# Hansard-T/FHE-Linformer

Measured on AMD Instinct MI355X. Metric: encrypted Linformer-d128 forward ms/sample, lower is better.
Workload: dtype u64

## Files before the change

### fhe-linformer_amd/csrc/context.cpp

```cpp
#include "context.h"
#include <hip/hip_runtime.h>
#include <algorithm>
#include <cstdio>
#include <cstdlib>
#include <cstring>
#include <sys/random.h>
#include <time.h>
#include <cxxabi.h>
#include <dlfcn.h>
#include <execinfo.h>

namespace fhelin {

void hip_check(hipError_t e, const char* what) {
    if (e != hipSuccess) throw Error(FHELIN_ERR_HIP, std::string(what) + ": " + hipGetErrorString(e));
}

void* DevicePool::raw_malloc(size_t bytes) {
    if (backend_.malloc_fn) return backend_.malloc_fn(bytes);
    void* p = nullptr;
    if (hipMalloc(&p, bytes) != hipSuccess) {
        (void)hipGetLastError();
        return nullptr;
    }
    return p;
}
void DevicePool::raw_free(void* p) {
    if (backend_.free_fn) backend_.free_fn(p);
    else (void)hipFree(p);
}
DevicePool::~DevicePool() {
    for (auto& ln : lane_) {
        for (auto& pk : ln.parked)
            for (int k = 0; k < pk.n_ev; ++k) (void)hipEventDestroy(pk.ev[k]);
        for (auto& sl : ln.slabs)
            if (sl.base) raw_free(sl.base);
    }
    for (hipEvent_t e : spare_events_) (void)hipEventDestroy(e);
}
size_t DevicePool::slabs() const {
    size_t n = 0;
    for (const auto& ln : lane_)
        for (const auto& sl : ln.slabs) n += sl.base != nullptr;
    return n;
}
size_t DevicePool::free_ranges() const {
    size_t n = 0;
    for (const auto& ln : lane_) n += ln.by_size.size();
    return n;
}
void DevicePool::erase_size_entry(Lane& ln, int slab, size_t off, size_t len) {
    auto r = ln.by_size.equal_range(len);
    for (auto it = r.first; it != r.second; ++it)
        if (it->second.first == slab && it->second.second == off) {
            ln.by_size.erase(it);
            return;
        }
    throw Error(FHELIN_ERR_INTERNAL, "DevicePool: free list out of step");
}
void DevicePool::insert_free(Lane& ln, int slab, size_t off, size_t len) {
    Slab& sl = ln.slabs[slab];
    auto nxt = sl.free_at.lower_bound(off);
    if (nxt != sl.free_at.begin()) {
        auto prv = std::prev(nxt);
        if (prv->first + prv->second == off) {
            off = prv->first;
            len += prv->second;
            erase_size_entry(ln, slab, prv->first, prv->second);
            sl.free_at.erase(prv);
        }
    }
    if (nxt != sl.free_at.end() && off + len == nxt->first) {
        len += nxt->second;
        erase_size_entry(ln, slab, nxt->first, nxt->second);
        sl.free_at.erase(nxt);
    }
    sl.free_at[off] = len;
    ln.by_size.emplace(len, std::make_pair(slab, off));
}
bool DevicePool::grow(Lane& ln, size_t bytes) {
    size_t want = std::max(bytes, std::min(SLAB_MAX, std::max(SLAB_MIN, reserved_)));
    want = (want + (size_t(2) << 20) - 1) & ~((size_t(2) << 20) - 1);
    timespec t0, t1;
    clock_gettime(CLOCK_MONOTONIC, &t0);
    void* p = raw_malloc(want);
    if (!p && want > bytes) {
        want = (bytes + (size_t(2) << 20) - 1) & ~((size_t(2) << 20) - 1);
        p = raw_malloc(want);
    }
    clock_gettime(CLOCK_MONOTONIC, &t1);
    if (!p) return false;
    malloc_calls += 1;
    malloc_bytes += want;
    malloc_ns += (u64)((t1.tv_sec - t0.tv_sec) * 1000000000ll + (t1.tv_nsec - t0.tv_nsec));
    reserved_ += want;
    if (reserved_ > reserved_peak) reserved_peak = reserved_;
    int idx = -1;
    for (size_t i = 0; i < ln.slabs.size(); ++i)
        if (!ln.slabs[i].base) idx = (int)i;
    if (idx < 0) {
        ln.slabs.emplace_back();
        idx = (int)ln.slabs.size() - 1;
    }
    Slab& sl = ln.slabs[idx];
    sl.base = static_cast<char*>(p);
    sl.size = want;
    sl.used = 0;
    sl.free_at.clear();
    insert_free(ln, idx, 0, want);
    return true;
}
void* DevicePool::alloc(size_t bytes) {
    if (bytes == 0) bytes = 256;
    const size_t gran = bytes > (size_t(64) << 10) ? 4096 : 256;
    bytes = (bytes + gran - 1) & ~(gran - 1);
    Lane& ln = lane_[cur_lane];
    if (!ln.parked.empty()) {
        for (auto& pk : ln.parked) {
            for (int k = 0; k < pk.n_ev; ++k) {
                hip_check(hipStreamWaitEvent(lane_stream[cur_lane], pk.ev[k], 0), "hipStreamWaitEvent(pool reuse)");
                spare_events_.push_back(pk.ev[k]);
            }
            insert_free(ln, pk.slab, pk.off, pk.len);
        }
        ln.parked.clear();
    }
    auto it = ln.by_size.lower_bound(bytes);
    if (it == ln.by_size.end()) {
        if (!grow(ln, bytes)) {
            trim();
            if (!grow(ln, bytes)) throw Error(FHELIN_ERR_HIP, "hipMalloc: out of device memory (" + std::to_string(bytes >> 20) + " MiB asked, " +
                                                                  std::to_string(reserved_ >> 20) + " MiB held, " + std::to_string(live_bytes_ >> 20) + " MiB in use)");
        }
        it = ln.by_size.lower_bound(bytes);
    }
    const int slab = it->second.first;
    const size_t off = it->second.second, len = it->first;
    Slab& sl = ln.slabs[slab];
    ln.by_size.erase(it);
    sl.free_at.erase(off);
    if (len > bytes) {
        sl.free_at[off + bytes] = len - bytes;
        ln.by_size.emplace(len - bytes, std::make_pair(slab, off + bytes));
    }
    sl.used += bytes;
    void* p = sl.base + off;
    live_[p] = Live{bytes, cur_lane, slab, off};
    live_bytes_ += bytes;
    if (live_bytes_ > live_peak) live_peak = live_bytes_;
    return p;
}
void DevicePool::free(void* p, unsigned used_by_lanes) {
    if (!p) return;
    auto it = live_.find(p);
    if (it == live_.end()) throw Error(FHELIN_ERR_STATE, "DevicePool::free of unknown pointer");
    const Live lv = it->second;
    live_.erase(it);
    live_bytes_ -= lv.bytes;
    Lane& ln = lane_[lv.lane];
    ln.slabs[lv.slab].used -= lv.bytes;
    unsigned wait = used_by_lanes;
    if (have_streams && lv.lane != cur_lane) {
        wait |= 1u << cur_lane;
        if (conservative_foreign_free)
            for (int k = 0; k <= n_user_lanes; ++k) wait |= 1u << k;
    }
    wait &= ~(1u << lv.lane);
    if (!have_streams || !wait) {
        insert_free(ln, lv.slab, lv.off, lv.bytes);
        return;
    }
    Parked pk{lv.slab, lv.off, lv.bytes, {}, 0};
    for (int k = 0; k < MAX_LANES; ++k) {
        if (!(wait & (1u << k)) || !lane_stream[k]) continue;
        hipEvent_t ev = nullptr;
        if (!spare_events_.empty()) {
            ev = spare_events_.back();
            spare_events_.pop_back();
        } else {
            hip_check(hipEventCreateWithFlags(&ev, hipEventDisableTiming), "hipEventCreate(pool)");
        }
        hip_check(hipEventRecord(ev, lane_stream[k]), "hipEventRecord(pool free)");
        pk.ev[pk.n_ev++] = ev;
    }
    foreign_frees += 1;
    ln.parked.push_back(pk);
}
void DevicePool::trim() {
    trims += 1;
    if (!backend_.malloc_fn) (void)hipDeviceSynchronize();
    for (auto& ln : lane_) {
        for (auto& pk : ln.parked) {
            for (int k = 0; k < pk.n_ev; ++k) spare_events_.push_back(pk.ev[k]);
            insert_free(ln, pk.slab, pk.off, pk.len);
        }
        ln.parked.clear();
        for (size_t i = 0; i < ln.slabs.size(); ++i) {
            Slab& sl = ln.slabs[i];
            if (!sl.base || sl.used != 0) continue;
            erase_size_entry(ln, (int)i, 0, sl.size);
            raw_free(sl.base);
            reserved_ -= sl.size;
            sl = Slab();
        }
    }
}

template <class T>
const T* Context::upload_table(const std::vector<T>& v) {
    void* p = nullptr;
    size_t bytes = std::max<size_t>(v.size() * sizeof(T), 16);
    hip_check(hipMalloc(&p, bytes), "hipMalloc(table)");
    if (!v.empty()) hip_check(hipMemcpy(p, v.data(), v.size() * sizeof(T), hipMemcpyHostToDevice), "hipMemcpy(table)");
    table_allocs.push_back(p);
    return static_cast<const T*>(p);
}
template const u64* Context::upload_table<u64>(const std::vector<u64>&);
template const int* Context::upload_table<int>(const std::vector<int>&);
template const u32* Context::upload_table<u32>(const std::vector<u32>&);
template const double* Context::upload_table<double>(const std::vector<double>&);

static u64 mont_r(u64 m) { return (u64)((((u128)1) << 64) % m); }

static u64 prod_mod(const std::vector<u64>& ms, int skip, u64 t) {
    u64 r = 1 % t;
    for (int i = 0; i < (int)ms.size(); ++i)
        if (i != skip) r = h_mulmod(r, ms[i] % t, t);
    return r;
}

static void resolve_seed(Params& p) {
    if (p.have_seed_bytes) return;
    if (p.seed != 0) {
        std::memset(p.seed_bytes, 0, sizeof p.seed_bytes);
        for (int i = 0; i < 8; ++i) p.seed_bytes[i] = (uint8_t)(p.seed >> (8 * i));
    } else {
        size_t got = 0;
        while (got < sizeof p.seed_bytes) {
            const ssize_t n = getrandom(p.seed_bytes + got, sizeof p.seed_bytes - got, 0);
            if (n <= 0) throw Error(FHELIN_ERR_INTERNAL, "getrandom failed: no entropy for key generation");
            got += (size_t)n;
        }
    }
    p.have_seed_bytes = true;
}

static Params resolve_params(Params p) {
    resolve_seed(p);
    if (p.n_p < 0 && p.n_q >= 1 && p.dnum >= 1 && p.special_bits >= 1) {
        const int a = (p.n_q + p.dnum - 1) / p.dnum;
        const int first = p.first_bits + (std::min(a, p.n_q) - 1) * p.scale_bits;
        const int other = p.n_q > a ? std::min(a, p.n_q - a) * p.scale_bits : 0;
        p.n_p = (std::max(first, other) + p.special_bits - 1) / p.special_bits;
    }
    return p;
}

Context::Context(const Params& p_in) : prm(resolve_params(p_in)) {
    const Params& p = prm;
    if (p.log_n < 12 || p.log_n > 17) throw Error(FHELIN_ERR_ARG, "log_n must be in [12,17]");
    if (p.n_q < 1 || p.n_q > 64 || p.n_p < 0 || p.n_p > 16) throw Error(FHELIN_ERR_ARG, "bad limb counts");
    if (p.dnum < 1) throw Error(FHELIN_ERR_ARG, "dnum must be >= 1");
    if (p.first_bits > 60 || p.scale_bits > 60 || p.special_bits > 60) throw Error(FHELIN_ERR_ARG, "primes must be <= 60 bits");
    if (p.first_bits < 20 || p.scale_bits < 20 || (p.n_p > 0 && p.special_bits < 20)) throw Error(FHELIN_ERR_ARG, "primes must be >= 20 bits");
    if (p.log_slots < 1 || p.log_slots > p.log_n - 1) throw Error(FHELIN_ERR_ARG, "log_slots out of range");
    N = 1 << p.log_n;
    L = p.n_q - 1;
    K = p.n_p;
    alpha = (p.n_q + p.dnum - 1) / p.dnum;
    if (alpha > 16) throw Error(FHELIN_ERR_ARG, "digit size > 16 limbs not supported");
    if ((p.n_q + alpha - 1) / alpha > 16) throw Error(FHELIN_ERR_ARG, "more than 16 key-switching digits not supported");
    try {
        chain = make_prime_chain(p.log_n, p.n_q, p.first_bits, p.scale_bits, p.n_p, p.special_bits);
    } catch (const std::exception& e) {
        throw Error(FHELIN_ERR_ARG, std::string("prime chain: ") + e.what());
    }
    moduli = chain.q;
    moduli.insert(moduli.end(), chain.p.begin(), chain.p.end());
    for (u64 q : moduli)
        if (q >> 60) throw Error(FHELIN_ERR_ARG, "prime chain: a modulus is >= 2^60 (lower scale_bits or first_bits)");
    for (u64 q : moduli) {
        barrett.push_back(h_barrett(q));
        tw.push_back(make_twiddles(q, p.log_n));
    }
    sf_real.assign(p.n_q + 1, 0.0L);
    sf_real[0] = (long double)chain.q[L];
    for (int k = 0; k < L; ++k) sf_real[k + 1] = sf_real[k] * sf_real[k] / (long double)chain.q[L - k];

    if (p.device < 0) return;

    int ndev = 0;
    if (hipGetDeviceCount(&ndev) != hipSuccess || ndev <= 0)
        throw Error(FHELIN_ERR_NO_DEVICE, "no HIP device visible: the fhe-linformer_amd engine has no CPU fallback");
    if (p.device >= ndev) throw Error(FHELIN_ERR_ARG, "device index out of range");
    hip_check(hipSetDevice(p.device), "hipSetDevice");
    hip_check(hipStreamCreateWithFlags(&stream, hipStreamNonBlocking), "hipStreamCreate");
    main_stream = stream;
    own_stream = true;
    {
        int want = 2;
        if (const char* e = std::getenv("FHELIN_LANES")) want = std::atoi(e);
        n_lanes = std::max(0, std::min(want, DevicePool::MAX_LANES - 1));
        for (int k = 1; k <= n_lanes; ++k) {
            hip_check(hipStreamCreateWithFlags(&lane_stream[k], hipStreamNonBlocking), "hipStreamCreate(lane)");
            hip_check(hipEventCreateWithFlags(&lane_event[k], hipEventDisableTiming), "hipEventCreate(lane)");
        }
        hip_check(hipEventCreateWithFlags(&fork_event, hipEventDisableTiming), "hipEventCreate(fork)");
        pool.lane_stream[0] = main_stream;
        for (int k = 1; k <= n_lanes; ++k) pool.lane_stream[k] = lane_stream[k];
        pool.have_streams = true;
        if (const char* e = std::getenv("FHELIN_ASYNC")) async_lanes = std::atoi(e) != 0;
        if (const char* e = std::getenv("FHELIN_FUSE_MODDOWN")) fuse_moddown = std::atoi(e) != 0;
        if (const char* e = std::getenv("FHELIN_FUSE_FINISH")) fuse_finish = std::atoi(e) != 0;
        if (const char* e = std::getenv("FHELIN_HOST_ENCODE")) host_encode = std::atoi(e) != 0;
        if (const char* e = std::getenv("FHELIN_FUSE_GATHER")) fuse_gather = std::atoi(e) != 0;
        if (const char* e = std::getenv("FHELIN_FUSE_LIFT")) fuse_lift = std::atoi(e) != 0;
        if (const char* e = std::getenv("FHELIN_LDS_DIGITS")) lds_digits = std::atoi(e) != 0;
        if (const char* e = std::getenv("FHELIN_NTT_TRACE")) trace_small_ntt = std::atoi(e);
        if (const char* e = std::getenv("FHELIN_HOST_WAITS")) trace_waits = std::atoi(e) != 0;
    }
    hip_check(hipEventCreate(&ev_start), "hipEventCreate");
    stage_words = (size_t)2 << p.log_n;
    for (int i = 0; i < STAGE_SLOTS; ++i) {
        hip_check(hipHostMalloc(reinterpret_cast<void**>(&stage_buf[i]), stage_words * sizeof(u64), hipHostMallocDefault), "hipHostMalloc(stage)");
        hip_check(hipEventCreateWithFlags(&stage_ev[i], hipEventDisableTiming), "hipEventCreate(stage)");
    }
    hip_check(hipHostMalloc(reinterpret_cast<void**>(&small_buf), (size_t)SMALL_SLOTS * SMALL_WORDS * sizeof(u64), hipHostMallocDefault), "hipHostMalloc(stage, small)");
    for (int i = 0; i < SMALL_SLOTS; ++i) hip_check(hipEventCreateWithFlags(&small_ev[i], hipEventDisableTiming), "hipEventCreate(stage, small)");
    hip_check(hipEventCreate(&ev_stop), "hipEventCreate");
    has_device = true;

    const int nl = (int)moduli.size();
    {
        std::vector<u64> bar(2 * nl), ninv(8 * nl, 0);
        for (int i = 0; i < nl; ++i) {
            bar[2 * i] = barrett[i].r0;
            bar[2 * i + 1] = barrett[i].r1;
            ninv[8 * i] = tw[i].n_inv;
            ninv[8 * i + 1] = tw[i].n_inv_s;
            ninv[8 * i + 2] = tw[i].w1_n_inv;
            ninv[8 * i + 3] = tw[i].w1_n_inv_s;
            int bits = 0;
            while (bits < 64 && (moduli[i] >> bits)) ++bits;
            if (bits >= 12 && bits <= 60) {
                ninv[8 * i + 4] = (u64)(bits - 10);
                ninv[8 * i + 5] = (u64)((((u128)1) << (bits + 22)) / moduli[i]);
            }
        }
        dt.log_n = p.log_n;
        dt.n_limbs = nl;
        dt.moduli = upload_table(moduli);
        dt.barrett = upload_table(bar);
        {
            std::vector<u64> qi(nl);
            for (int i = 0; i < nl; ++i) {
                u64 x = moduli[i];
                for (int it = 0; it < 6; ++it) x *= 2 - moduli[i] * x;
                qi[i] = x;
            }
            dt.qinv = upload_table(qi);
            std::vector<u64> mr(2 * (size_t)nl);
            for (int i = 0; i < nl; ++i) {
                mr[2 * i] = mont_r(moduli[i]);
                mr[2 * i + 1] = h_shoup(mr[2 * i], moduli[i]);
            }
            dt.mont = upload_table(mr);
        }
        dt.ninv = upload_table(ninv);
        std::vector<u64> f((size_t)nl * 2 * N), g((size_t)nl * 2 * N);
        for (int i = 0; i < nl; ++i) {
            std::memcpy(&f[(size_t)i * 2 * N], tw[i].fwd.data(), sizeof(u64) * 2 * N);
            std::memcpy(&g[(size_t)i * 2 * N], tw[i].inv.data(), sizeof(u64) * 2 * N);
        }
        dt.tw_fwd = upload_table(f);
        dt.tw_inv = upload_table(g);
        const size_t tiles = N >> 12;
        const size_t per_limb = tiles * 15 * 256 * 2;
        for (int dir = 0; dir < 2; ++dir) {
            const std::vector<u64>& src = dir ? g : f;
            std::vector<u64> r((size_t)nl * per_limb);
            for (int i = 0; i < nl; ++i)
                for (size_t T = 0; T < tiles; ++T)
                    for (int kb = 0; kb < 4; ++kb)
                        for (int j = 0; j < (8 >> kb); ++j)
                            for (size_t tau = 0; tau < 256; ++tau) {
                                const size_t idx = (N >> (kb + 1)) + ((((T << 8) | tau)) << (3 - kb)) + j;
                                const size_t s_ = (size_t)(8 >> kb) - 1 + j;
                                const size_t o = (size_t)i * per_limb + ((T * 15 + s_) * 256 + tau) * 2;
                                r[o] = src[(size_t)i * 2 * N + 2 * idx];
                                r[o + 1] = src[(size_t)i * 2 * N + 2 * idx + 1];
                            }
            (dir ? dt.tw_rows_inv : dt.tw_rows_fwd) = upload_table(r);
        }
    }
    {
        std::vector<u64> phatinv(2 * std::max(K, 1)), phatmod((size_t)std::max(K, 1) * (L + 1)), pinv(2 * (L + 1));
        for (int j = 0; j < K; ++j) {
            u64 pj = chain.p[j];
            u64 hat = prod_mod(chain.p, j, pj);
            u64 inv = h_invmod(hat, pj);
            phatinv[2 * j] = inv;
            phatinv[2 * j + 1] = h_shoup(inv, pj);
            for (int t = 0; t <= L; ++t) phatmod[(size_t)j * (L + 1) + t] = pack30(h_mulmod(prod_mod(chain.p, j, chain.q[t]), mont_r(chain.q[t]), chain.q[t]));
        }
        for (int t = 0; t <= L; ++t) {
            u64 qt = chain.q[t];
            u64 pm = prod_mod(chain.p, -1, qt);
            u64 inv = K > 0 ? h_invmod(pm, qt) : 1;
            pinv[2 * t] = inv;
            pinv[2 * t + 1] = h_shoup(inv, qt);
        }
        d_phatinv = upload_table(phatinv);
        d_phatmod = upload_table(phatmod);
        d_pinv = upload_table(pinv);
        std::vector<u64> pmod(2 * (L + 1));
        for (int t = 0; t <= L; ++t) {
            pmod[2 * t] = prod_mod(chain.p, -1, chain.q[t]);
            pmod[2 * t + 1] = h_shoup(pmod[2 * t], chain.q[t]);
        }
        d_pmod = upload_table(pmod);
        std::vector<u64> qlinv((size_t)(L + 1) * (L + 1) * 2, 0), qlmod((size_t)(L + 1) * (L + 1), 0);
        for (int l = 0; l <= L; ++l)
            for (int t = 0; t < l; ++t) {
                u64 qt = chain.q[t];
                u64 r = chain.q[l] % qt;
                u64 inv = h_invmod(r, qt);
                qlmod[(size_t)l * (L + 1) + t] = r;
                qlinv[((size_t)l * (L + 1) + t) * 2] = inv;
                qlinv[((size_t)l * (L + 1) + t) * 2 + 1] = h_shoup(inv, qt);
            }
        d_qlinv = upload_table(qlinv);
        d_qlmod = upload_table(qlmod);
    }
    lvl.resize(L + 2);
    for (int ell = 1; ell <= L + 1; ++ell) {
        LevelTables& lt = lvl[ell];
        lt.ell = ell;
        lt.beta = digits_at(ell);
        const int nt = ell + K;
        std::vector<u64> hatinv(2 * ell), hatmod((size_t)ell * nt, 0), hatmod2((size_t)ell * nt, 0);
        std::vector<int> tab((size_t)lt.beta * nt, -1);
        for (int j = 0; j < lt.beta; ++j) {
            const int lo = j * alpha, hi = std::min((j + 1) * alpha, ell);
            std::vector<u64> dig(chain.q.begin() + lo, chain.q.begin() + hi);
            for (int i = lo; i < hi; ++i) {
                u64 qi = chain.q[i];
                u64 inv = h_invmod(prod_mod(dig, i - lo, qi), qi);
                hatinv[2 * i] = inv;
                hatinv[2 * i + 1] = h_shoup(inv, qi);
                for (int t = 0; t < nt; ++t) {
                    u64 mt = t < ell ? chain.q[t] : chain.p[t - ell];
                    const u64 hr = h_mulmod(prod_mod(dig, i - lo, mt), mont_r(mt), mt);
                    hatmod[(size_t)i * nt + t] = pack30(hr);
                    hatmod2[(size_t)i * nt + t] = pack30(h_mulmod(hr, mont_r(mt), mt));
                }
            }
            for (int t = 0; t < nt; ++t) {
                bool own = t >= lo && t < hi;
                tab[(size_t)j * nt + t] = own ? -1 : (t < ell ? limb_id_q(t) : limb_id_p(t - ell));
            }
        }
        lt.up_hatinv = upload_table(hatinv);
        lt.up_hatmod = upload_table(hatmod);
        lt.up_hatmod_r2 = upload_table(hatmod2);
        lt.ext_limb_tab = upload_table(tab);
        if (ell >= 2 && K >= 1) {
            const u64 ql = chain.q[ell - 1];
            const int e1 = ell - 1;
            std::vector<u64> mhi(2 * (K + 1)), mhm((size_t)(K + 1) * e1), minv(2 * e1), mmod(e1);
            for (int j = 0; j <= K; ++j) {
                const u64 b = j < K ? chain.p[j] : ql;
                const u64 hat_b = j < K ? h_mulmod(prod_mod(chain.p, j, b), ql % b, b) : prod_mod(chain.p, -1, b);
                const u64 inv = h_invmod(hat_b, b);
                mhi[2 * j] = inv;
                mhi[2 * j + 1] = h_shoup(inv, b);
                for (int t = 0; t < e1; ++t) {
                    const u64 qt = chain.q[t];
                    mhm[(size_t)j * e1 + t] = pack30(j < K ? h_mulmod(prod_mod(chain.p, j, qt), ql % qt, qt) : prod_mod(chain.p, -1, qt));
                }
            }
            for (int t = 0; t < e1; ++t) {
                const u64 qt = chain.q[t];
                mmod[t] = h_mulmod(prod_mod(chain.p, -1, qt), ql % qt, qt);
                const u64 inv = h_invmod(mmod[t], qt);
                minv[2 * t] = inv;
                minv[2 * t + 1] = h_shoup(inv, qt);
            }
            lt.md_hatinv = upload_table(mhi);
            lt.md_hatmod = upload_table(mhm);
            lt.md_minv = upload_table(minv);
            lt.md_mmod = upload_table(mmod);
        }
    }
}

void Context::upload_async(u64* dst, const u64* src, size_t words) {
    if (words <= SMALL_WORDS && small_buf) {
        const int i = small_next;
        small_next = (small_next + 1) % SMALL_SLOTS;
        if (small_used[i]) {
            timespec a, b;
            if (trace_waits) clock_gettime(CLOCK_MONOTONIC, &a);
            hip_check(hipEventSynchronize(small_ev[i]), "hipEventSynchronize(stage, small)");
            if (trace_waits) {
                clock_gettime(CLOCK_MONOTONIC, &b);
                note_wait("upload ring (small)", (u64)((b.tv_sec - a.tv_sec) * 1000000000ll + (b.tv_nsec - a.tv_nsec)));
            }
        }
        u64* slot = small_buf + (size_t)i * SMALL_WORDS;
        std::memcpy(slot, src, words * sizeof(u64));
        hip_check(hipMemcpyAsync(dst, slot, words * sizeof(u64), hipMemcpyHostToDevice, stream), "hipMemcpyAsync(stage, small)");
        hip_check(hipEventRecord(small_ev[i], stream), "hipEventRecord(stage, small)");
        small_used[i] = true;
        return;
    }
    if (words > stage_words) throw Error(FHELIN_ERR_INTERNAL, "upload_async: block larger than a staging slot");
    const int i = stage_next;
    stage_next = (stage_next + 1) % STAGE_SLOTS;
    if (stage_used[i]) {
        timespec a, b;
        if (trace_waits) clock_gettime(CLOCK_MONOTONIC, &a);
        hip_check(hipEventSynchronize(stage_ev[i]), "hipEventSynchronize(stage)");
        if (trace_waits) {
            clock_gettime(CLOCK_MONOTONIC, &b);
            note_wait("upload ring (large)", (u64)((b.tv_sec - a.tv_sec) * 1000000000ll + (b.tv_nsec - a.tv_nsec)));
        }
    }
    std::memcpy(stage_buf[i], src, words * sizeof(u64));
    hip_check(hipMemcpyAsync(dst, stage_buf[i], words * sizeof(u64), hipMemcpyHostToDevice, stream), "hipMemcpyAsync(stage)");
    hip_check(hipEventRecord(stage_ev[i], stream), "hipEventRecord(stage)");
    stage_used[i] = true;
}

Context::~Context() {
    if (trace_waits) {
        fprintf(stderr, "[fhelin] host time blocked inside the library, by site (waits, ms):\n");
        for (const auto& e : wait_sites) fprintf(stderr, "  %8llu %10.1f  %s\n", (unsigned long long)e.second.first, e.second.second / 1e6, e.first.c_str());
    }
    if (trace_small_ntt && !small_ntt_sites.empty()) {
        std::vector<std::pair<std::string, std::pair<u64, u64>>> v(small_ntt_sites.begin(), small_ntt_sites.end());
        std::sort(v.begin(), v.end(), [](const auto& a, const auto& b) { return a.second.first > b.second.first; });
        fprintf(stderr, "[fhelin] transforms of <= %d limb vectors by call stack (launch pairs, limb vectors):\n", trace_small_ntt);
        for (size_t i = 0; i < v.size() && i < 40; ++i)
            fprintf(stderr, "  %8llu %9llu  %s\n", (unsigned long long)v[i].second.first, (unsigned long long)v[i].second.second, v[i].first.c_str());
    }
    if (has_device) {
        (void)hipSetDevice(prm.device);
        (void)hipDeviceSynchronize();
        for (void* p : table_allocs) (void)hipFree(p);
        for (int k = 1; k <= n_lanes; ++k) {
            if (lane_event[k]) (void)hipEventDestroy(lane_event[k]);
            if (lane_stream[k]) (void)hipStreamDestroy(lane_stream[k]);
        }
        if (fork_event) (void)hipEventDestroy(fork_event);
        for (int i = 0; i < STAGE_SLOTS; ++i) {
            if (stage_ev[i]) (void)hipEventDestroy(stage_ev[i]);
            if (stage_buf[i]) (void)hipHostFree(stage_buf[i]);
        }
        for (int i = 0; i < SMALL_SLOTS; ++i)
            if (small_ev[i]) (void)hipEventDestroy(small_ev[i]);
        if (small_buf) (void)hipHostFree(small_buf);
        if (ev_start) (void)hipEventDestroy(ev_start);
        if (ev_stop) (void)hipEventDestroy(ev_stop);
        if (own_stream && main_stream) (void)hipStreamDestroy(main_stream);
    }
}

void Context::require_device() const {
    if (!has_device)
        throw Error(FHELIN_ERR_NO_DEVICE, "operation needs the HIP device path (host-only context): no CPU fallback exists");
}

void Context::sync() {
    require_device();
    hip_check(hipStreamSynchronize(stream), "hipStreamSynchronize");
    if (stream == main_stream) {
        for (int k = 1; k <= n_lanes; ++k) {
            hip_check(hipStreamSynchronize(lane_stream[k]), "hipStreamSynchronize(lane)");
            lane_hold[k].clear();
        }
    }
}

void Context::note_small_ntt(int nvec) {
    void* fr[12];
    const int n = backtrace(fr, 12);
    std::string key;
    for (int i = 2; i < n && i < 9; ++i) {
        Dl_info info;
        std::string name = "?";
        if (dladdr(fr[i], &info) && info.dli_sname) {
            int st = 0;
            char* d = abi::__cxa_demangle(info.dli_sname, nullptr, nullptr, &st);
            name = (st == 0 && d) ? d : info.dli_sname;
            if (d) std::free(d);
            const size_t par = name.find('(');
            if (par != std::string::npos) name.resize(par);
        }
        key += (i > 2 ? " < " : "") + name;
    }
    auto& e = small_ntt_sites[key];
    e.first += 1;
    e.second += (u64)nvec;
}

void Context::release_holds(int lane, u64 up_to_seq) {
    auto& h = lane_hold[lane];
    h.erase(std::remove_if(h.begin(), h.end(), [&](const std::pair<u64, std::shared_ptr<void>>& e) { return e.first <= up_to_seq; }),
            h.end());
}

void Context::fork_lanes() {
    hip_check(hipEventRecord(fork_event, main_stream), "hipEventRecord(fork)");
    for (int k = 1; k <= n_lanes; ++k) hip_check(hipStreamWaitEvent(lane_stream[k], fork_event, 0), "hipStreamWaitEvent(fork)");
}

void Context::join_lanes() {
    for (int k = 1; k <= n_lanes; ++k) {
        hip_check(hipEventRecord(lane_event[k], lane_stream[k]), "hipEventRecord(lane)");
        hip_check(hipStreamWaitEvent(main_stream, lane_event[k], 0), "hipStreamWaitEvent(join)");
    }
}

u64 Context::galois_element(int r) const {
    const u64 M = 2ull * N;
    const u64 order = N / 2;
    long rr = r % (long)order;
    if (rr < 0) rr += order;
    u64 g = 1, b = 5;
    u64 e = (u64)rr;
    while (e) {
        if (e & 1) g = (g * b) % M;
        b = (b * b) % M;
        e >>= 1;
    }
    return g;
}

static std::vector<u32> build_automorph_map(u64 g, size_t N, int ln) {
    const u64 M = 2ull * N;
    std::vector<u32> m(N);
    for (u32 j = 0; j < (u32)N; ++j) {
        u64 e = (2ull * bitrev32(j, ln) + 1) * g % M;
        m[j] = bitrev32((u32)((e - 1) >> 1), ln);
    }
    return m;
}

const u32* Context::automorph_map(u64 g) {
    require_device();
    auto it = automorph_maps.find(g);
    if (it != automorph_maps.end()) return it->second;
    const u64 M = 2ull * N;
    u64 gi = g;
    for (int i = 0; i < 6; ++i) gi = gi * (2 - g * gi % M + M) % M;
    const u32* d = upload_table(build_automorph_map(g, N, prm.log_n));
    automorph_maps[g] = d;
    const u32* di = d;
    if (gi != g) {
        auto iit = automorph_maps.find(gi);
        di = iit != automorph_maps.end() ? iit->second : upload_table(build_automorph_map(gi, N, prm.log_n));
        automorph_maps[gi] = di;
    }
    automorph_inverse[d] = di;
    automorph_inverse[di] = d;
    return d;
}

const u32* Context::automorph_inverse_of(const u32* map) {
    if (!map) return nullptr;
    auto it = automorph_inverse.find(map);
    if (it == automorph_inverse.end()) throw Error(FHELIN_ERR_INTERNAL, "automorphism map without a registered inverse");
    return it->second;
}

}
```

### fhe-linformer_amd/csrc/context.h

```cpp
#pragma once
#include <cstdint>
#include <map>
#include <memory>
#include <stdexcept>
#include <string>
#include <unordered_map>
#include <vector>
#include <hip/hip_runtime_api.h>
#include "../../include/fhelin.h"
#include "hostmath.h"
#include "kernels.h"

namespace fhelin {

struct Params {
    int log_n = 16;
    int n_q = 24;
    int first_bits = 55;
    int scale_bits = 52;
    int n_p = 6;
    int special_bits = 60;
    int dnum = 4;
    int log_slots = 14;
    int hamming = 192;
    uint64_t seed = 0;
    uint8_t seed_bytes[32] = {};
    bool have_seed_bytes = false;
    int device = 0;
};

struct Error : std::runtime_error {
    int code;
    Error(int c, const std::string& m) : std::runtime_error(m), code(c) {}
};

void hip_check(hipError_t e, const char* what);

class DevicePool {
public:
    static constexpr int MAX_LANES = 5;
    static constexpr size_t SLAB_MAX = size_t(8) << 30, SLAB_MIN = size_t(32) << 20;
    struct Backend {
        void* (*malloc_fn)(size_t) = nullptr;
        void (*free_fn)(void*) = nullptr;
    };
    DevicePool() = default;
    explicit DevicePool(const Backend& b) : backend_(b) {}
    ~DevicePool();
    void* alloc(size_t bytes);
    void free(void* p, unsigned used_by_lanes = 0);
    bool conservative_foreign_free = false;
    int n_user_lanes = 0;
    void trim();
    size_t bytes_reserved() const { return reserved_; }
    size_t bytes_live() const { return live_bytes_; }
    size_t slabs() const;
    size_t free_ranges() const;
    int cur_lane = 0;
    hipStream_t lane_stream[MAX_LANES] = {};
    bool have_streams = false;
    u64 malloc_calls = 0, malloc_bytes = 0, malloc_ns = 0;
    u64 foreign_frees = 0;
    u64 trims = 0;
    size_t live_peak = 0, reserved_peak = 0;
private:
    struct Slab {
        char* base = nullptr;
        size_t size = 0, used = 0;
        std::map<size_t, size_t> free_at;
    };
    struct Live { size_t bytes; int lane; int slab; size_t off; };
    struct Parked { int slab; size_t off, len; hipEvent_t ev[MAX_LANES]; int n_ev; };
    struct Lane {
        std::vector<Slab> slabs;
        std::multimap<size_t, std::pair<int, size_t>> by_size;
        std::vector<Parked> parked;
    };
    Backend backend_;
    Lane lane_[MAX_LANES];
    std::unordered_map<void*, Live> live_;
    std::vector<hipEvent_t> spare_events_;
    size_t reserved_ = 0, live_bytes_ = 0;
    void insert_free(Lane& ln, int slab, size_t off, size_t len);
    void erase_size_entry(Lane& ln, int slab, size_t off, size_t len);
    bool grow(Lane& ln, size_t bytes);
    void* raw_malloc(size_t bytes);
    void raw_free(void* p);
};

template <class T>
class Scratch {
public:
    Scratch() = default;
    Scratch(DevicePool& pool, size_t count) : pool_(&pool), p_(static_cast<T*>(pool.alloc(count * sizeof(T)))) {}
    Scratch(Scratch&& o) noexcept : pool_(o.pool_), p_(o.release()) {}
    Scratch& operator=(Scratch&& o) noexcept {
        if (this != &o) {
            drop();
            pool_ = o.pool_;
            p_ = o.release();
        }
        return *this;
    }
    Scratch(const Scratch&) = delete;
    Scratch& operator=(const Scratch&) = delete;
    ~Scratch() { drop(); }
    operator T*() const& { return p_; }
    operator T*() && = delete;
    T* get() const { return p_; }
    void reset() {
        if (T* p = release()) pool_->free(p);
    }
    T* release() noexcept {
        T* p = p_;
        p_ = nullptr;
        return p;
    }
private:
    void drop() noexcept {
        try { reset(); } catch (...) {}
    }
    DevicePool* pool_ = nullptr;
    T* p_ = nullptr;
};

struct LevelTables {
    int ell = 0;
    int beta = 0;
    const u64* up_hatinv = nullptr;
    const u64* up_hatmod = nullptr;
    const u64* up_hatmod_r2 = nullptr;
    const int* ext_limb_tab = nullptr;
    const u64* md_hatinv = nullptr;
    const u64* md_hatmod = nullptr;
    const u64* md_minv = nullptr;
    const u64* md_mmod = nullptr;
};

struct OpStats {
    u64 limb_ntt = 0;
    u64 keyswitch = 0;
    u64 keyswitch_limbs = 0;
    u64 rescale = 0;
    u64 ct_pt_mult = 0;
    u64 bootstrap = 0;
    u64 encode = 0;
    u64 rescale_limbs = 0;
    u64 ct_pt_limbs = 0;
};

struct Context {
    Params prm;
    OpStats stats;
    int N = 0;
    int L = 0;
    int K = 0;
    int alpha = 0;
    PrimeChain chain;
    std::vector<u64> moduli;
    std::vector<Barrett> barrett;
    std::vector<TwiddleTable> tw;
    std::vector<long double> sf_real;

    bool has_device = false;
    hipStream_t stream = nullptr;
    hipStream_t main_stream = nullptr;
    bool own_stream = false;
    int n_lanes = 0;
    hipStream_t lane_stream[DevicePool::MAX_LANES] = {};
    hipEvent_t lane_event[DevicePool::MAX_LANES] = {};
    hipEvent_t fork_event = nullptr;
    bool async_lanes = true;
    int async_rr = 0;
    u64 lane_seq[DevicePool::MAX_LANES] = {};
    std::vector<std::pair<u64, std::shared_ptr<void>>> lane_hold[DevicePool::MAX_LANES];
    void release_holds(int lane, u64 up_to_seq);
    void fork_lanes();
    void join_lanes();
    struct LaneScope {
        Context& c;
        LaneScope(Context& ctx, int k) : c(ctx) {
            c.stream = c.lane_stream[k];
            c.pool.cur_lane = k;
        }
        ~LaneScope() {
            c.stream = c.main_stream;
            c.pool.cur_lane = 0;
        }
    };
    DevicePool pool;
    DeviceTables dt{};
    std::vector<void*> table_allocs;
    hipEvent_t ev_start = nullptr, ev_stop = nullptr;

    static constexpr int STAGE_SLOTS = 64;
    u64* stage_buf[STAGE_SLOTS] = {};
    hipEvent_t stage_ev[STAGE_SLOTS] = {};
    bool stage_used[STAGE_SLOTS] = {};
    int stage_next = 0;
    size_t stage_words = 0;
    static constexpr int SMALL_SLOTS = 256;
    static constexpr size_t SMALL_WORDS = 8192;
    u64* small_buf = nullptr;
    hipEvent_t small_ev[SMALL_SLOTS] = {};
    bool small_used[SMALL_SLOTS] = {};
    int small_next = 0;
    void upload_async(u64* dst, const u64* src, size_t words);

    const u64* d_phatinv = nullptr;
    const u64* d_phatmod = nullptr;
    const u64* d_pinv = nullptr;
    const u64* d_pmod = nullptr;
    const u64* d_qlinv = nullptr;
    const u64* d_qlmod = nullptr;
    std::vector<LevelTables> lvl;
    std::map<u64, const u32*> automorph_maps;

    explicit Context(const Params& p);
    ~Context();
    Context(const Context&) = delete;
    Context& operator=(const Context&) = delete;

    void require_device() const;
    template <class T> T* dalloc(size_t count) { return static_cast<T*>(pool.alloc(count * sizeof(T))); }
    template <class T> Scratch<T> scratch(size_t count) { return Scratch<T>(pool, count); }
    template <class T> const T* upload_table(const std::vector<T>& v);
    int limb_id_q(int i) const { return i; }
    int limb_id_p(int j) const { return L + 1 + j; }
    int digits_at(int ell) const { return (ell + alpha - 1) / alpha; }
    u64 galois_element(int rot_index) const;
    const u32* automorph_map(u64 galois);
    const u32* automorph_inverse_of(const u32* map);
    std::map<const u32*, const u32*> automorph_inverse;
    bool fuse_finish = true;
    bool fuse_moddown = false;
    bool host_encode = false;
    bool fuse_gather = true;
    bool fuse_lift = true;
    bool lds_digits = true;
    struct FftDev {
        const u32* rot = nullptr;
        const double* ksi = nullptr;
    };
    std::map<int, FftDev> fft_dev;
    void sync();
    void ntt(const LimbBatch& b, bool inverse, int active = -1) {
        stats.limb_ntt += (u64)(active >= 0 ? active : b.nvec);
        if (trace_small_ntt && b.nvec <= trace_small_ntt) note_small_ntt(b.nvec);
        launch_ntt(dt, b, inverse, stream);
    }
    bool trace_waits = false;
    std::map<std::string, std::pair<u64, u64>> wait_sites;
    void note_wait(const char* site, u64 ns) {
        auto& e = wait_sites[site];
        e.first += 1;
        e.second += ns;
    }
    int trace_small_ntt = 0;
    std::map<std::string, std::pair<u64, u64>> small_ntt_sites;
    void note_small_ntt(int nvec);
    void ntt_epilogue(const LimbBatch& b, const NttEpilogue& ep) {
        stats.limb_ntt += (u64)b.nvec;
        if (trace_small_ntt && b.nvec <= trace_small_ntt) note_small_ntt(b.nvec);
        launch_ntt_epilogue(dt, b, ep, stream);
    }
};

}
```

### fhe-linformer_amd/csrc/evaluator.cpp

```cpp
#include "evaluator.h"
#include <map>
#include <hip/hip_runtime.h>
#include <cmath>
#include <cstring>

namespace fhelin {

DevBlock::~DevBlock() {
    if (d && ctx) {
        try { ctx->pool.free(d); } catch (...) {}
    }
}
Ciphertext::~Ciphertext() {
    if (async_ev) (void)hipEventDestroy(async_ev);
    if (d && ctx && !block) {
        try { ctx->pool.free(d); } catch (...) {}
    }
}
Encoding::~Encoding() {
    if (ready) (void)hipEventDestroy(ready);
    if (d && ctx) {
        try { ctx->pool.free(d, lanes_ordered); } catch (...) {}
    }
}
EvalKey::~EvalKey() {
    if (d && ctx) {
        try { ctx->pool.free(d); } catch (...) {}
    }
    if (d_perm && ctx) {
        try { ctx->pool.free(d_perm); } catch (...) {}
    }
}

static void launch_ok(const char* what) { hip_check(hipGetLastError(), what); }

CtPtr Evaluator::new_ct(int npoly, int ell, int deg, long double scale, int slots) {
    c_.require_device();
    if (ell < 1 || ell > c_.L + 1 || npoly < 1 || npoly > 3) throw Error(FHELIN_ERR_ARG, "new_ct: bad shape");
    auto ct = std::make_shared<Ciphertext>();
    ct->ctx = &c_;
    ct->npoly = npoly;
    ct->ell = ell;
    ct->deg = deg;
    ct->scale = scale;
    ct->slots = slots;
    ct->d = c_.dalloc<u64>(ct->words());
    return ct;
}

CtPtr Evaluator::clone(const CtPtr& a) {
    CtPtr o = new_ct(a->npoly, a->ell, a->deg, a->scale, a->slots);
    hip_check(hipMemcpyAsync(o->d, a->d, a->words() * 8, hipMemcpyDeviceToDevice, c_.stream), "clone");
    return o;
}

std::vector<CtPtr> Evaluator::new_ct_batch(int count, int npoly, int ell, int deg, long double scale, int slots) {
    c_.require_device();
    if (count < 1 || ell < 1 || ell > c_.L + 1 + (c_.K > 0 ? 1 : 0) || npoly < 1 || npoly > 3) throw Error(FHELIN_ERR_ARG, "new_ct_batch: bad shape");
    auto blk = std::make_shared<DevBlock>();
    blk->ctx = &c_;
    const size_t words = (size_t)npoly * ell * c_.N;
    blk->d = c_.dalloc<u64>(words * count);
    std::vector<CtPtr> v;
    for (int i = 0; i < count; ++i) {
        auto ct = std::make_shared<Ciphertext>();
        ct->ctx = &c_;
        ct->npoly = npoly;
        ct->ell = ell;
        ct->deg = deg;
        ct->scale = scale;
        ct->slots = slots;
        ct->block = blk;
        ct->d = blk->d + words * i;
        v.push_back(ct);
    }
    return v;
}

u64* Evaluator::contiguous_base(const std::vector<CtPtr>& v) {
    if (v.empty() || !v[0]->block) return nullptr;
    const size_t words = v[0]->words();
    for (size_t i = 0; i < v.size(); ++i)
        if (v[i]->block != v[0]->block || v[i]->d != v[0]->d + words * i || v[i]->words() != words) return nullptr;
    return v[0]->d;
}

std::vector<CtPtr> Evaluator::make_contiguous(const std::vector<CtPtr>& v, int site) {
    if (v.size() <= 1 || contiguous_base(v)) return v;
    if (site >= 0 && site < 8) gather_copies[site] += v.size();
    std::vector<CtPtr> o = new_ct_batch((int)v.size(), v[0]->npoly, v[0]->ell, v[0]->deg, v[0]->scale, v[0]->slots);
    for (size_t lo = 0; lo < v.size(); lo += EwItems::MAX_ITEMS) {
        EwItems it;
        it.n = (int)std::min<size_t>(EwItems::MAX_ITEMS, v.size() - lo);
        it.vecs = v[0]->npoly * v[0]->ell;
        it.b_vecs = 0;
        for (int i = 0; i < it.n; ++i) {
            if (v[lo + i]->words() != v[0]->words()) throw Error(FHELIN_ERR_INTERNAL, "make_contiguous: operands of different shapes");
            it.out[i] = o[lo + i]->d;
            it.a[i] = v[lo + i]->d;
            it.b[i] = nullptr;
        }
        launch_ew_items(c_.dt, it, 4, v[0]->ell, c_.stream);
    }
    hip_check(hipGetLastError(), "batch gather");
    return o;
}

KeyPtr Evaluator::new_key() {
    c_.require_device();
    auto k = std::make_shared<EvalKey>();
    k->ctx = &c_;
    k->digits = c_.digits_at(c_.L + 1);
    k->d = c_.dalloc<u64>(k->words());
    return k;
}

void Evaluator::keyswitch(const u64* c_ntt, int ell, const EvalKey& key, u64* out, const u64* add0, const u64* add1,
                          const u32* map, const u64* post) {
    keyswitch_batch(1, c_ntt, 0, ell, key, out, 0, add0, add1, 0, map, post, 0);
}

void Evaluator::keyswitch_batch(int B, const u64* c_ntt, size_t c_stride, int ell, const EvalKey& key, u64* out, size_t out_stride,
                                const u64* add0, const u64* add1, size_t add_stride, const u32* map, const u64* post,
                                size_t post_stride) {
    keyswitch_impl(B, nullptr, c_ntt, c_stride, ell, &key, out, out_stride, add0, add1, add_stride, map, post, post_stride);
}

void Evaluator::keyswitch_rows(const KsRows& rows, const u64* c_ntt, size_t c_stride, int ell, u64* out, size_t out_stride,
                               const u64* add0, size_t add_stride) {
    const int B = (int)rows.keys.size();
    if (B < 1) return;
    if (B > KsShape::MAX_ROWS || rows.maps.size() != rows.keys.size()) throw Error(FHELIN_ERR_ARG, "keyswitch_rows: bad row count");
    keyswitch_impl(B, &rows, c_ntt, c_stride, ell, nullptr, out, out_stride, add0, nullptr, add_stride, nullptr, nullptr, 0);
}

void Evaluator::keyswitch_impl(int B, const KsRows* rows, const u64* c_ntt, size_t c_stride, int ell, const EvalKey* key, u64* out,
                               size_t out_stride, const u64* add0, const u64* add1, size_t add_stride, const u32* map, const u64* post,
                               size_t post_stride) {
    c_.require_device();
    if (c_.K < 1) throw Error(FHELIN_ERR_STATE, "hybrid key switching needs at least one special prime");
    if (B < 1) return;
    const size_t N = c_.N;
    const int K = c_.K;
    KsShape sh{ell, K, c_.alpha, c_.lvl[ell].beta, c_.L + 1, B, c_stride, out_stride, add_stride, post_stride};
    const bool shared = rows && rows->shared_input;
    if (rows) {
        sh.per_row = 1;
        sh.shared_input = shared ? 1 : 0;
        for (int b = 0; b < B; ++b) {
            sh.evk_row[b] = rows->keys[b]->d;
            sh.map_row[b] = rows->maps[b];
        }
    }
    KsShape shu = sh;
    shu.batch = shared ? 1 : B;
    c_.stats.keyswitch += (u64)B;
    c_.stats.keyswitch_limbs += (u64)B * ell;
    Scratch<u64> ext = modup(shu, c_ntt, true);
    Scratch<u64> accQ = c_.scratch<u64>((size_t)B * 2 * ell * N);
    Scratch<u64> accP = c_.scratch<u64>((size_t)B * 2 * K * N);
    launch_ks_inner(c_.dt, sh, accQ, accP, ext, key ? key->d : nullptr, c_ntt, c_.stream);
    const bool identity = !map && !rows;
    moddown(sh, accQ, accP, out, add0, add1, map, post, c_.fuse_moddown || (c_.fuse_finish && identity));
    launch_ok("keyswitch");
}


Scratch<u64> Evaluator::modup(const KsShape& up, const u64* src, bool times_r2, int group2, size_t group2_stride) {
    const size_t N = c_.N;
    const int n = up.batch, ell = up.ell, nt = ell + c_.K;
    const LevelTables& lt = c_.lvl[ell];
    Scratch<u64> cc = c_.scratch<u64>((size_t)n * ell * N);
    {
        LimbBatch ib{cc, n * ell, nullptr, 0, ell, src};
        if (n > 1 && up.c_stride != (size_t)ell * N) {
            ib.src_group = ell;
            ib.src_group_stride = up.c_stride;
        }
        if (group2 > 0) {
            ib.src_group2 = group2;
            ib.src_group2_stride = group2_stride;
        }
        c_.ntt(ib, true);
    }
    Scratch<u64> ext = c_.scratch<u64>((size_t)n * lt.beta * nt * N);
    launch_modup_conv(c_.dt, up, ext, cc, src, lt.up_hatinv, times_r2 ? lt.up_hatmod_r2 : lt.up_hatmod, c_.stream);
    LimbBatch eb{ext, n * lt.beta * nt, lt.ext_limb_tab, 0, 1};
    eb.tab_len = lt.beta * nt;
    eb.lazy_out = true;
    c_.ntt(eb, false, n * (lt.beta * nt - ell));
    return ext;
}

void Evaluator::moddown(const KsShape& sh, const u64* accQ, u64* accP, u64* out, const u64* add0, const u64* add1, const u32* map,
                        const u64* post, bool row_pass, const std::function<void(const u64* conv)>& finish) {
    const size_t N = c_.N;
    const int B = sh.batch, ell = sh.ell, K = c_.K;
    c_.ntt(LimbBatch{accP, B * 2 * K, nullptr, c_.L + 1, K}, true);
    Scratch<u64> conv = c_.scratch<u64>((size_t)B * 2 * ell * N);
    launch_moddown_conv(c_.dt, sh, conv, accP, c_.d_phatinv, c_.d_phatmod, c_.stream);
    const LimbBatch cb{conv, B * 2 * ell, nullptr, 0, ell};
    if (row_pass) {
        NttEpilogue ep;
        ep.acc = accQ;
        ep.acc_poly_stride = (size_t)ell * N;
        ep.out = out;
        ep.out_stride = sh.out_stride;
        ep.w = c_.d_pinv;
        ep.ell = ell;
        ep.add0 = add0;
        ep.add1 = add1;
        ep.add_stride = sh.add_stride;
        ep.post = post;
        ep.post_stride = sh.post_stride;
        if (sh.per_row) {
            ep.per_row = 1;
            for (int b = 0; b < B; ++b) ep.invmap_row[b] = c_.automorph_inverse_of(sh.map_row[b]);
        } else if (map) {
            ep.invmap = c_.automorph_inverse_of(map);
        }
        c_.ntt_epilogue(cb, ep);
        return;
    }
    c_.ntt(cb, false);
    if (finish) finish(conv);
    else launch_moddown_finish(c_.dt, sh, out, accQ, conv, c_.d_pinv, add0, add1, map, post, c_.stream);
}

void Evaluator::moddown_rescale(const KsShape& sh, const u64* accQ, u64* accP, u64* out) {
    const size_t N = c_.N;
    const int B = sh.batch, ell = sh.ell, K = c_.K;
    const LevelTables& lt = c_.lvl[ell];
    c_.ntt(LimbBatch{accP, B * 2 * K, nullptr, c_.L + 1, K}, true);
    Scratch<u64> top = c_.scratch<u64>((size_t)B * 2 * N);
    {
        LimbBatch tb{top, B * 2, nullptr, ell - 1, 1, accQ + (size_t)(ell - 1) * N};
        tb.src_group = 1;
        tb.src_group_stride = (size_t)ell * N;
        c_.ntt(tb, true);
    }
    Scratch<u64> conv = c_.scratch<u64>((size_t)B * 2 * (ell - 1) * N);
    launch_moddown_rescale_conv(c_.dt, sh, conv, accP, top, lt.md_hatinv, lt.md_hatmod, lt.md_mmod, c_.stream);
    moddown_rescale_finish(sh, out, accQ, conv, lt.md_minv);
}

void Evaluator::moddown_rescale_finish(const KsShape& sh, u64* out, const u64* accQ, u64* conv, const u64* minv) {
    const int e1 = sh.ell - 1;
    const LimbBatch cb{conv, sh.batch * 2 * e1, nullptr, 0, e1};
    if (c_.fuse_finish) {
        NttEpilogue ep;
        ep.acc = accQ;
        ep.acc_poly_stride = (size_t)sh.ell * c_.N;
        ep.out = out;
        ep.out_stride = sh.out_stride;
        ep.w = minv;
        ep.ell = e1;
        c_.ntt_epilogue(cb, ep);
        return;
    }
    c_.ntt(cb, false);
    launch_moddown_rescale_finish(c_.dt, sh, out, accQ, conv, minv, c_.stream);
}

bool Evaluator::have_rotation_keys(const std::vector<int>& indices, int slots) const {
    const int ns = slots > 0 ? slots : (1 << c_.prm.log_slots);
    for (int r : indices) {
        if (r % ns == 0) return false;
        if (!rot_keys.count(c_.galois_element(r))) return false;
    }
    return !indices.empty();
}

const u64* Evaluator::permuted(const EvalKey& key, const u32* map) {
    if (key.d_perm) return key.d_perm;
    const int nvec = key.digits * 2 * (c_.L + 1 + c_.K);
    key.d_perm = c_.dalloc<u64>(key.words());
    launch_automorph_pack30(c_.dt, key.d_perm, key.d, map, nvec, c_.stream);
    launch_ok("key permutation");
    hip_check(hipStreamSynchronize(c_.stream), "key permutation sync");
    return key.d_perm;
}

std::vector<CtPtr> Evaluator::rotate_sum_batch(const std::vector<CtPtr>& vin, const std::vector<int>& indices) {
    if (vin.empty()) return {};
    const int R = (int)indices.size();
    if (R < 1 || R > KsShape::MAX_ROT) throw Error(FHELIN_ERR_ARG, "rotate_sum_batch: 1..7 rotations");
    if (!have_rotation_keys(indices, vin[0]->slots)) throw Error(FHELIN_ERR_KEY, "rotate_sum_batch: missing rotation key");
    if (c_.K < 1) throw Error(FHELIN_ERR_STATE, "hybrid key switching needs at least one special prime");
    std::vector<const EvalKey*> keys;
    std::vector<const u32*> maps;
    for (int r : indices) {
        const u64 g = c_.galois_element(r);
        keys.push_back(rot_keys.at(g).get());
        maps.push_back(c_.automorph_map(g));
    }
    const size_t N = c_.N;
    const int K = c_.K, L1 = c_.L + 1;
    hipStream_t s = c_.stream;
    std::vector<CtPtr> out(vin.size());
    std::vector<char> done(vin.size(), 0);
    for (size_t first = 0; first < vin.size(); ++first) {
        if (done[first]) continue;
        if (vin[first]->npoly != 2) throw Error(FHELIN_ERR_STATE, "rotate: ciphertext must have 2 components");
        std::vector<size_t> idx;
        for (size_t i = first; i < vin.size() && (int)idx.size() < batch_limit; ++i) {
            const CtPtr &a = vin[first], &b = vin[i];
            if (!done[i] && b->npoly == 2 && b->ell == a->ell && b->deg == a->deg && fabsl(b->scale / a->scale - 1.0L) < 1e-9L)
                idx.push_back(i);
        }
        std::vector<CtPtr> chunk;
        for (size_t i : idx) chunk.push_back(vin[i]);
        chunk = make_contiguous(chunk, 0);
        const int B = (int)chunk.size(), ell = chunk[0]->ell;
        const size_t pn = (size_t)ell * N, ctw = 2 * pn;
        const LevelTables& lt = c_.lvl[ell];
        std::vector<CtPtr> o = new_ct_batch(B, 2, ell, chunk[0]->deg, chunk[0]->scale, chunk[0]->slots);
        const u64* base = chunk[0]->d;
        KsShape sh{ell, K, c_.alpha, lt.beta, L1, B, ctw, ctw, pn, ctw};
        sh.n_rot = R;
        sh.lds_digits = c_.lds_digits ? 1 : 0;
        for (int r = 0; r < R; ++r) {
            sh.evk_rot[r] = permuted(*keys[r], maps[r]);
            sh.map_rot[r] = maps[r];
            if (c_.galois_element(indices[r]) % (u64)(c_.N / 256) != 1) sh.lds_digits = 0;
        }
        int steps = 0;
        while ((1 << steps) < R + 1) ++steps;
        c_.stats.keyswitch += (u64)B * steps;
        c_.stats.keyswitch_limbs += (u64)B * steps * ell;
        {
            Scratch<u64> ext = modup(sh, base + pn, false);
            Scratch<u64> accQ = c_.scratch<u64>((size_t)B * 2 * ell * N);
            Scratch<u64> accP = c_.scratch<u64>((size_t)B * 2 * K * N);
            launch_ks_inner_multi(c_.dt, sh, accQ, accP, ext, base + pn, s);
            Scratch<u64> c0sum;
            if (c_.fuse_gather) {
                sh.gsrc = base;
                sh.gsrc_stride = ctw;
            } else {
                c0sum = c_.scratch<u64>((size_t)B * ell * N);
                launch_gather_sum(c_.dt, sh, c0sum, base, ctw, s);
            }
            moddown(sh, accQ, accP, o[0]->d, c0sum, nullptr, nullptr, base);
            launch_ok("rotate_sum_batch");
        }
        for (int b = 0; b < B; ++b) {
            o[b]->scale = vin[idx[b]]->scale;
            out[idx[b]] = o[b];
            done[idx[b]] = 1;
        }
    }
    return out;
}

Evaluator::FoldedKey Evaluator::folded_key(const PtPtr& p, int index, long double scale) {
    const u64 g = c_.galois_element(index);
    auto kit = rot_keys.find(g);
    if (kit == rot_keys.end()) throw Error(FHELIN_ERR_KEY, "no rotation key for index " + std::to_string(index) + " (EvalRotateKeyGen list)");
    for (size_t i = 0; i < folded_keys.size(); ++i) {
        const FoldedKey& f = folded_keys[i];
        if (f.pt.get() == p.get() && f.key.get() == kit->second.get() && f.index == index && f.scale == scale) {
            FoldedKey hit = f;
            if (i + 1 != folded_keys.size()) {
                folded_keys.erase(folded_keys.begin() + i);
                folded_keys.push_back(hit);
            }
            return hit;
        }
    }
    FoldedKey f;
    f.pt = p;
    f.key = kit->second;
    f.index = index;
    f.scale = scale;
    const int nl = c_.L + 1 + c_.K;
    f.enc = p->at(nl, scale);
    f.d = std::make_shared<DevBlock>();
    f.d->ctx = &c_;
    f.d->d = c_.dalloc<u64>(f.key->words());
    launch_fold_key(c_.dt, f.d->d, f.key->d, c_.automorph_map(g), f.enc->d, f.key->digits * 2 * nl, c_.stream);
    launch_ok("fold_key");
    hip_check(hipStreamSynchronize(c_.stream), "fold_key sync");
    if (folded_keys.size() >= MAX_FOLDED) {
        hip_check(hipStreamSynchronize(c_.main_stream), "folded key eviction sync");
        for (int k = 1; k <= c_.n_lanes; ++k) hip_check(hipStreamSynchronize(c_.lane_stream[k]), "folded key eviction sync (lane)");
        folded_keys.erase(folded_keys.begin());
    }
    folded_keys.push_back(f);
    return f;
}

std::vector<CtPtr> Evaluator::hoisted_dot_rows(const std::vector<CtPtr>& xin, const std::vector<PtPtr>& pts, const std::vector<int>& indices,
                                              bool rescale_out) {
    if (xin.empty()) return {};
    const int R = (int)indices.size();
    if (R < 1 || R > KsShape::MAX_ROT || (int)pts.size() != R + 1)
        throw Error(FHELIN_ERR_ARG, "hoisted_dot_rows: 1..7 rotations, one plaintext per rotation + the unrotated term's");
    if (!have_rotation_keys(indices, xin[0]->slots)) throw Error(FHELIN_ERR_KEY, "hoisted_dot_rows: missing rotation key");
    if (c_.K < 1) throw Error(FHELIN_ERR_STATE, "hybrid key switching needs at least one special prime");
    const int ns = xin[0]->slots > 0 ? xin[0]->slots : (1 << c_.prm.log_slots);
    for (int r : indices)
        if (r % ns == 0) throw Error(FHELIN_ERR_ARG, "hoisted_dot_rows: a rotation by 0 is the unrotated term (pts[0])");
    if (rescale_out && c_.K + 1 > 16)
        return rescale_batch(hoisted_dot_rows(xin, pts, indices, false));
    std::vector<CtPtr> x = xin;
    {
        std::vector<CtPtr> need;
        std::vector<size_t> pos;
        for (size_t i = 0; i < x.size(); ++i)
            if (x[i]->deg >= 2) {
                need.push_back(x[i]);
                pos.push_back(i);
            }
        if (!need.empty()) {
            std::vector<CtPtr> r = rescale_batch(need);
            for (size_t k = 0; k < pos.size(); ++k) x[pos[k]] = r[k];
        }
    }
    std::vector<const u32*> maps;
    for (int r : indices) maps.push_back(c_.automorph_map(c_.galois_element(r)));
    const size_t N = c_.N;
    const int K = c_.K, L1 = c_.L + 1;
    hipStream_t s = c_.stream;
    std::vector<CtPtr> out(x.size());
    std::vector<char> done(x.size(), 0);
    for (size_t first = 0; first < x.size(); ++first) {
        if (done[first]) continue;
        if (x[first]->npoly != 2) throw Error(FHELIN_ERR_STATE, "hoisted_dot_rows: ciphertext must have 2 components");
        std::vector<size_t> idx;
        for (size_t i = first; i < x.size() && (int)idx.size() < batch_limit; ++i) {
            const CtPtr &a = x[first], &b = x[i];
            if (!done[i] && b->npoly == 2 && b->ell == a->ell && b->deg == a->deg && fabsl(b->scale / a->scale - 1.0L) < 1e-9L) idx.push_back(i);
        }
        std::vector<CtPtr> chunk;
        for (size_t i : idx) chunk.push_back(x[i]);
        chunk = make_contiguous(chunk, 0);
        const int B = (int)chunk.size(), ell = chunk[0]->ell;
        const size_t pn = (size_t)ell * N, ctw = 2 * pn;
        const LevelTables& lt = c_.lvl[ell];
        const long double sf = c_.sf_real[chunk[0]->level()];
        const bool merged = rescale_out && ell >= 2 && K + 1 <= 16;
        if (rescale_out && !merged) throw Error(FHELIN_ERR_STATE, "hoisted_dot_rows: no limb left to drop");
        const int oell = merged ? ell - 1 : ell;
        std::vector<CtPtr> o = new_ct_batch(B, 2, oell, merged ? chunk[0]->deg : chunk[0]->deg + 1, chunk[0]->scale * sf, chunk[0]->slots);
        const u64* base = chunk[0]->d;
        KsShape sh{ell, K, c_.alpha, lt.beta, L1, B, ctw, (size_t)2 * oell * N, pn, ctw};
        sh.n_rot = R;
        sh.lds_digits = c_.lds_digits ? 1 : 0;
        HoistAdd h;
        h.n_rot = R;
        std::vector<FoldedKey> hold;
        const std::shared_ptr<Encoding> e0 = pts[0]->at(ell, sf);
        h.v[0] = e0->d;
        for (int r = 0; r < R; ++r) {
            hold.push_back(folded_key(pts[r + 1], indices[r], sf));
            sh.evk_rot[r] = hold.back().d->d;
            sh.map_rot[r] = maps[r];
            h.v[r + 1] = hold.back().enc->d;
            h.map[r] = maps[r];
            if (c_.galois_element(indices[r]) % (u64)(c_.N / 256) != 1) sh.lds_digits = 0;
        }
        c_.stats.keyswitch += (u64)B * R;
        c_.stats.keyswitch_limbs += (u64)B * R * ell;
        c_.stats.ct_pt_mult += (u64)B * (R + 1);
        c_.stats.ct_pt_limbs += (u64)B * (R + 1) * ell;
        if (merged) {
            c_.stats.rescale += (u64)B;
            c_.stats.rescale_limbs += (u64)B * ell;
        }
        {
            Scratch<u64> ext = modup(sh, base + pn, false);
            Scratch<u64> accQ = c_.scratch<u64>((size_t)B * 2 * ell * N);
            Scratch<u64> accP = c_.scratch<u64>((size_t)B * 2 * K * N);
            launch_ks_inner_multi(c_.dt, sh, accQ, accP, ext, base + pn, s);
            if (!merged) {
                Scratch<u64> pre = c_.scratch<u64>((size_t)B * ctw);
                launch_hoist_addends(c_.dt, sh, h, pre, base, s);
                moddown(sh, accQ, accP, o[0]->d, nullptr, nullptr, nullptr, pre);
            } else {
                h.acc = accQ;
                h.pmod = c_.d_pmod;
                launch_hoist_addends(c_.dt, sh, h, nullptr, base, s);
                moddown_rescale(sh, accQ, accP, o[0]->d);
            }
            launch_ok("hoisted_dot_rows");
        }
        for (int b = 0; b < B; ++b) {
            o[b]->scale = x[idx[b]]->scale * sf;
            if (merged) o[b]->scale = o[b]->scale / (long double)c_.chain.q[ell - 1];
            out[idx[b]] = o[b];
            done[idx[b]] = 1;
        }
    }
    return out;
}

CtPtr Evaluator::rotate_each_sum(const std::vector<CtPtr>& vin, const std::vector<int>& indices) {
    if (vin.empty() || vin.size() != indices.size()) throw Error(FHELIN_ERR_ARG, "rotate_each_sum: one index per ciphertext");
    const int ns = vin[0]->slots > 0 ? vin[0]->slots : (1 << c_.prm.log_slots);
    std::vector<CtPtr> rot;
    std::vector<int> ridx;
    CtPtr acc;
    for (size_t i = 0; i < vin.size(); ++i) {
        if (indices[i] % ns == 0) acc = acc ? add(acc, vin[i]) : vin[i];
        else {
            rot.push_back(vin[i]);
            ridx.push_back(indices[i]);
        }
    }
    for (size_t first = 0; first < rot.size(); first += KsShape::MAX_ROT) {
        const int R = (int)std::min(rot.size() - first, (size_t)KsShape::MAX_ROT);
        std::vector<CtPtr> chunk(rot.begin() + first, rot.begin() + first + R);
        bool uniform = have_rotation_keys(std::vector<int>(ridx.begin() + first, ridx.begin() + first + R), ns) && c_.K >= 1;
        for (const CtPtr& c : chunk)
            uniform = uniform && c->npoly == 2 && c->ell == chunk[0]->ell && c->deg == chunk[0]->deg &&
                      fabsl(c->scale / chunk[0]->scale - 1.0L) < 1e-9L;
        if (!uniform || R < 2) {
            for (int r = 0; r < R; ++r) {
                CtPtr t = rotate(chunk[r], ridx[first + r]);
                acc = acc ? add(acc, t) : t;
            }
            continue;
        }
        chunk = make_contiguous(chunk, 1);
        const size_t N = c_.N;
        const int K = c_.K, L1 = c_.L + 1, ell = chunk[0]->ell;
        const size_t pn = (size_t)ell * N, ctw = 2 * pn;
        const LevelTables& lt = c_.lvl[ell];
        const int nt = ell + K;
        hipStream_t s = c_.stream;
        const u64* base = chunk[0]->d;
        CtPtr o = new_ct(2, ell, chunk[0]->deg, chunk[0]->scale, chunk[0]->slots);
        {
            Scratch<u64> ext = modup(KsShape{ell, K, c_.alpha, lt.beta, L1, R, ctw, 0, 0, 0}, base + pn, false);
            KsShape sh{ell, K, c_.alpha, lt.beta, L1, 1, 0, ctw, pn, 0};
            sh.n_rot = R;
            sh.rot_ext_stride = (size_t)lt.beta * nt * N;
            sh.rot_input_stride = ctw;
            for (int r = 0; r < R; ++r) {
                const u64 g = c_.galois_element(ridx[first + r]);
                sh.map_rot[r] = c_.automorph_map(g);
                sh.evk_rot[r] = permuted(*rot_keys.at(g), sh.map_rot[r]);
            }
            c_.stats.keyswitch += (u64)R;
            c_.stats.keyswitch_limbs += (u64)R * ell;
            Scratch<u64> accQ = c_.scratch<u64>((size_t)2 * ell * N);
            Scratch<u64> accP = c_.scratch<u64>((size_t)2 * K * N);
            launch_ks_inner_multi(c_.dt, sh, accQ, accP, ext, base + pn, s);
            Scratch<u64> c0sum;
            if (c_.fuse_gather) {
                sh.gsrc = base;
                sh.gsrc_stride = 0;
            } else {
                c0sum = c_.scratch<u64>((size_t)ell * N);
                launch_gather_sum(c_.dt, sh, c0sum, base, 0, s);
            }
            moddown(sh, accQ, accP, o->d, c0sum, nullptr, nullptr, nullptr);
            launch_ok("rotate_each_sum");
        }
        acc = acc ? add(acc, o) : o;
    }
    return acc;
}

std::vector<CtPtr> Evaluator::rotate_each_sum_rows(const std::vector<std::vector<CtPtr>>& rows, const std::vector<int>& indices) {
    if (rows.empty()) return {};
    const int ns = rows[0][0]->slots > 0 ? rows[0][0]->slots : (1 << c_.prm.log_slots);
    std::vector<int> rot_pos, plain_pos, ridx;
    for (size_t r = 0; r < indices.size(); ++r) {
        if (indices[r] % ns == 0) plain_pos.push_back((int)r);
        else {
            rot_pos.push_back((int)r);
            ridx.push_back(indices[r]);
        }
    }
    const int R = (int)rot_pos.size();
    bool uniform = R >= 2 && R <= KsShape::MAX_ROT && have_rotation_keys(ridx, ns) && c_.K >= 1;
    const CtPtr& f = rows[0][0];
    for (const auto& row : rows) {
        uniform = uniform && row.size() == indices.size();
        for (const CtPtr& c : row)
            uniform = uniform && c->npoly == 2 && c->ell == f->ell && c->deg == f->deg && fabsl(c->scale / f->scale - 1.0L) < 1e-9L;
    }
    std::vector<CtPtr> out(rows.size());
    if (!uniform) {
        for (size_t b = 0; b < rows.size(); ++b) out[b] = rotate_each_sum(rows[b], indices);
        return out;
    }
    const size_t N = c_.N;
    const int K = c_.K, L1 = c_.L + 1, ell = f->ell;
    const size_t pn = (size_t)ell * N, ctw = 2 * pn;
    const LevelTables& lt = c_.lvl[ell];
    const int nt = ell + K;
    hipStream_t s = c_.stream;
    const size_t chunk_rows = (size_t)std::max(1, batch_limit / 2);
    for (size_t lo = 0; lo < rows.size(); lo += chunk_rows) {
        const size_t hi = std::min(rows.size(), lo + chunk_rows);
        const int B = (int)(hi - lo);
        std::vector<CtPtr> flat;
        for (size_t b = lo; b < hi; ++b)
            for (int r : rot_pos) flat.push_back(rows[b][r]);
        size_t row_stride = (size_t)R * ctw;
        bool regular = B >= 1 && flat[0]->block != nullptr;
        for (int b = 0; b < B && regular; ++b) {
            for (int r = 0; r < R && regular; ++r) {
                const CtPtr& c = flat[(size_t)b * R + r];
                regular = c->block == flat[0]->block && c->words() == (size_t)ctw &&
                          c->d == flat[(size_t)b * R]->d + (size_t)r * ctw;
            }
            if (regular && b == 1) {
                regular = flat[R]->d > flat[0]->d;
                if (regular) row_stride = (size_t)(flat[R]->d - flat[0]->d);
            }
            if (regular && b >= 1) regular = flat[(size_t)b * R]->d == flat[0]->d + (size_t)b * row_stride;
        }
        if (!regular) {
            flat = make_contiguous(flat, 2);
            row_stride = (size_t)R * ctw;
        }
        const u64* base = flat[0]->d;
        std::vector<CtPtr> o = new_ct_batch(B, 2, ell, f->deg, f->scale, f->slots);
        {
            const bool spaced = row_stride != (size_t)R * ctw;
            Scratch<u64> ext = modup(KsShape{ell, K, c_.alpha, lt.beta, L1, B * R, ctw, 0, 0, 0}, base + pn, false, spaced ? R : 0,
                                     spaced ? row_stride : 0);
            KsShape sh{ell, K, c_.alpha, lt.beta, L1, B, row_stride, ctw, pn, 0};
            sh.n_rot = R;
            sh.rot_ext_stride = (size_t)lt.beta * nt * N;
            sh.rot_input_stride = ctw;
            sh.ext_batch_stride = (size_t)R * lt.beta * nt * N;
            for (int r = 0; r < R; ++r) {
                const u64 g = c_.galois_element(ridx[r]);
                sh.map_rot[r] = c_.automorph_map(g);
                sh.evk_rot[r] = permuted(*rot_keys.at(g), sh.map_rot[r]);
            }
            sh.gsrc = base;
            sh.gsrc_stride = row_stride;
            c_.stats.keyswitch += (u64)B * R;
            c_.stats.keyswitch_limbs += (u64)B * R * ell;
            Scratch<u64> accQ = c_.scratch<u64>((size_t)B * 2 * ell * N);
            Scratch<u64> accP = c_.scratch<u64>((size_t)B * 2 * K * N);
            launch_ks_inner_multi(c_.dt, sh, accQ, accP, ext, base + pn, s);
            moddown(sh, accQ, accP, o[0]->d, nullptr, nullptr, nullptr, nullptr);
            launch_ok("rotate_each_sum_rows");
        }
        for (int b = 0; b < B; ++b) out[lo + b] = o[b];
    }
    if (!plain_pos.empty()) {
        std::vector<CtPtr> acc(rows.size());
        for (size_t b = 0; b < rows.size(); ++b) acc[b] = rows[b][plain_pos[0]];
        for (size_t k = 1; k < plain_pos.size(); ++k) {
            std::vector<CtPtr> t(rows.size());
            for (size_t b = 0; b < rows.size(); ++b) t[b] = rows[b][plain_pos[k]];
            acc = add_batch(acc, t);
        }
        out = add_batch(acc, out);
    }
    return out;
}

std::vector<CtPtr> Evaluator::rotate_many(const CtPtr& a, const std::vector<int>& indices) {
    if (a->npoly != 2) throw Error(FHELIN_ERR_STATE, "rotate: ciphertext must have 2 components");
    const int ns = a->slots > 0 ? a->slots : (1 << c_.prm.log_slots);
    std::vector<CtPtr> out(indices.size());
    std::vector<size_t> todo;
    for (size_t i = 0; i < indices.size(); ++i) {
        if (indices[i] % ns == 0) out[i] = a;
        else todo.push_back(i);
    }
    const size_t pn = (size_t)a->ell * c_.N, ctw = 2 * pn;
    for (size_t first = 0; first < todo.size(); first += KsShape::MAX_ROWS) {
        const int B = (int)std::min(todo.size() - first, (size_t)KsShape::MAX_ROWS);
        if (B == 1) {
            out[todo[first]] = rotate(a, indices[todo[first]]);
            continue;
        }
        KsRows rows;
        rows.shared_input = true;
        for (int b = 0; b < B; ++b) {
            const int index = indices[todo[first + b]];
            const u64 g = c_.galois_element(index);
            auto it = rot_keys.find(g);
            if (it == rot_keys.end())
                throw Error(FHELIN_ERR_KEY, "no rotation key for index " + std::to_string(index) + " (EvalRotateKeyGen list)");
            rows.keys.push_back(it->second.get());
            rows.maps.push_back(c_.automorph_map(g));
        }
        std::vector<CtPtr> o = new_ct_batch(B, 2, a->ell, a->deg, a->scale, a->slots);
        keyswitch_rows(rows, a->d + pn, 0, a->ell, o[0]->d, ctw, a->d, 0);
        for (int b = 0; b < B; ++b) out[todo[first + b]] = o[b];
    }
    return out;
}

std::vector<CtPtr> Evaluator::rotate_each(const std::vector<CtPtr>& vin, const std::vector<int>& indices) {
    if (vin.size() != indices.size()) throw Error(FHELIN_ERR_ARG, "rotate_each: one index per ciphertext");
    std::vector<CtPtr> out(vin.size());
    std::vector<char> done(vin.size(), 0);
    for (size_t first = 0; first < vin.size(); ++first) {
        if (done[first]) continue;
        const CtPtr& a = vin[first];
        if (a->npoly != 2) throw Error(FHELIN_ERR_STATE, "rotate: ciphertext must have 2 components");
        const int ns = a->slots > 0 ? a->slots : (1 << c_.prm.log_slots);
        if (indices[first] % ns == 0) {
            out[first] = clone(a);
            done[first] = 1;
            continue;
        }
        std::vector<size_t> idx;
        for (size_t i = first; i < vin.size() && (int)idx.size() < std::min(batch_limit, (int)KsShape::MAX_ROWS); ++i) {
            const CtPtr& b = vin[i];
            if (!done[i] && indices[i] % ns != 0 && b->npoly == 2 && b->ell == a->ell && b->deg == a->deg &&
                fabsl(b->scale / a->scale - 1.0L) < 1e-9L)
                idx.push_back(i);
        }
        if (idx.size() < 2) {
            out[first] = rotate(a, indices[first]);
            done[first] = 1;
            continue;
        }
        std::vector<CtPtr> chunk;
        KsRows rows;
        for (size_t i : idx) {
            chunk.push_back(vin[i]);
            const u64 g = c_.galois_element(indices[i]);
            auto it = rot_keys.find(g);
            if (it == rot_keys.end())
                throw Error(FHELIN_ERR_KEY, "no rotation key for index " + std::to_string(indices[i]) + " (EvalRotateKeyGen list)");
            rows.keys.push_back(it->second.get());
            rows.maps.push_back(c_.automorph_map(g));
        }
        chunk = make_contiguous(chunk, 3);
        const int B = (int)chunk.size();
        const size_t pn = (size_t)a->ell * c_.N, ctw = 2 * pn;
        std::vector<CtPtr> o = new_ct_batch(B, 2, a->ell, a->deg, a->scale, a->slots);
        keyswitch_rows(rows, chunk[0]->d + pn, ctw, a->ell, o[0]->d, ctw, chunk[0]->d, ctw);
        for (int b = 0; b < B; ++b) {
            o[b]->scale = vin[idx[b]]->scale;
            out[idx[b]] = o[b];
            done[idx[b]] = 1;
        }
    }
    return out;
}

void Evaluator::lift_and_ntt(u64* lifted, const u64* last, int P, int ell, const NttEpilogue* ep, const u64* qlm_row) {
    auto ntt = [&](const LimbBatch& b) {
        if (ep)
            c_.ntt_epilogue(b, *ep);
        else
            c_.ntt(b, false);
    };
    const u64* qlm = qlm_row ? qlm_row : c_.d_qlmod + (size_t)(ell - 1) * (c_.L + 1);
    bool fuse = c_.fuse_lift;
    for (int j = 0; j + 1 < ell && fuse; ++j) fuse = c_.moduli[ell - 1] < 2 * c_.chain.q[j];
    if (fuse) {
        LimbBatch fb{lifted, P * (ell - 1), nullptr, 0, ell - 1, last};
        fb.lift_qlm = qlm;
        fb.lift_limb = ell - 1;
        ntt(fb);
        return;
    }
    launch_rescale_lift(c_.dt, lifted, last, P, ell, qlm, c_.stream);
    ntt(LimbBatch{lifted, P * (ell - 1), nullptr, 0, ell - 1});
}

void Evaluator::rescale_finish(u64* out, const u64* c, const u64* last, int P, int ell, const u64* qlinv_row, const u64* qlm_row) {
    const size_t N = c_.N;
    const u64* qlinv = qlinv_row ? qlinv_row : c_.d_qlinv + (size_t)(ell - 1) * (c_.L + 1) * 2;
    Scratch<u64> lifted = c_.scratch<u64>((size_t)P * (ell - 1) * N);
    if (c_.fuse_finish) {
        NttEpilogue ep;
        ep.acc = c;
        ep.acc_poly_stride = (size_t)ell * N;
        ep.out = out;
        ep.out_stride = (size_t)2 * (ell - 1) * N;
        ep.w = qlinv;
        ep.ell = ell - 1;
        lift_and_ntt(lifted, last, P, ell, &ep, qlm_row);
    } else {
        lift_and_ntt(lifted, last, P, ell, nullptr, qlm_row);
        launch_rescale_finish(c_.dt, out, c, lifted, P, ell, qlinv, c_.stream);
    }
}

CtPtr Evaluator::raw_rescale(const CtPtr& a) {
    const int ell = a->ell, P = a->npoly;
    if (ell < 2) throw Error(FHELIN_ERR_STATE, "rescale: no limb left to drop");
    const size_t N = c_.N;
    Scratch<u64> last = c_.scratch<u64>((size_t)P * N);
    c_.stats.rescale += 1;
    c_.stats.rescale_limbs += (u64)ell;
    {
        LimbBatch lb{last, P, nullptr, ell - 1, 1, a->d + (size_t)(ell - 1) * N};
        lb.src_group = 1;
        lb.src_group_stride = (size_t)ell * N;
        c_.ntt(lb, true);
    }
    CtPtr o = new_ct(P, ell - 1, a->deg, a->scale, a->slots);
    rescale_finish(o->d, a->d, last, P, ell);
    launch_ok("rescale");
    return o;
}

CtPtr Evaluator::raw_rotate(const CtPtr& a, u64 g, const EvalKey& key, bool accumulate) {
    if (a->npoly != 2) throw Error(FHELIN_ERR_STATE, "rotate: ciphertext must have 2 components");
    const size_t pn = (size_t)a->ell * c_.N;
    CtPtr o = new_ct(2, a->ell, a->deg, a->scale, a->slots);
    keyswitch(a->d + pn, a->ell, key, o->d, a->d, nullptr, c_.automorph_map(g), accumulate ? a->d : nullptr);
    return o;
}

std::vector<CtPtr> Evaluator::rotate_batch(const std::vector<CtPtr>& vin, int index) { return rotate_batch_impl(vin, index, false); }
std::vector<CtPtr> Evaluator::rotate_add_batch(const std::vector<CtPtr>& vin, int index) { return rotate_batch_impl(vin, index, true); }

std::vector<CtPtr> Evaluator::rotate_batch_impl(const std::vector<CtPtr>& vin, int index, bool accumulate) {
    if (vin.empty()) return {};
    const int ns = vin[0]->slots > 0 ? vin[0]->slots : (1 << c_.prm.log_slots);
    std::vector<CtPtr> out(vin.size());
    if (vin.size() == 1 || index % ns == 0) {
        for (size_t i = 0; i < vin.size(); ++i) out[i] = accumulate ? rotate_add(vin[i], index) : rotate(vin[i], index);
        return out;
    }
    const u64 g = c_.galois_element(index);
    auto it = rot_keys.find(g);
    if (it == rot_keys.end())
        throw Error(FHELIN_ERR_KEY, "no rotation key for index " + std::to_string(index) + " (EvalRotateKeyGen list)");
    return rotate_galois_batch(vin, g, *it->second, accumulate);
}

std::vector<CtPtr> Evaluator::conjugate_batch(const std::vector<CtPtr>& v) {
    if (!conj_key) throw Error(FHELIN_ERR_KEY, "no conjugation key");
    return rotate_galois_batch(v, 2ull * c_.N - 1, *conj_key, false);
}

std::vector<CtPtr> Evaluator::rotate_galois_batch(const std::vector<CtPtr>& vin, u64 g, const EvalKey& key, bool accumulate) {
    std::vector<CtPtr> out(vin.size());
    if (vin.size() == 1) {
        out[0] = raw_rotate(vin[0], g, key, accumulate);
        return out;
    }
    const u32* map = c_.automorph_map(g);
    std::vector<char> done(vin.size(), 0);
    for (size_t first = 0; first < vin.size(); ++first) {
        if (done[first]) continue;
        if (vin[first]->npoly != 2) throw Error(FHELIN_ERR_STATE, "rotate: ciphertext must have 2 components");
        std::vector<size_t> idx;
        for (size_t i = first; i < vin.size() && (int)idx.size() < batch_limit; ++i) {
            const CtPtr &a = vin[first], &b = vin[i];
            if (!done[i] && b->npoly == 2 && b->ell == a->ell && b->deg == a->deg && fabsl(b->scale / a->scale - 1.0L) < 1e-9L)
                idx.push_back(i);
        }
        std::vector<CtPtr> chunk;
        for (size_t i : idx) chunk.push_back(vin[i]);
        chunk = make_contiguous(chunk, 4);
        const int B = (int)chunk.size();
        const int ell = chunk[0]->ell;
        const size_t pn = (size_t)ell * c_.N, ctw = 2 * pn;
        std::vector<CtPtr> o = new_ct_batch(B, 2, ell, chunk[0]->deg, chunk[0]->scale, chunk[0]->slots);
        const u64* base = chunk[0]->d;
        keyswitch_batch(B, base + pn, ctw, ell, key, o[0]->d, ctw, base, nullptr, ctw, map, accumulate ? base : nullptr, ctw);
        for (int b = 0; b < B; ++b) {
            o[b]->scale = vin[idx[b]]->scale;
            out[idx[b]] = o[b];
            done[idx[b]] = 1;
        }
    }
    return out;
}

std::vector<std::vector<CtPtr>> Evaluator::rotate_many_batch(const std::vector<CtPtr>& xs, const std::vector<int>& indices) {
    std::vector<std::vector<CtPtr>> out(xs.size());
    if (xs.empty()) return out;
    bool uniform = xs.size() >= 2 && !c_.fuse_moddown && c_.K >= 1;
    for (const CtPtr& x : xs)
        uniform = uniform && x->npoly == 2 && x->ell == xs[0]->ell && x->deg == xs[0]->deg && x->slots == xs[0]->slots;
    if (!uniform) {
        for (size_t i = 0; i < xs.size(); ++i) out[i] = rotate_many(xs[i], indices);
        return out;
    }
    const int ns = xs[0]->slots > 0 ? xs[0]->slots : (1 << c_.prm.log_slots);
    std::vector<size_t> todo;
    for (size_t i = 0; i < xs.size(); ++i) out[i].resize(indices.size());
    for (size_t k = 0; k < indices.size(); ++k) {
        if (indices[k] % ns == 0)
            for (size_t i = 0; i < xs.size(); ++i) out[i][k] = xs[i];
        else
            todo.push_back(k);
    }
    const int R = (int)todo.size();
    if (R == 0) return out;
    std::vector<const EvalKey*> keys;
    std::vector<const u32*> maps;
    for (size_t k : todo) {
        const u64 g = c_.galois_element(indices[k]);
        auto it = rot_keys.find(g);
        if (it == rot_keys.end())
            throw Error(FHELIN_ERR_KEY, "no rotation key for index " + std::to_string(indices[k]) + " (EvalRotateKeyGen list)");
        keys.push_back(it->second.get());
        maps.push_back(c_.automorph_map(g));
    }
    const size_t N = c_.N;
    const int K = c_.K, L1 = c_.L + 1, ell = xs[0]->ell;
    const size_t pn = (size_t)ell * N, ctw = 2 * pn;
    const LevelTables& lt = c_.lvl[ell];
    const int nt = ell + K;
    hipStream_t s = c_.stream;
    const size_t per_pass = (size_t)std::max(1, 160 / R);
    for (size_t lo = 0; lo < xs.size(); lo += per_pass) {
        const size_t hi = std::min(xs.size(), lo + per_pass);
        const int B = (int)(hi - lo);
        std::vector<CtPtr> in = make_contiguous(std::vector<CtPtr>(xs.begin() + lo, xs.begin() + hi), 6);
        const u64* base = in[0]->d;
        const int rows = B * R;
        c_.stats.keyswitch += (u64)rows;
        c_.stats.keyswitch_limbs += (u64)rows * ell;
        std::vector<CtPtr> o = new_ct_batch(rows, 2, ell, xs[lo]->deg, xs[lo]->scale, xs[lo]->slots);
        {
            Scratch<u64> ext = modup(KsShape{ell, K, c_.alpha, lt.beta, L1, B, ctw, 0, 0, 0}, base + pn, true);
            Scratch<u64> accQ = c_.scratch<u64>((size_t)rows * 2 * ell * N);
            Scratch<u64> accP = c_.scratch<u64>((size_t)rows * 2 * K * N);
            auto row_shape = [&](int first, int cnt) {
                KsShape sh{ell, K, c_.alpha, lt.beta, L1, B * cnt, ctw, ctw, ctw, 0};
                sh.per_row = 1;
                sh.shared_input = 1;
                sh.row_mod = cnt;
                sh.ext_batch_stride = (size_t)lt.beta * nt * N;
                for (int b = 0; b < cnt; ++b) {
                    sh.evk_row[b] = keys[first + b]->d;
                    sh.map_row[b] = maps[first + b];
                }
                return sh;
            };
            auto for_row_chunks = [&](auto&& launch) {
                for (int i = 0; i < B; ++i)
                    for (int first = 0; first < R; first += KsShape::MAX_ROWS) {
                        const int cnt = std::min(R - first, (int)KsShape::MAX_ROWS);
                        KsShape sh1{ell, K, c_.alpha, lt.beta, L1, cnt, 0, ctw, 0, 0};
                        sh1.per_row = 1;
                        sh1.shared_input = 1;
                        for (int b = 0; b < cnt; ++b) {
                            sh1.evk_row[b] = keys[first + b]->d;
                            sh1.map_row[b] = maps[first + b];
                        }
                        launch(sh1, (size_t)i * R + first, i);
                    }
            };
            const bool one_chunk = R <= (int)KsShape::MAX_ROWS;
            if (one_chunk) launch_ks_inner(c_.dt, row_shape(0, R), accQ, accP, ext, nullptr, base + pn, s);
            else
                for_row_chunks([&](const KsShape& sh1, size_t row0, int i) {
                    launch_ks_inner(c_.dt, sh1, accQ + row0 * 2 * ell * N, accP + row0 * 2 * K * N, ext + (size_t)i * lt.beta * nt * N, nullptr,
                                    base + pn + (size_t)i * ctw, s);
                });
            moddown(KsShape{ell, K, c_.alpha, lt.beta, L1, rows, 0, ctw, 0, 0}, accQ, accP, nullptr, nullptr, nullptr, nullptr, nullptr, false,
                    [&](const u64* conv) {
                        if (one_chunk) launch_moddown_finish(c_.dt, row_shape(0, R), o[0]->d, accQ, conv, c_.d_pinv, base, nullptr, nullptr, nullptr, s);
                        else
                            for_row_chunks([&](const KsShape& sh1, size_t row0, int i) {
                                launch_moddown_finish(c_.dt, sh1, o[row0]->d, accQ + row0 * 2 * ell * N, conv + row0 * 2 * ell * N, c_.d_pinv,
                                                      base + (size_t)i * ctw, nullptr, nullptr, nullptr, s);
                            });
                    });
            launch_ok("rotate_many_batch");
        }
        for (int i = 0; i < B; ++i)
            for (int r = 0; r < R; ++r) {
                o[(size_t)i * R + r]->scale = xs[lo + i]->scale;
                out[lo + i][todo[r]] = o[(size_t)i * R + r];
            }
    }
    return out;
}

std::vector<CtPtr> Evaluator::rescale_batch(const std::vector<CtPtr>& vin) {
    std::vector<CtPtr> out(vin.size());
    std::vector<char> done(vin.size(), 0);
    for (size_t first = 0; first < vin.size(); ++first) {
        if (done[first]) continue;
        std::vector<size_t> idx;
        for (size_t i = first; i < vin.size() && (int)idx.size() < batch_limit; ++i)
            if (!done[i] && vin[i]->npoly == 2 && vin[first]->npoly == 2 && vin[i]->ell == vin[first]->ell) idx.push_back(i);
        if (idx.size() < 2) {
            out[first] = rescale(vin[first]);
            done[first] = 1;
            continue;
        }
        std::vector<CtPtr> chunk;
        for (size_t i : idx) chunk.push_back(vin[i]);
        chunk = make_contiguous(chunk, 5);
        const int B = (int)chunk.size(), ell = chunk[0]->ell, P = 2 * B;
        if (ell < 2) throw Error(FHELIN_ERR_STATE, "rescale: no limb left to drop");
        const size_t N = c_.N;
        const u64* base = chunk[0]->d;
        Scratch<u64> last = c_.scratch<u64>((size_t)P * N);
        c_.stats.rescale += (u64)B;
        c_.stats.rescale_limbs += (u64)B * ell;
        LimbBatch lb{last, P, nullptr, ell - 1, 1, base + (size_t)(ell - 1) * N};
        lb.src_group = 1;
        lb.src_group_stride = (size_t)ell * N;
        c_.ntt(lb, true);
        std::vector<CtPtr> o = new_ct_batch(B, 2, ell - 1, 1, 0, chunk[0]->slots);
        rescale_finish(o[0]->d, base, last, P, ell);
        launch_ok("rescale_batch");
        last.reset();
        for (int b = 0; b < B; ++b) {
            const CtPtr& a = vin[idx[b]];
            o[b]->scale = a->scale / (long double)c_.chain.q[ell - 1];
            o[b]->deg = a->deg > 1 ? a->deg - 1 : 1;
            out[idx[b]] = o[b];
            done[idx[b]] = 1;
        }
    }
    return out;
}

std::vector<CtPtr> Evaluator::mult_plain_batch(const std::vector<CtPtr>& vin, const PtPtr& p) {
    return mult_plain_each(vin, std::vector<PtPtr>(vin.size(), p));
}

namespace {
template <class SameShape, class Emit>
void for_runs(size_t n, SameShape same, Emit emit) {
    size_t lo = 0;
    while (lo < n) {
        size_t hi = lo + 1;
        while (hi < n && hi - lo < (size_t)EwItems::MAX_ITEMS && same(lo, hi)) ++hi;
        emit(lo, hi);
        lo = hi;
    }
}
}

std::vector<CtPtr> Evaluator::mult_plain_each(const std::vector<CtPtr>& vin, const std::vector<PtPtr>& p) {
    if (vin.size() != p.size()) throw Error(FHELIN_ERR_ARG, "mult_plain_each: one plaintext per ciphertext");
    if (vin.empty()) return {};
    std::vector<CtPtr> x = vin;
    {
        std::vector<CtPtr> need;
        std::map<const Ciphertext*, size_t> slot;
        for (size_t i = 0; i < vin.size(); ++i)
            if (vin[i]->deg >= 2 && !slot.count(vin[i].get())) {
                slot[vin[i].get()] = need.size();
                need.push_back(vin[i]);
            }
        if (!need.empty()) {
            std::vector<CtPtr> r = rescale_batch(need);
            for (size_t i = 0; i < vin.size(); ++i)
                if (vin[i]->deg >= 2) x[i] = r[slot[vin[i].get()]];
        }
    }
    std::vector<CtPtr> out(x.size());
    bool one_shape = x.size() > 1;
    for (const CtPtr& c : x) one_shape = one_shape && c->npoly == x[0]->npoly && c->ell == x[0]->ell && c->deg == x[0]->deg;
    std::vector<CtPtr> all;
    if (one_shape) all = new_ct_batch((int)x.size(), x[0]->npoly, x[0]->ell, x[0]->deg + 1, x[0]->scale, x[0]->slots);
    for_runs(x.size(), [&](size_t a, size_t b) { return x[a]->npoly == x[b]->npoly && x[a]->ell == x[b]->ell && x[a]->deg == x[b]->deg; },
             [&](size_t lo, size_t hi) {
                 const CtPtr& f = x[lo];
                 std::vector<CtPtr> o = one_shape ? std::vector<CtPtr>(all.begin() + lo, all.begin() + hi)
                                                  : new_ct_batch((int)(hi - lo), f->npoly, f->ell, f->deg + 1, f->scale, f->slots);
                 EwItems it;
                 it.n = (int)(hi - lo);
                 it.vecs = f->npoly * f->ell;
                 it.b_vecs = f->ell;
                 for (size_t i = lo; i < hi; ++i) {
                     auto enc = p[i]->at(x[i]->ell, c_.sf_real[x[i]->level()]);
                     o[i - lo]->scale = x[i]->scale * enc->scale;
                     it.out[i - lo] = o[i - lo]->d;
                     it.a[i - lo] = x[i]->d;
                     it.b[i - lo] = enc->d;
                     out[i] = o[i - lo];
                 }
                 launch_ew_items(c_.dt, it, 0, f->ell, c_.stream);
                 c_.stats.ct_pt_mult += (u64)(hi - lo);
                 c_.stats.ct_pt_limbs += (u64)(hi - lo) * f->ell;
             });
    launch_ok("mult_plain_each");
    return out;
}

CtPtr Evaluator::dot_plain(const std::vector<CtPtr>& vin, const std::vector<PtPtr>& p, long double pt_scale, const CtPtr& dest) {
    if (vin.size() != p.size() || vin.empty()) throw Error(FHELIN_ERR_ARG, "dot_plain: one plaintext per ciphertext, at least one term");
    std::vector<CtPtr> x = vin;
    {
        std::vector<CtPtr> need;
        std::map<const Ciphertext*, size_t> slot;
        for (size_t i = 0; i < vin.size(); ++i)
            if (vin[i]->deg >= 2 && !slot.count(vin[i].get())) {
                slot[vin[i].get()] = need.size();
                need.push_back(vin[i]);
            }
        if (!need.empty()) {
            std::vector<CtPtr> r = rescale_batch(need);
            for (size_t i = 0; i < vin.size(); ++i)
                if (vin[i]->deg >= 2) x[i] = r[slot[vin[i].get()]];
        }
    }
    bool uniform = x.size() >= 2;
    for (const CtPtr& c : x)
        uniform = uniform && c->npoly == x[0]->npoly && c->ell == x[0]->ell && c->deg == x[0]->deg && fabsl(c->scale / x[0]->scale - 1.0L) < 1e-9L;
    if (!uniform) {
        if (pt_scale > 0) throw Error(FHELIN_ERR_ARG, "dot_plain: an explicit plaintext scale needs uniform operands");
        std::vector<CtPtr> prod = mult_plain_each(x, p);
        CtPtr acc = prod[0];
        for (size_t i = 1; i < prod.size(); ++i) acc = add(acc, prod[i]);
        return acc;
    }
    const CtPtr& f = x[0];
    const long double sf = pt_scale > 0 ? pt_scale : c_.sf_real[f->level()];
    CtPtr acc;
    for (size_t lo = 0; lo < x.size(); lo += EwItems::MAX_ITEMS) {
        const size_t hi = std::min(x.size(), lo + (size_t)EwItems::MAX_ITEMS);
        EwItems it;
        it.n = (int)(hi - lo);
        it.vecs = f->npoly * f->ell;
        it.b_vecs = f->ell;
        for (size_t i = lo; i < hi; ++i) {
            it.a[i - lo] = x[i]->d;
            it.b[i - lo] = p[i]->at(f->ell, sf)->d;
        }
        const bool into_dest = dest && x.size() <= (size_t)EwItems::MAX_ITEMS && dest->npoly == f->npoly && dest->ell == f->ell;
        CtPtr o = into_dest ? dest : new_ct(f->npoly, f->ell, f->deg + 1, f->scale * sf, f->slots);
        if (into_dest) {
            o->deg = f->deg + 1;
            o->scale = f->scale * sf;
            o->slots = f->slots;
        }
        launch_ew_dot(c_.dt, o->d, it, f->ell, c_.stream);
        c_.stats.ct_pt_mult += (u64)(hi - lo);
        c_.stats.ct_pt_limbs += (u64)(hi - lo) * f->ell;
        acc = acc ? add(acc, o) : o;
    }
    launch_ok("dot_plain");
    return acc;
}

bool Evaluator::dot_plain_groups(const std::vector<CtPtr>& cts, const std::vector<std::vector<PtPtr>>& pts, long double pt_scale,
                                 const std::vector<CtPtr>& dest) {
    if (!dot_groups || cts.empty() || cts.size() > (size_t)EwDotGroups::MAX_A || pts.empty() || pts.size() > (size_t)EwDotGroups::MAX_G ||
        dest.size() != pts.size())
        return false;
    const CtPtr& f = cts[0];
    for (const CtPtr& c : cts)
        if (c->npoly != 2 || c->deg != 1 || c->ell != f->ell || fabsl(c->scale / f->scale - 1.0L) > 1e-9L) return false;
    for (const CtPtr& o : dest)
        if (!o || o->npoly != 2 || o->ell != f->ell) return false;
    const long double sf = pt_scale > 0 ? pt_scale : c_.sf_real[f->level()];
    EwDotGroups d;
    d.na = (int)cts.size();
    d.ng = (int)pts.size();
    d.ell = f->ell;
    for (int b = 0; b < d.na; ++b) d.a[b] = cts[b]->d;
    u64 terms = 0;
    for (int g = 0; g < d.ng; ++g) {
        if (pts[g].size() != cts.size()) return false;
        for (int b = 0; b < d.na; ++b) {
            d.p[g][b] = pts[g][b] ? pts[g][b]->at(f->ell, sf)->d : nullptr;
            terms += pts[g][b] ? 1 : 0;
        }
        d.out[g] = dest[g]->d;
        dest[g]->deg = f->deg + 1;
        dest[g]->scale = f->scale * sf;
        dest[g]->slots = f->slots;
    }
    launch_ew_dot_groups(c_.dt, d, c_.stream);
    launch_ok("dot_plain_groups");
    c_.stats.ct_pt_mult += terms;
    c_.stats.ct_pt_limbs += terms * (u64)f->ell;
    return true;
}

bool Evaluator::dot_plain_groups_batch(const std::vector<std::vector<CtPtr>>& cts, const std::vector<std::vector<PtPtr>>& pts, long double pt_scale,
                                       const std::vector<std::vector<CtPtr>>& dest) {
    const size_t nb = cts.size();
    if (!dot_groups || nb < 2 || dest.size() != nb || cts[0].empty() || cts[0].size() > (size_t)EwDotGroups::MAX_A || pts.empty() ||
        pts.size() > (size_t)EwDotGroups::MAX_G)
        return false;
    const size_t na = cts[0].size(), ng = pts.size();
    const CtPtr& f = cts[0][0];
    for (size_t x = 0; x < nb; ++x) {
        if (cts[x].size() != na || dest[x].size() != ng) return false;
        for (const CtPtr& c : cts[x])
            if (c->npoly != 2 || c->deg != 1 || c->ell != f->ell || fabsl(c->scale / f->scale - 1.0L) > 1e-9L) return false;
        for (const CtPtr& o : dest[x])
            if (!o || o->npoly != 2 || o->ell != f->ell) return false;
    }
    EwDotGroups d;
    d.na = (int)na;
    d.ng = (int)ng;
    d.ell = f->ell;
    d.nbatch = (int)nb;
    for (size_t b = 0; b < na; ++b) {
        if (cts[1][b]->d <= cts[0][b]->d) return false;
        const size_t st = (size_t)(cts[1][b]->d - cts[0][b]->d);
        for (size_t x = 0; x < nb; ++x)
            if (cts[x][b]->d != cts[0][b]->d + x * st) return false;
        d.a[b] = cts[0][b]->d;
        d.a_stride[b] = st;
    }
    for (size_t g = 0; g < ng; ++g) {
        if (dest[1][g]->d <= dest[0][g]->d) return false;
        const size_t st = (size_t)(dest[1][g]->d - dest[0][g]->d);
        for (size_t x = 0; x < nb; ++x)
            if (dest[x][g]->d != dest[0][g]->d + x * st) return false;
        d.out[g] = dest[0][g]->d;
        d.out_stride[g] = st;
    }
    const long double sf = pt_scale > 0 ? pt_scale : c_.sf_real[f->level()];
    u64 terms = 0;
    std::vector<std::shared_ptr<Encoding>> hold;
    for (size_t g = 0; g < ng; ++g) {
        if (pts[g].size() != na) return false;
        for (size_t b = 0; b < na; ++b) {
            if (pts[g][b]) {
                hold.push_back(pts[g][b]->at(f->ell, sf));
                d.p[g][b] = hold.back()->d;
                ++terms;
            } else {
                d.p[g][b] = nullptr;
            }
        }
        for (size_t x = 0; x < nb; ++x) {
            dest[x][g]->deg = f->deg + 1;
            dest[x][g]->scale = cts[x][0]->scale * sf;
            dest[x][g]->slots = f->slots;
        }
    }
    launch_ew_dot_groups(c_.dt, d, c_.stream);
    launch_ok("dot_plain_groups_batch");
    c_.stats.ct_pt_mult += terms * nb;
    c_.stats.ct_pt_limbs += terms * nb * (u64)f->ell;
    return true;
}

bool Evaluator::dot_plain_cyclic(const std::vector<CtPtr>& cts, const std::vector<PtPtr>& pts, const std::vector<CtPtr>& dest) {
    constexpr int P = EwCyclic::PERIOD;
    if (cts.empty() || (int)cts.size() > P || (int)pts.size() != P || (int)dest.size() != P) return false;
    const CtPtr& f = cts[0];
    for (const CtPtr& c : cts)
        if (c->npoly != 2 || c->deg != 1 || c->ell != f->ell || fabsl(c->scale / f->scale - 1.0L) > 1e-9L) return false;
    for (const CtPtr& o : dest)
        if (!o || o->npoly != 2 || o->ell != f->ell) return false;
    const long double sf = c_.sf_real[f->level()];
    EwCyclic d;
    d.n = (int)cts.size();
    d.ell = f->ell;
    std::vector<std::shared_ptr<Encoding>> hold;
    for (int j = 0; j < P; ++j) {
        hold.push_back(pts[j]->at(f->ell, sf));
        d.m[j] = hold.back()->d;
        d.a[j] = j < d.n ? cts[j]->d : nullptr;
        d.out[j] = dest[j]->d;
        dest[j]->deg = f->deg + 1;
        dest[j]->scale = f->scale * sf;
        dest[j]->slots = f->slots;
    }
    launch_ew_cyclic_dot(c_.dt, d, c_.stream);
    launch_ok("dot_plain_cyclic");
    c_.stats.ct_pt_mult += (u64)P * d.n;
    c_.stats.ct_pt_limbs += (u64)P * d.n * (u64)f->ell;
    return true;
}

bool Evaluator::dot_plain_window(const std::vector<CtPtr>& cur, const std::vector<CtPtr>& prev, const std::vector<PtPtr>& pts,
                                 const std::vector<CtPtr>& dest, bool accumulate) {
// ... 610 lines not shown
```

### fhe-linformer_amd/csrc/evaluator.h

```cpp
#pragma once
#include <functional>
#include <map>
#include <memory>
#include <vector>
#include "context.h"
#include "kernels_elem.h"

namespace fhelin {

struct DevBlock {
    Context* ctx = nullptr;
    u64* d = nullptr;
    ~DevBlock();
};

struct Ciphertext {
    Context* ctx = nullptr;
    u64* d = nullptr;
    std::shared_ptr<DevBlock> block;
    int npoly = 2;
    int ell = 0;
    int deg = 1;
    long double scale = 0;
    int slots = 0;
    bool async_pending = false;
    int async_lane = 0;
    u64 async_seq = 0;
    hipEvent_t async_ev = nullptr;
    bool seeded = false;
    u64 nonce = 0;
    uint8_t seed[32] = {};
    std::vector<int> wrap_pos;
    int wrap_total = 0;
    bool wrapped() const { return !wrap_pos.empty(); }
    ~Ciphertext();
    int level() const { return ctx->L + 1 - ell; }
    size_t words() const { return (size_t)npoly * ell * ctx->N; }
};
typedef std::shared_ptr<Ciphertext> CtPtr;

struct Encoding {
    Context* ctx = nullptr;
    u64* d = nullptr;
    int ell = 0;
    long double scale = 0;
    hipEvent_t ready = nullptr;
    int made_lane = 0;
    unsigned lanes_ordered = 0;
    ~Encoding();
};

struct Plaintext {
    Context* ctx = nullptr;
    std::vector<double> values;
    std::vector<double> imag;
    int slots = 0;
    int level = 0;
    static constexpr size_t MAX_ENCODINGS = 16;
    std::vector<std::shared_ptr<Encoding>> cache;
    std::shared_ptr<Encoding> at(int ell, long double scale);
};
typedef std::shared_ptr<Plaintext> PtPtr;

struct EvalKey {
    Context* ctx = nullptr;
    u64* d = nullptr;
    mutable u64* d_perm = nullptr;
    int digits = 0;
    bool seeded = false;
    ~EvalKey();
    size_t words() const { return (size_t)digits * 2 * (ctx->L + 1 + ctx->K) * ctx->N; }
};
typedef std::shared_ptr<EvalKey> KeyPtr;

void real_to_scalars(const Context& c, long double v, int ell, ScalarSet& sc);

class Evaluator {
public:
    explicit Evaluator(Context& c) : c_(c) {}
    Context& ctx() { return c_; }

    CtPtr new_ct(int npoly, int ell, int deg, long double scale, int slots);
    std::vector<CtPtr> new_ct_batch(int count, int npoly, int ell, int deg, long double scale, int slots);
    static u64* contiguous_base(const std::vector<CtPtr>& v);
    std::vector<CtPtr> make_contiguous(const std::vector<CtPtr>& v, int site = -1);
    u64 gather_copies[8] = {};
    bool dot_groups = true;
    bool cheb_leaf_at_product = true;
    bool cheb_leaf_classes = true;
    bool cheb_rounds = true;
    int batch_limit = 32;
    CtPtr clone(const CtPtr& a);
    KeyPtr new_key();

    std::map<u64, KeyPtr> rot_keys;
    KeyPtr relin_key;
    KeyPtr conj_key;

    void keyswitch(const u64* c_ntt, int ell, const EvalKey& key, u64* out, const u64* add0, const u64* add1, const u32* map,
                   const u64* post = nullptr);
    void keyswitch_batch(int batch, const u64* c_ntt, size_t c_stride, int ell, const EvalKey& key, u64* out, size_t out_stride,
                         const u64* add0, const u64* add1, size_t add_stride, const u32* map, const u64* post, size_t post_stride);
    struct KsRows {
        std::vector<const EvalKey*> keys;
        std::vector<const u32*> maps;
        bool shared_input = false;
    };
    void keyswitch_rows(const KsRows& rows, const u64* c_ntt, size_t c_stride, int ell, u64* out, size_t out_stride, const u64* add0,
                        size_t add_stride);
    std::vector<CtPtr> rotate_sum_batch(const std::vector<CtPtr>& v, const std::vector<int>& indices);
    bool have_rotation_keys(const std::vector<int>& indices, int slots) const;
    const u64* permuted(const EvalKey& key, const u32* map);
    CtPtr rotate_each_sum(const std::vector<CtPtr>& v, const std::vector<int>& indices);
    std::vector<CtPtr> rotate_each_sum_rows(const std::vector<std::vector<CtPtr>>& rows, const std::vector<int>& indices);
    std::vector<CtPtr> hoisted_dot_rows(const std::vector<CtPtr>& xs, const std::vector<PtPtr>& pts, const std::vector<int>& indices,
                                        bool rescale_out = false);
    bool merged_products = false;
    bool merged_rescale = true;
    bool double_hoist = true;
    struct FoldedKey {
        PtPtr pt;
        KeyPtr key;
        int index = 0;
        long double scale = 0;
        std::shared_ptr<Encoding> enc;
        std::shared_ptr<DevBlock> d;
    };
    std::vector<FoldedKey> folded_keys;
    static constexpr size_t MAX_FOLDED = 12;
    FoldedKey folded_key(const PtPtr& p, int index, long double scale);
    std::vector<CtPtr> rotate_many(const CtPtr& a, const std::vector<int>& indices);
    std::vector<std::vector<CtPtr>> rotate_many_batch(const std::vector<CtPtr>& xs, const std::vector<int>& indices);
    std::vector<CtPtr> rotate_galois_batch(const std::vector<CtPtr>& v, u64 galois, const EvalKey& key, bool accumulate);
    std::vector<CtPtr> conjugate_batch(const std::vector<CtPtr>& v);
    std::vector<CtPtr> raw_modraise_batch(const std::vector<CtPtr>& v, int new_ell);
    std::vector<CtPtr> rotate_each(const std::vector<CtPtr>& v, const std::vector<int>& indices);
    std::vector<CtPtr> rotate_add_batch(const std::vector<CtPtr>& v, int index);
    std::vector<CtPtr> rotate_batch(const std::vector<CtPtr>& v, int index);
    std::vector<CtPtr> rotate_batch_impl(const std::vector<CtPtr>& v, int index, bool accumulate);
    std::vector<CtPtr> mult_plain_batch(const std::vector<CtPtr>& v, const PtPtr& p);
    std::vector<CtPtr> mult_plain_each(const std::vector<CtPtr>& v, const std::vector<PtPtr>& p);
    bool dot_plain_groups(const std::vector<CtPtr>& cts, const std::vector<std::vector<PtPtr>>& pts, long double pt_scale,
                          const std::vector<CtPtr>& dest);
    bool dot_plain_cyclic(const std::vector<CtPtr>& cts, const std::vector<PtPtr>& pts, const std::vector<CtPtr>& dest);
    bool dot_plain_window(const std::vector<CtPtr>& cur, const std::vector<CtPtr>& prev, const std::vector<PtPtr>& pts,
                          const std::vector<CtPtr>& dest, bool accumulate);
    bool dot_plain_groups_batch(const std::vector<std::vector<CtPtr>>& cts, const std::vector<std::vector<PtPtr>>& pts, long double pt_scale,
                                const std::vector<std::vector<CtPtr>>& dest);
    CtPtr dot_plain(const std::vector<CtPtr>& v, const std::vector<PtPtr>& p, long double pt_scale = 0,
                    const CtPtr& dest = CtPtr());
    std::vector<CtPtr> add_batch(const std::vector<CtPtr>& a, const std::vector<CtPtr>& b);
    std::vector<CtPtr> add_plain_batch(const std::vector<CtPtr>& v, const PtPtr& p);
    std::vector<CtPtr> sub_batch(const std::vector<CtPtr>& a, const std::vector<CtPtr>& b);
    std::vector<CtPtr> mult_batch(const std::vector<CtPtr>& a, const std::vector<CtPtr>& b);
    std::vector<CtPtr> mult_affine_rescale_batch(const std::vector<CtPtr>& a, const std::vector<CtPtr>& b, int f, double cadd,
                                                 const std::vector<CtPtr>& sub);
    std::vector<CtPtr> eval_chebyshev_many(const std::vector<CtPtr>& xs, const std::vector<double>& coeffs, double a, double b);
    std::vector<CtPtr> rescale_batch(const std::vector<CtPtr>& v);

    CtPtr add(const CtPtr& a, const CtPtr& b);
    CtPtr sub(const CtPtr& a, const CtPtr& b);
    CtPtr negate(const CtPtr& a);
    CtPtr add_plain(const CtPtr& a, const PtPtr& p);
    CtPtr mult_plain(const CtPtr& a, const PtPtr& p);
    CtPtr mult(const CtPtr& a, const CtPtr& b);
    CtPtr mult_no_relin(const CtPtr& a, const CtPtr& b);
    CtPtr relinearize(const CtPtr& a);
    CtPtr mult_int(const CtPtr& a, u64 k, bool raise_deg, long double new_scale, int keep_ell = 0);
    std::vector<CtPtr> adjust_deg1_batch(const std::vector<CtPtr>& v, int ell, long double scale);
    std::vector<CtPtr> adjust_deg1_batch(const std::vector<CtPtr>& v, int ell, const std::vector<long double>& scales);
    std::vector<CtPtr> scaled_diff_batch(const std::vector<CtPtr>& u, const std::vector<CtPtr>& w, const std::vector<u128>& a,
                                         const std::vector<u128>& c, bool raise_deg, const std::vector<long double>& scales);
    CtPtr mult_real(const CtPtr& a, double c);
    CtPtr add_real(const CtPtr& a, double c);
    CtPtr lincomb(const std::vector<CtPtr>& terms, const std::vector<double>& coef, double c0);
    CtPtr lincomb_at(const std::vector<CtPtr>& terms, const std::vector<double>& coef, double c0, long double want_scale, int keep_ell);
    CtPtr rotate(const CtPtr& a, int index);
    CtPtr conjugate(const CtPtr& a);
    CtPtr eval_poly(const CtPtr& x, const std::vector<double>& coeffs);
    CtPtr eval_chebyshev(const CtPtr& x, const std::vector<double>& coeffs, double a, double b);
    CtPtr mult_many(const std::vector<CtPtr>& v);
    std::vector<CtPtr> eval_poly_many(const std::vector<CtPtr>& xs, const std::vector<double>& coeffs);
    std::vector<CtPtr> mult_many_rows(const std::vector<std::vector<CtPtr>>& vs);
    CtPtr rescale(const CtPtr& a);
    CtPtr level_reduce(const CtPtr& a, int new_ell);
    CtPtr adjust(const CtPtr& a, int ell, int deg, long double scale);

    CtPtr raw_rescale(const CtPtr& a);
    void lift_and_ntt(u64* lifted, const u64* last, int P, int ell, const NttEpilogue* ep = nullptr, const u64* qlm_row = nullptr);
    void rescale_finish(u64* out, const u64* c, const u64* last, int P, int ell, const u64* qlinv_row = nullptr, const u64* qlm_row = nullptr);
    CtPtr raw_rotate(const CtPtr& a, u64 galois, const EvalKey& key, bool accumulate = false);
    CtPtr rotate_add(const CtPtr& a, int index);
    CtPtr raw_mult_relin(const CtPtr& a, const CtPtr& b, const EvalKey& key);
    CtPtr raw_modraise(const CtPtr& a, int new_ell);

private:
    Context& c_;
    void keyswitch_impl(int batch, const KsRows* rows, const u64* c_ntt, size_t c_stride, int ell, const EvalKey* key, u64* out,
                        size_t out_stride, const u64* add0, const u64* add1, size_t add_stride, const u32* map, const u64* post,
                        size_t post_stride);
    Scratch<u64> modup(const KsShape& up, const u64* src, bool times_r2, int group2 = 0, size_t group2_stride = 0);
    void moddown(const KsShape& sh, const u64* accQ, u64* accP, u64* out, const u64* add0, const u64* add1, const u32* map, const u64* post,
                 bool row_pass = false, const std::function<void(const u64* conv)>& finish = nullptr);
    void moddown_rescale(const KsShape& sh, const u64* accQ, u64* accP, u64* out);
    void moddown_rescale_finish(const KsShape& sh, u64* out, const u64* accQ, u64* conv, const u64* minv);
    typedef std::vector<CtPtr> CtRow;
    CtRow cheb_recurse(const std::vector<double>& c, const std::vector<CtRow>& T, const std::map<int, CtRow>& G, int baby);
    std::vector<CtPtr> add_sub_batch(const std::vector<CtPtr>& a, const std::vector<CtPtr>& b, int op);
    void match(const CtPtr& a, const CtPtr& b, CtPtr& ao, CtPtr& bo);
    void match_batch(const std::vector<CtPtr>& a, const std::vector<CtPtr>& b, std::vector<CtPtr>& x, std::vector<CtPtr>& y);
};

}
```

### fhe-linformer_amd/csrc/kernels_elem.h

```cpp
#pragma once
#include "kernels.h"

namespace fhelin {

struct ScalarSet {
    u64 v[128];
};

void launch_ew_mul(const DeviceTables& t, u64* out, const u64* a, const u64* b, int nvec, int b_mod, int limb_first, int limb_count, hipStream_t s);
void launch_ew_add(const DeviceTables& t, u64* out, const u64* a, const u64* b, int nvec, int b_mod, int limb_first, int limb_count, hipStream_t s);
void launch_ew_sub(const DeviceTables& t, u64* out, const u64* a, const u64* b, int nvec, int b_mod, int limb_first, int limb_count, hipStream_t s);
void launch_ew_muladd(const DeviceTables& t, u64* out, const u64* acc, const u64* a, const u64* b, int nvec, int b_mod, int limb_first,
                      int limb_count, hipStream_t s);
void launch_ew_neg(const DeviceTables& t, u64* out, const u64* a, int nvec, int limb_first, int limb_count, hipStream_t s);
void launch_ew_scalar(const DeviceTables& t, u64* out, const u64* a, const ScalarSet& sc, int nvec, int limb_first, int limb_count, hipStream_t s,
                      int in_limbs = 0);
void launch_ew_addscalar(const DeviceTables& t, u64* out, const u64* a, const ScalarSet& sc, int nvec, int limb_first, int limb_count, hipStream_t s,
                         int add_vecs = -1);
struct LinComb {
    static constexpr int MAX_TERMS = 32;
    int n = 0;
    int vecs = 0;
    const u64* a[MAX_TERMS];
};
void launch_ew_lincomb(const DeviceTables& t, u64* out, const LinComb& lc, const u64* scal, int ell, hipStream_t s, int in_limbs = 0);
void launch_tensor(const DeviceTables& t, u64* d, const u64* a, const u64* b, int ell, hipStream_t s);
struct EwItems;
void launch_tensor_items(const DeviceTables& t, const EwItems& it, int ell, hipStream_t s);
void launch_automorph(const DeviceTables& t, u64* out, const u64* in, const u32* map, int nvec, hipStream_t s);
void launch_automorph_pack30(const DeviceTables& t, u64* out, const u64* in, const u32* map, int nvec, hipStream_t s);
struct WrapMaskRow {
    const u64* src;
    u64* dst;
    const u64* mask;
    const u32* map;
    int32_t ell;
    int32_t src_ell;
};
static_assert(sizeof(WrapMaskRow) == 40, "WrapMaskRow is 40 bytes");
void launch_wrap_mask(const DeviceTables& t, const WrapMaskRow* rows, int n_rows, int max_ell, hipStream_t s);
void launch_rescale_lift(const DeviceTables& t, u64* lifted, const u64* last, int npoly, int ell, const u64* qlmod_row, hipStream_t s);
void launch_rescale_finish(const DeviceTables& t, u64* out, const u64* c, const u64* lifted, int npoly, int ell, const u64* qlinv_row,
                           hipStream_t s);
void launch_modraise(const DeviceTables& t, u64* out, const u64* src, int npoly, int src_limb, int nl, hipStream_t s);
void launch_reduce_i128(const DeviceTables& t, u64* out, const u64* coeffs, int limb_first, int nlimbs, hipStream_t s);

struct EwItems {
    static constexpr int MAX_ITEMS = 32;
    int n = 0;
    int vecs = 0;
    int b_vecs = 0;
    u64* out[MAX_ITEMS];
    const u64* a[MAX_ITEMS];
    const u64* b[MAX_ITEMS];
};
void launch_ew_items(const DeviceTables& t, const EwItems& it, int op, int limb_count, hipStream_t s);
struct EwScaledDiff {
    static constexpr int MAX_ITEMS = 32;
    int n = 0;
    int vecs = 0;
    int ell = 0;
    u64* out[MAX_ITEMS];
    const u64* u[MAX_ITEMS];
    const u64* w[MAX_ITEMS];
};
void launch_ew_scaled_diff(const DeviceTables& t, const EwScaledDiff& d, const u64* consts, hipStream_t s);
void launch_ew_dot(const DeviceTables& t, u64* out, const EwItems& it, int limb_count, hipStream_t s);
struct EwDotGroups {
    static constexpr int MAX_A = 16, MAX_G = 8;
    int na = 0, ng = 0, ell = 0;
    const u64* a[MAX_A];
    const u64* p[MAX_G][MAX_A];
    u64* out[MAX_G];
    int nbatch = 1;
    size_t a_stride[MAX_A] = {};
    size_t out_stride[MAX_G] = {};
    u32 pmask[MAX_G] = {};
};
void launch_ew_dot_groups(const DeviceTables& t, const EwDotGroups& d, hipStream_t s);
struct EwCyclic {
    static constexpr int PERIOD = 32;
    int n = 0, ell = 0;
    const u64* a[PERIOD];
    const u64* m[PERIOD];
    u64* out[PERIOD];
};
void launch_ew_cyclic_dot(const DeviceTables& t, const EwCyclic& d, hipStream_t s);
struct EwWindow {
    static constexpr int W = 32;
    int ell = 0, accumulate = 0;
    u32 cur_mask = 0, prev_mask = 0;
    const u64* cur[W];
    const u64* prev[W];
    const u64* m[W];
    u64* out[W];
};
void launch_ew_window_dot(const DeviceTables& t, const EwWindow& d, hipStream_t s);

struct KsShape {
    int ell;
    int k;
    int alpha;
    int beta;
    int L1;
    int batch = 1;
    size_t c_stride = 0;
    size_t out_stride = 0;
    size_t add_stride = 0;
    size_t post_stride = 0;
    static constexpr int MAX_ROWS = 16;
    int per_row = 0;
    int shared_input = 0;
    int row_mod = 0;
    const u64* evk_row[MAX_ROWS] = {};
    const u32* map_row[MAX_ROWS] = {};
    static constexpr int MAX_ROT = 7;
    int n_rot = 0;
    const u64* evk_rot[MAX_ROT] = {};
    const u32* map_rot[MAX_ROT] = {};
    size_t rot_ext_stride = 0;
    size_t rot_input_stride = 0;
    int lds_digits = 0;
    size_t ext_batch_stride = 0;
    const u64* gsrc = nullptr;
    size_t gsrc_stride = 0;
    int tch = 16;
};
void launch_modup_conv(const DeviceTables& t, const KsShape& sh, u64* ext, const u64* cc, const u64* c_ntt, const u64* hatinv,
                       const u64* hatmod, hipStream_t s);
void launch_ks_inner(const DeviceTables& t, const KsShape& sh, u64* accQ, u64* accP, const u64* ext, const u64* evk, const u64* c_ntt,
                     hipStream_t s);
void launch_ks_inner_multi(const DeviceTables& t, const KsShape& sh, u64* accQ, u64* accP, const u64* ext, const u64* c_ntt,
                           hipStream_t s);
void launch_fold_key(const DeviceTables& t, u64* out, const u64* key, const u32* map, const u64* V, int nvec, hipStream_t s);
struct HoistAdd {
    int n_rot = 0;
    const u64* v[KsShape::MAX_ROT + 1] = {};
    const u32* map[KsShape::MAX_ROT] = {};
    u64* acc = nullptr;
    const u64* pmod = nullptr;
};
void launch_hoist_addends(const DeviceTables& t, const KsShape& sh, const HoistAdd& h, u64* pre, const u64* ct, hipStream_t s);
void launch_gather_sum(const DeviceTables& t, const KsShape& sh, u64* out, const u64* in, size_t in_stride, hipStream_t s);
void launch_moddown_conv(const DeviceTables& t, const KsShape& sh, u64* conv, const u64* accP, const u64* phatinv, const u64* phatmod,
                         hipStream_t s);
void launch_affine_acc(const DeviceTables& t, const KsShape& sh, u64* accQ, const u64* d, const u64* sub, const ScalarSet& cst, int has_cst, int f,
                       const u64* pmod, hipStream_t s);
void launch_moddown_rescale_conv(const DeviceTables& t, const KsShape& sh, u64* conv, const u64* accP, const u64* top, const u64* hatinv,
                                 const u64* hatmod, const u64* mmod, hipStream_t s);
void launch_moddown_rescale_finish(const DeviceTables& t, const KsShape& sh, u64* out, const u64* accQ, const u64* conv, const u64* minv,
                                   hipStream_t s);
void launch_moddown_finish(const DeviceTables& t, const KsShape& sh, u64* out, const u64* accQ, const u64* conv, const u64* pinv,
                           const u64* add0, const u64* add1, const u32* map, const u64* post, hipStream_t s);

}
```

### fhe-linformer_amd/csrc/kernels_ks.hip

```cpp
#include <hip/hip_runtime.h>
#include <cstdlib>
#include "kernels.h"
#include "kernels_elem.h"

namespace fhelin {
namespace {

typedef u64 u64x2 __attribute__((ext_vector_type(2)));

__device__ __forceinline__ Barrett load_barrett(const DeviceTables& t, int limb) {
    Barrett b;
    b.q = t.moduli[limb];
    b.r0 = t.barrett[2 * limb];
    b.r1 = t.barrett[2 * limb + 1];
    return b;
}

constexpr int TCH = 16;

template <int MAXA, bool FULL>
__device__ __forceinline__ void modup_body(const DeviceTables& t, const KsShape& sh, u64* __restrict__ ext, const u64* __restrict__ cc,
                                           const u64* __restrict__ hatinv, const u64* __restrict__ hatmod, int j, int lo, int cnt, size_t n) {
    const size_t N = (size_t)1 << t.log_n;
    const int nt = sh.ell + sh.k;
    u32 y0[MAXA], y1[MAXA];
#pragma unroll
    for (int i = 0; i < MAXA; ++i) {
        if (FULL || i < cnt) {
            const int li = lo + i;
            split30(mul_shoup(cc[(size_t)li * N + n], hatinv[2 * li], hatinv[2 * li + 1], t.moduli[li]), y0[i], y1[i]);
        } else {
            y0[i] = y1[i] = 0;
        }
    }
    u64* dst = ext + (size_t)j * nt * N + n;
    const int t0 = blockIdx.z * sh.tch, t1 = min(nt, t0 + sh.tch);
    for (int tt = t0; tt < t1; ++tt) {
        if (tt >= lo && tt < lo + cnt) continue;
        const int limb = tt < sh.ell ? tt : sh.L1 + (tt - sh.ell);
        const u64 qt = t.moduli[limb], qti = t.qinv[limb];
        u64 slo = 0, shi = 0;
#pragma unroll
        for (int i0 = 0; i0 < MAXA; i0 += 8) {
            Acc30 acc = {0, 0, 0};
#pragma unroll
            for (int i = i0; i < i0 + 8 && i < MAXA; ++i)
                if (FULL || i < cnt) {
                    const u64 h = hatmod[(size_t)(lo + i) * nt + tt];
                    mac30(acc, y0[i], y1[i], (u32)h, (u32)(h >> 32));
                }
            acc30_flush(acc, slo, shi);
        }
        dst[(size_t)tt * N] = redc128(slo, shi, qt, qti);
    }
}

template <int MAXA>
__global__ __launch_bounds__(256) void modup_conv_kernel(DeviceTables t, KsShape sh, u64* __restrict__ ext, const u64* __restrict__ cc, const u64* __restrict__ c_ntt,
                                                         const u64* __restrict__ hatinv, const u64* __restrict__ hatmod) {
    const int bi = blockIdx.y / sh.beta, j = blockIdx.y % sh.beta;
    const size_t N = (size_t)1 << t.log_n;
    const size_t n = (size_t)blockIdx.x * 256 + threadIdx.x;
    const int lo = j * sh.alpha;
    const int cnt = min(sh.alpha, sh.ell - lo);
    const int nt = sh.ell + sh.k;
    cc += (size_t)bi * sh.ell * N;
    ext += (size_t)bi * sh.beta * nt * N;
    (void)c_ntt;
    if (cnt == MAXA)
        modup_body<MAXA, true>(t, sh, ext, cc, hatinv, hatmod, j, lo, cnt, n);
    else
        modup_body<MAXA, false>(t, sh, ext, cc, hatinv, hatmod, j, lo, cnt, n);
}

struct KsBlock {
    int bx, bi, tt;
};
__device__ __forceinline__ KsBlock ks_block(const KsShape& sh, int rows = 0) {
    const unsigned nx = gridDim.x, nblk = gridDim.x * gridDim.y;
    const unsigned nb = rows ? (unsigned)rows : (unsigned)sh.batch;
    unsigned b = blockIdx.y * nx + blockIdx.x;
    if ((nblk & 7) == 0) b = (b & 7) * (nblk >> 3) + (b >> 3);
    KsBlock k;
    k.bi = (int)(b % nb);
    k.bx = (int)((b / nb) % nx);
    k.tt = (int)(b / (nb * nx));
    return k;
}

__global__ __launch_bounds__(256) void ks_inner_kernel(DeviceTables t, KsShape sh, u64* __restrict__ accQ, u64* __restrict__ accP, const u64* __restrict__ ext,
                                                       const u64* __restrict__ evk, const u64* __restrict__ c_ntt) {
    const int nt = sh.ell + sh.k;
    const KsBlock kb_ = ks_block(sh);
    const int bi = kb_.bi, tt = kb_.tt;
    const int limb = tt < sh.ell ? tt : sh.L1 + (tt - sh.ell);
    if (sh.row_mod) {
        const int in = bi / sh.row_mod;
        ext += (size_t)in * sh.ext_batch_stride;
        c_ntt += (size_t)in * sh.c_stride;
        evk = sh.evk_row[bi % sh.row_mod];
    } else {
        if (!sh.shared_input) {
            ext += (size_t)bi * sh.beta * nt * ((size_t)1 << t.log_n);
            c_ntt += (size_t)bi * sh.c_stride;
        }
        if (sh.per_row) evk = sh.evk_row[bi];
    }
    const int own = tt < sh.ell ? tt / sh.alpha : -1;
    accQ += (size_t)bi * 2 * sh.ell * ((size_t)1 << t.log_n);
    accP += (size_t)bi * 2 * sh.k * ((size_t)1 << t.log_n);
    const Barrett br = load_barrett(t, limb);
    const size_t row = ((size_t)1 << t.log_n) >> 1;
    const size_t n2 = (size_t)kb_.bx * 256 + threadIdx.x;
    const size_t kstride = (size_t)(sh.L1 + sh.k) * row;
    const u64x2* E = reinterpret_cast<const u64x2*>(ext);
    const u64x2* K = reinterpret_cast<const u64x2*>(evk);
    u64 lo[4] = {0, 0, 0, 0}, hi[4] = {0, 0, 0, 0};
    const u64 monR = t.mont[2 * limb], monRs = t.mont[2 * limb + 1];
    for (int j0 = 0; j0 < sh.beta; j0 += 8) {
        Acc30 b0 = {0, 0, 0}, b1 = {0, 0, 0}, a0 = {0, 0, 0}, a1 = {0, 0, 0};
        const int j1 = min(sh.beta, j0 + 8);
        for (int j = j0; j < j1; ++j) {
            u64x2 d = j == own ? reinterpret_cast<const u64x2*>(c_ntt)[(size_t)tt * row + n2] : E[((size_t)j * nt + tt) * row + n2];
            if (j == own) {
                d.x = mul_shoup(d.x, monR, monRs, br.q);
                d.y = mul_shoup(d.y, monR, monRs, br.q);
            }
            const u64x2 kb = K[(size_t)(2 * j) * kstride + (size_t)limb * row + n2];
            const u64x2 ka = K[(size_t)(2 * j + 1) * kstride + (size_t)limb * row + n2];
            u32 dx0, dx1, dy0, dy1, k0, k1;
            split30(d.x, dx0, dx1);
            split30(d.y, dy0, dy1);
            split30(kb.x, k0, k1);
            mac30(b0, dx0, dx1, k0, k1);
            split30(kb.y, k0, k1);
            mac30(b1, dy0, dy1, k0, k1);
            split30(ka.x, k0, k1);
            mac30(a0, dx0, dx1, k0, k1);
            split30(ka.y, k0, k1);
            mac30(a1, dy0, dy1, k0, k1);
        }
        acc30_flush(b0, lo[0], hi[0]);
        acc30_flush(b1, lo[1], hi[1]);
        acc30_flush(a0, lo[2], hi[2]);
        acc30_flush(a1, lo[3], hi[3]);
    }
    u64x2 rb, ra;
    const u64 qi = t.qinv[limb];
    rb.x = redc128(lo[0], hi[0], br.q, qi);
    rb.y = redc128(lo[1], hi[1], br.q, qi);
    ra.x = redc128(lo[2], hi[2], br.q, qi);
    ra.y = redc128(lo[3], hi[3], br.q, qi);
    if (tt < sh.ell) {
        u64x2* O = reinterpret_cast<u64x2*>(accQ);
        O[(size_t)tt * row + n2] = rb;
        O[(size_t)(sh.ell + tt) * row + n2] = ra;
    } else {
        u64x2* O = reinterpret_cast<u64x2*>(accP);
        const int pj = tt - sh.ell;
        O[(size_t)pj * row + n2] = rb;
        O[(size_t)(sh.k + pj) * row + n2] = ra;
    }
}

__device__ __forceinline__ u32 sel_mask(u32 a, u32 b, unsigned long long mask) {
    u32 r;
    asm("v_cndmask_b32_e64 %0, %1, %2, %3" : "=v"(r) : "v"(a), "v"(b), "s"(mask));
    return r;
}

template <bool STAGE, int ROWS>
__global__ __launch_bounds__(256) void ks_inner_multi_kernel(DeviceTables t, KsShape sh, u64* __restrict__ accQ, u64* __restrict__ accP,
                                                             const u64* __restrict__ ext, const u64* __restrict__ c_ntt) {
    __shared__ u64x2 dl[STAGE ? ROWS : 1][STAGE ? 4 : 1][256];
    const int nt = sh.ell + sh.k;
    const KsBlock kb_ = ks_block(sh, (sh.batch + ROWS - 1) / ROWS);
    const int bi = kb_.bi * ROWS, tt = kb_.tt;
    const int limb = tt < sh.ell ? tt : sh.L1 + (tt - sh.ell);
    const size_t N = (size_t)1 << t.log_n, row = N >> 1;
    const size_t ext_stride = sh.ext_batch_stride ? sh.ext_batch_stride : (size_t)sh.beta * nt * N;
    const int own = tt < sh.ell ? tt / sh.alpha : -1;
    const Barrett br = load_barrett(t, limb);
    const size_t n2 = (size_t)kb_.bx * 256 + threadIdx.x;
    const size_t kstride = (size_t)(sh.L1 + sh.k) * row;
    bool live[ROWS];
    const u64* extr[ROWS];
    const u64* cr_[ROWS];
#pragma unroll
    for (int q = 0; q < ROWS; ++q) {
        live[q] = bi + q < sh.batch;
        const int b = live[q] ? bi + q : bi;
        extr[q] = ext + (size_t)b * ext_stride;
        cr_[q] = c_ntt + (size_t)b * sh.c_stride;
    }
    u64 lo[ROWS][4], hi[ROWS][4];
    Acc30 acc[ROWS][4];
#pragma unroll
    for (int q = 0; q < ROWS; ++q)
#pragma unroll
        for (int i = 0; i < 4; ++i) {
            lo[q][i] = hi[q][i] = 0;
            acc[q][i] = Acc30{0, 0, 0};
        }
    int pending = 0, folded = 0;
    if constexpr (STAGE) {
#pragma unroll
        for (int q = 0; q < ROWS; ++q) {
            const u64x2* __restrict__ e0 = reinterpret_cast<const u64x2*>(extr[q]);
            const u64x2* __restrict__ c0 = reinterpret_cast<const u64x2*>(cr_[q]);
            for (int j = 0; j < sh.beta; ++j) dl[q][j][threadIdx.x] = j == own ? c0[(size_t)tt * row + n2] : e0[((size_t)j * nt + tt) * row + n2];
        }
        __syncthreads();
    }
    struct Operands {
        u64x2 d[ROWS], kb, ka;
    };
    auto map_of = [&](int r) -> u32 { return sh.map_rot[r] ? sh.map_rot[r][2 * n2] : (u32)(2 * n2); };
    auto issue = [&](int r, int j, u32 m0) {
        const size_t mp = m0 >> 1;
        const u64x2* __restrict__ K = reinterpret_cast<const u64x2*>(sh.evk_rot[r]) + (size_t)limb * row + n2;
        Operands o;
#pragma unroll
        for (int q = 0; q < ROWS; ++q) {
            if constexpr (STAGE) {
                o.d[q] = dl[q][j][mp & 255];
            } else {
                const u64x2* __restrict__ er = reinterpret_cast<const u64x2*>(extr[q] + (size_t)r * sh.rot_ext_stride);
                const u64x2* __restrict__ cr = reinterpret_cast<const u64x2*>(cr_[q] + (size_t)r * sh.rot_input_stride);
                o.d[q] = j == own ? cr[(size_t)tt * row + mp] : er[((size_t)j * nt + tt) * row + mp];
            }
        }
        o.kb = K[(size_t)(2 * j) * kstride];
        o.ka = K[(size_t)(2 * j + 1) * kstride];
        return o;
    };
    const int total = sh.n_rot * sh.beta;
    int r = 0, j = 0;
    u32 m_cur = map_of(0), m_nxt = sh.n_rot > 1 ? map_of(1) : 0;
    Operands cur = issue(0, 0, m_cur);
    for (int it = 0; it < total; ++it) {
        int rn = r, jn = j + 1;
        u32 mn = m_cur;
        if (jn == sh.beta) {
            jn = 0;
            rn = r + 1;
            mn = m_nxt;
        }
        Operands nxt = cur;
        if (it + 1 < total) {
            nxt = issue(rn, jn, mn);
            if (jn == 0 && rn + 1 < sh.n_rot) m_nxt = map_of(rn + 1);
        }
        {
            const unsigned long long swp = __ballot((m_cur & 1) != 0);
            const u64x2 kb = cur.kb, ka = cur.ka;
            const u32 kbx0 = (u32)kb.x, kbx1 = (u32)(kb.x >> 32), kby0 = (u32)kb.y, kby1 = (u32)(kb.y >> 32);
            const u32 kax0 = (u32)ka.x, kax1 = (u32)(ka.x >> 32), kay0 = (u32)ka.y, kay1 = (u32)(ka.y >> 32);
#pragma unroll
            for (int q = 0; q < ROWS; ++q) {
                const u64x2 d = cur.d[q];
                u32 p0, p1, q0, q1;
                split30(d.x, p0, p1);
                split30(d.y, q0, q1);
                const u32 dx0 = sel_mask(p0, q0, swp), dx1 = sel_mask(p1, q1, swp), dy0 = sel_mask(q0, p0, swp), dy1 = sel_mask(q1, p1, swp);
                mac30(acc[q][0], dx0, dx1, kbx0, kbx1);
                mac30(acc[q][1], dy0, dy1, kby0, kby1);
                mac30(acc[q][2], dx0, dx1, kax0, kax1);
                mac30(acc[q][3], dy0, dy1, kay0, kay1);
            }
            if (++pending == 8) {
                pending = 0;
                const bool fold = ++folded == 2;
                if (fold) folded = 0;
#pragma unroll
                for (int q = 0; q < ROWS; ++q)
#pragma unroll
                    for (int i = 0; i < 4; ++i) {
                        acc30_flush(acc[q][i], lo[q][i], hi[q][i]);
                        acc[q][i] = Acc30{0, 0, 0};
                        if (fold) {
                            lo[q][i] = barrett_reduce128(lo[q][i], hi[q][i], br);
                            hi[q][i] = 0;
                        }
                    }
            }
        }
        cur = nxt;
        r = rn;
        j = jn;
        m_cur = mn;
    }
#pragma unroll
    for (int q = 0; q < ROWS; ++q) {
        if (!live[q]) continue;
        u64x2 rb, ra;
#pragma unroll
        for (int i = 0; i < 4; ++i) acc30_flush(acc[q][i], lo[q][i], hi[q][i]);
        const u64 qi = t.qinv[limb];
        rb.x = redc128(lo[q][0], hi[q][0], br.q, qi);
        rb.y = redc128(lo[q][1], hi[q][1], br.q, qi);
        ra.x = redc128(lo[q][2], hi[q][2], br.q, qi);
        ra.y = redc128(lo[q][3], hi[q][3], br.q, qi);
        if (tt < sh.ell) {
            u64x2* O = reinterpret_cast<u64x2*>(accQ + (size_t)(bi + q) * 2 * sh.ell * N);
            O[(size_t)tt * row + n2] = rb;
            O[(size_t)(sh.ell + tt) * row + n2] = ra;
        } else {
            u64x2* O = reinterpret_cast<u64x2*>(accP + (size_t)(bi + q) * 2 * sh.k * N);
            const int pj = tt - sh.ell;
            O[(size_t)pj * row + n2] = rb;
            O[(size_t)(sh.k + pj) * row + n2] = ra;
        }
    }
}

__global__ __launch_bounds__(256) void gather_sum_kernel(DeviceTables t, KsShape sh, u64* __restrict__ out, const u64* __restrict__ in,
                                                         size_t in_stride) {
    const int bi = blockIdx.y / sh.ell, tt = blockIdx.y % sh.ell;
    const size_t N = (size_t)1 << t.log_n;
    const size_t n = (size_t)blockIdx.x * 256 + threadIdx.x;
    const u64 q = t.moduli[tt];
    const u64* src = in + (size_t)bi * in_stride + (size_t)tt * N;
    u64 acc = 0;
    for (int r = 0; r < sh.n_rot; ++r) {
        const u64* sr = src + (size_t)r * sh.rot_input_stride;
        acc = add_mod(acc, sr[sh.map_rot[r] ? (size_t)sh.map_rot[r][n] : n], q);
    }
    out[((size_t)bi * sh.ell + tt) * N + n] = acc;
}

template <int MAXK, bool FULL>
__device__ __forceinline__ void moddown_body(const DeviceTables& t, const KsShape& sh, u64* __restrict__ conv, const u64* __restrict__ accP,
                                             const u64* __restrict__ phatinv, const u64* __restrict__ phatmod, int c, size_t n) {
    const size_t N = (size_t)1 << t.log_n;
    u32 z0[MAXK], z1[MAXK];
#pragma unroll
    for (int p = 0; p < MAXK; ++p) {
        if (FULL || p < sh.k) {
            split30(mul_shoup(accP[((size_t)c * sh.k + p) * N + n], phatinv[2 * p], phatinv[2 * p + 1], t.moduli[sh.L1 + p]), z0[p], z1[p]);
        } else {
            z0[p] = z1[p] = 0;
        }
    }
    u64* dst = conv + (size_t)c * sh.ell * N + n;
    const int t0 = blockIdx.z * sh.tch, t1 = min(sh.ell, t0 + sh.tch);
    for (int tt = t0; tt < t1; ++tt) {
        const u64 qt = t.moduli[tt], qti = t.qinv[tt];
        u64 slo = 0, shi = 0;
#pragma unroll
        for (int p0 = 0; p0 < MAXK; p0 += 8) {
            Acc30 acc = {0, 0, 0};
#pragma unroll
            for (int p = p0; p < p0 + 8 && p < MAXK; ++p)
                if (FULL || p < sh.k) {
                    const u64 h = phatmod[(size_t)p * sh.L1 + tt];
                    mac30(acc, z0[p], z1[p], (u32)h, (u32)(h >> 32));
                }
            acc30_flush(acc, slo, shi);
        }
        dst[(size_t)tt * N] = redc128(slo, shi, qt, qti);
    }
}

template <int MAXK>
__global__ __launch_bounds__(256) void moddown_conv_kernel(DeviceTables t, KsShape sh, u64* __restrict__ conv, const u64* __restrict__ accP, const u64* __restrict__ phatinv,
                                                           const u64* __restrict__ phatmod) {
    const int bi = blockIdx.y >> 1, c = blockIdx.y & 1;
    const size_t N = (size_t)1 << t.log_n;
    const size_t n = (size_t)blockIdx.x * 256 + threadIdx.x;
    accP += (size_t)bi * 2 * sh.k * N;
    conv += (size_t)bi * 2 * sh.ell * N;
    if (sh.k == MAXK)
        moddown_body<MAXK, true>(t, sh, conv, accP, phatinv, phatmod, c, n);
    else
        moddown_body<MAXK, false>(t, sh, conv, accP, phatinv, phatmod, c, n);
}

__global__ __launch_bounds__(256) void moddown_finish_kernel(DeviceTables t, KsShape sh, u64* __restrict__ out, const u64* __restrict__ accQ, const u64* __restrict__ conv,
                                                             const u64* __restrict__ pinv, const u64* __restrict__ add0, const u64* __restrict__ add1, const u32* __restrict__ map,
                                                             const u64* __restrict__ post) {
    const int bi = blockIdx.y / (2 * sh.ell), v = blockIdx.y % (2 * sh.ell);
    const int c = v / sh.ell, tt = v % sh.ell;
    const u64 q = t.moduli[tt];
    const u64 w = pinv[2 * tt], ws = pinv[2 * tt + 1];
    const size_t N = (size_t)1 << t.log_n;
    const size_t j = ((size_t)blockIdx.x * 256 + threadIdx.x) * 2;
    accQ += (size_t)bi * 2 * sh.ell * N;
    conv += (size_t)bi * 2 * sh.ell * N;
    out += (size_t)bi * sh.out_stride;
    const u64* add = c == 0 ? add0 : add1;
    if (add) add += (size_t)(sh.row_mod ? bi / sh.row_mod : bi) * sh.add_stride;
    if (post) post += (size_t)bi * sh.post_stride;
    if (sh.per_row) map = sh.map_row[sh.row_mod ? bi % sh.row_mod : bi];
    u64x2 r;
    if (map) {
        const u32 m0 = map[j], m1 = map[j + 1];
        r.x = mul_shoup(sub_mod(accQ[(size_t)v * N + m0], conv[(size_t)v * N + m0], q), w, ws, q);
        r.y = mul_shoup(sub_mod(accQ[(size_t)v * N + m1], conv[(size_t)v * N + m1], q), w, ws, q);
        if (add) {
            r.x = add_mod(r.x, add[(size_t)tt * N + m0], q);
            r.y = add_mod(r.y, add[(size_t)tt * N + m1], q);
        }
    } else {
        const u64x2 a = reinterpret_cast<const u64x2*>(accQ)[((size_t)v * N + j) >> 1];
        const u64x2 b = reinterpret_cast<const u64x2*>(conv)[((size_t)v * N + j) >> 1];
        r.x = mul_shoup(sub_mod(a.x, b.x, q), w, ws, q);
        r.y = mul_shoup(sub_mod(a.y, b.y, q), w, ws, q);
        if (add) {
            const u64x2 d = reinterpret_cast<const u64x2*>(add)[((size_t)tt * N + j) >> 1];
            r.x = add_mod(r.x, d.x, q);
            r.y = add_mod(r.y, d.y, q);
        }
    }
    if (post) {
        const u64x2 p = reinterpret_cast<const u64x2*>(post)[((size_t)v * N + j) >> 1];
        r.x = add_mod(r.x, p.x, q);
        r.y = add_mod(r.y, p.y, q);
    }
    if (sh.gsrc && c == 0) {
        const u64* __restrict__ g = sh.gsrc + (size_t)bi * sh.gsrc_stride + (size_t)tt * N;
        for (int rr = 0; rr < sh.n_rot; ++rr) {
            const u64* __restrict__ gr = g + (size_t)rr * sh.rot_input_stride;
            const u32* __restrict__ mr = sh.map_rot[rr];
            const u32 m0 = mr ? mr[j] : (u32)j;
            const u64x2 gp = reinterpret_cast<const u64x2*>(gr)[m0 >> 1];
            r.x = add_mod(r.x, (m0 & 1) ? gp.y : gp.x, q);
            r.y = add_mod(r.y, (m0 & 1) ? gp.x : gp.y, q);
        }
    }
    reinterpret_cast<u64x2*>(out)[((size_t)v * N + j) >> 1] = r;
}

__global__ __launch_bounds__(256) void fold_key_kernel(DeviceTables t, u64* __restrict__ out, const u64* __restrict__ key, const u32* __restrict__ map,
                                                       const u64* __restrict__ V) {
    const size_t v = blockIdx.y;
    const int limb = (int)(v % (size_t)t.n_limbs);
    const Barrett br = load_barrett(t, limb);
    const size_t N = (size_t)1 << t.log_n;
    const size_t j = ((size_t)blockIdx.x * 256 + threadIdx.x) * 2;
    const u32 m0 = map[j], m1 = map[j + 1];
    const u64x2 pv = reinterpret_cast<const u64x2*>(V)[((size_t)limb * N + j) >> 1];
    u64x2 r;
    const u64 R = t.mont[2 * limb], Rs = t.mont[2 * limb + 1];
    r.x = pack30(mul_shoup(mul_mod(pv.x, key[v * N + m0], br), R, Rs, br.q));
    r.y = pack30(mul_shoup(mul_mod(pv.y, key[v * N + m1], br), R, Rs, br.q));
    reinterpret_cast<u64x2*>(out)[(v * N + j) >> 1] = r;
}

__global__ __launch_bounds__(256) void hoist_addends_kernel(DeviceTables t, KsShape sh, HoistAdd h, u64* __restrict__ pre, const u64* __restrict__ ct) {
    const int bi = blockIdx.y / (2 * sh.ell), v = blockIdx.y % (2 * sh.ell);
    const int c = v / sh.ell, tt = v % sh.ell;
    const Barrett br = load_barrett(t, tt);
    const size_t N = (size_t)1 << t.log_n, row = N >> 1;
    const size_t n2 = (size_t)blockIdx.x * 256 + threadIdx.x;
    const u64x2* __restrict__ src = reinterpret_cast<const u64x2*>(ct + (size_t)bi * sh.c_stride + (size_t)v * N);
    const u64x2 x = src[n2];
    const u64x2 p0 = reinterpret_cast<const u64x2*>(h.v[0])[(size_t)tt * row + n2];
    Acc128 a0 = {0, 0}, a1 = {0, 0};
    acc_mac(a0, x.x, p0.x);
    acc_mac(a1, x.y, p0.y);
    if (c == 0)
        for (int r = 0; r < h.n_rot; ++r) {
            const u32 m0 = h.map[r][2 * n2];
            const u64x2 g = src[m0 >> 1];
            const u64x2 pr = reinterpret_cast<const u64x2*>(h.v[r + 1])[(size_t)tt * row + n2];
            acc_mac(a0, (m0 & 1) ? g.y : g.x, pr.x);
            acc_mac(a1, (m0 & 1) ? g.x : g.y, pr.y);
        }
    u64x2 o;
    o.x = barrett_reduce128(a0.lo, a0.hi, br);
    o.y = barrett_reduce128(a1.lo, a1.hi, br);
    if (h.acc) {
        u64x2* A = reinterpret_cast<u64x2*>(h.acc + (size_t)bi * 2 * sh.ell * N) + (size_t)v * row + n2;
        const u64 w = h.pmod[2 * tt], ws = h.pmod[2 * tt + 1];
        u64x2 a = *A;
        a.x = add_mod(a.x, mul_shoup(o.x, w, ws, br.q), br.q);
        a.y = add_mod(a.y, mul_shoup(o.y, w, ws, br.q), br.q);
        *A = a;
        return;
    }
    reinterpret_cast<u64x2*>(pre + (size_t)bi * 2 * sh.ell * N)[(size_t)v * row + n2] = o;
}

__global__ __launch_bounds__(256) void affine_acc_kernel(DeviceTables t, KsShape sh, u64* __restrict__ accQ, const u64* __restrict__ d,
                                                         const u64* __restrict__ sub, ScalarSet cst, int has_cst, int f, const u64* __restrict__ pmod) {
    const int bi = blockIdx.y / (2 * sh.ell), v = blockIdx.y % (2 * sh.ell);
    const int c = v / sh.ell, tt = v % sh.ell;
    const u64 q = t.moduli[tt];
    const size_t row = ((size_t)1 << t.log_n) >> 1;
    const size_t n2 = (size_t)blockIdx.x * 256 + threadIdx.x;
    u64x2 x = reinterpret_cast<const u64x2*>(d)[((size_t)bi * 3 * sh.ell + v) * row + n2];
    if (f == 2) {
        x.x = add_mod(x.x, x.x, q);
        x.y = add_mod(x.y, x.y, q);
    }
    if (has_cst && c == 0) {
        x.x = add_mod(x.x, cst.v[2 * tt], q);
        x.y = add_mod(x.y, cst.v[2 * tt], q);
    }
    if (sub) {
        const u64x2 sv = reinterpret_cast<const u64x2*>(sub)[((size_t)bi * 2 * sh.ell + v) * row + n2];
        x.x = sub_mod(x.x, sv.x, q);
        x.y = sub_mod(x.y, sv.y, q);
    }
    u64x2* A = reinterpret_cast<u64x2*>(accQ) + ((size_t)bi * 2 * sh.ell + v) * row + n2;
    u64x2 a = *A;
    if (f == 2) {
        a.x = add_mod(a.x, a.x, q);
        a.y = add_mod(a.y, a.y, q);
    }
    const u64 w = pmod[2 * tt], ws = pmod[2 * tt + 1];
    a.x = add_mod(a.x, mul_shoup(x.x, w, ws, q), q);
    a.y = add_mod(a.y, mul_shoup(x.y, w, ws, q), q);
    *A = a;
}

__global__ __launch_bounds__(256) void moddown_rescale_conv_kernel(DeviceTables t, KsShape sh, u64* __restrict__ conv, const u64* __restrict__ accP,
                                                                   const u64* __restrict__ top, const u64* __restrict__ hatinv,
                                                                   const u64* __restrict__ hatmod, const u64* __restrict__ mmod) {
    constexpr int MAXS = 16;
    const int bi = blockIdx.y >> 1, c = blockIdx.y & 1;
    const size_t N = (size_t)1 << t.log_n;
    const size_t n = (size_t)blockIdx.x * 256 + threadIdx.x;
    const int e1 = sh.ell - 1, ns = sh.k + 1;
    u32 z0[MAXS], z1[MAXS];
    u32 neg = 0;
#pragma unroll
    for (int p = 0; p < MAXS; ++p) {
        if (p < ns) {
            const u64 x = p < sh.k ? accP[(((size_t)bi * 2 + c) * sh.k + p) * N + n] : top[((size_t)bi * 2 + c) * N + n];
            const u64 m = t.moduli[p < sh.k ? sh.L1 + p : sh.ell - 1];
            const u64 y = mul_shoup(x, hatinv[2 * p], hatinv[2 * p + 1], m);
            neg += y > (m >> 1);
            split30(y, z0[p], z1[p]);
        } else {
            z0[p] = z1[p] = 0;
        }
    }
    u64* dst = conv + ((size_t)bi * 2 + c) * e1 * N + n;
    const int t0 = blockIdx.z * sh.tch, t1 = min(e1, t0 + sh.tch);
    for (int tt = t0; tt < t1; ++tt) {
        const Barrett br = load_barrett(t, tt);
        u64 slo = 0, shi = 0;
#pragma unroll
        for (int p0 = 0; p0 < MAXS; p0 += 8) {
            Acc30 acc = {0, 0, 0};
#pragma unroll
            for (int p = p0; p < p0 + 8; ++p)
                if (p < ns) {
                    const u64 hm = hatmod[(size_t)p * e1 + tt];
                    mac30(acc, z0[p], z1[p], (u32)hm, (u32)(hm >> 32));
                }
            acc30_flush(acc, slo, shi);
        }
        dst[(size_t)tt * N] = sub_mod(barrett_reduce128(slo, shi, br), barrett_reduce128((u64)neg * mmod[tt], 0, br), br.q);
    }
}

__global__ __launch_bounds__(256) void moddown_rescale_finish_kernel(DeviceTables t, KsShape sh, u64* __restrict__ out, const u64* __restrict__ accQ,
                                                                     const u64* __restrict__ conv, const u64* __restrict__ minv) {
    const int e1 = sh.ell - 1;
    const int bi = blockIdx.y / (2 * e1), v = blockIdx.y % (2 * e1);
    const int c = v / e1, tt = v % e1;
    const u64 q = t.moduli[tt];
    const u64 w = minv[2 * tt], ws = minv[2 * tt + 1];
    const size_t row = ((size_t)1 << t.log_n) >> 1;
    const size_t n2 = (size_t)blockIdx.x * 256 + threadIdx.x;
    const u64x2 a = reinterpret_cast<const u64x2*>(accQ)[(((size_t)bi * 2 + c) * sh.ell + tt) * row + n2];
    const u64x2 b = reinterpret_cast<const u64x2*>(conv)[(((size_t)bi * 2 + c) * e1 + tt) * row + n2];
    u64x2 r;
    r.x = mul_shoup(sub_mod(a.x, b.x, q), w, ws, q);
    r.y = mul_shoup(sub_mod(a.y, b.y, q), w, ws, q);
    reinterpret_cast<u64x2*>(out + (size_t)bi * sh.out_stride)[(size_t)v * row + n2] = r;
}

}

void launch_fold_key(const DeviceTables& t, u64* out, const u64* key, const u32* map, const u64* V, int nvec, hipStream_t s) {
    hipLaunchKernelGGL(fold_key_kernel, dim3((1u << t.log_n) / 512, (unsigned)nvec), dim3(256), 0, s, t, out, key, map, V);
}
void launch_hoist_addends(const DeviceTables& t, const KsShape& sh, const HoistAdd& h, u64* pre, const u64* ct, hipStream_t s) {
    hipLaunchKernelGGL(hoist_addends_kernel, dim3((1u << t.log_n) / 512, (unsigned)(sh.batch * 2 * sh.ell)), dim3(256), 0, s, t, sh, h, pre, ct);
}

void launch_affine_acc(const DeviceTables& t, const KsShape& sh, u64* accQ, const u64* d, const u64* sub, const ScalarSet& cst, int has_cst, int f,
                       const u64* pmod, hipStream_t s) {
    hipLaunchKernelGGL(affine_acc_kernel, dim3((1u << t.log_n) / 512, (unsigned)(sh.batch * 2 * sh.ell)), dim3(256), 0, s, t, sh, accQ, d, sub, cst,
                       has_cst, f, pmod);
}
static int conv_tch(unsigned planes, int targets) {
    static const int force = [] {
        const char* e = std::getenv("FHELIN_CONV_CHUNKS");
        return e ? std::atoi(e) : 0;
    }();
    if (force || planes < 2048u) return TCH;
    return targets > TCH ? targets : TCH;
}
void launch_moddown_rescale_conv(const DeviceTables& t, const KsShape& sh_in, u64* conv, const u64* accP, const u64* top, const u64* hatinv,
                                 const u64* hatmod, const u64* mmod, hipStream_t s) {
    KsShape sh = sh_in;
    const unsigned nx = (1u << t.log_n) / 256;
    sh.tch = conv_tch(nx * (unsigned)(sh.batch * 2), sh.ell - 1);
    dim3 g(nx, (unsigned)(sh.batch * 2), (unsigned)((sh.ell - 1 + sh.tch - 1) / sh.tch));
    hipLaunchKernelGGL(moddown_rescale_conv_kernel, g, dim3(256), 0, s, t, sh, conv, accP, top, hatinv, hatmod, mmod);
}
void launch_moddown_rescale_finish(const DeviceTables& t, const KsShape& sh, u64* out, const u64* accQ, const u64* conv, const u64* minv,
                                   hipStream_t s) {
    dim3 g((1u << t.log_n) / 512, (unsigned)(sh.batch * 2 * (sh.ell - 1)));
    hipLaunchKernelGGL(moddown_rescale_finish_kernel, g, dim3(256), 0, s, t, sh, out, accQ, conv, minv);
}

void launch_modup_conv(const DeviceTables& t, const KsShape& sh_in, u64* ext, const u64* cc, const u64* c_ntt, const u64* hatinv,
                       const u64* hatmod, hipStream_t s) {
    KsShape sh = sh_in;
    const unsigned nx = (1u << t.log_n) / 256;
    sh.tch = conv_tch(nx * (unsigned)(sh.batch * sh.beta), sh.ell + sh.k);
    dim3 g(nx, (unsigned)(sh.batch * sh.beta), (unsigned)((sh.ell + sh.k + sh.tch - 1) / sh.tch));
#define FHELIN_MODUP_CASE(A) case A: hipLaunchKernelGGL((modup_conv_kernel<A>), g, dim3(256), 0, s, t, sh, ext, cc, c_ntt, hatinv, hatmod); break;
    switch (sh.alpha) {
        FHELIN_MODUP_CASE(1) FHELIN_MODUP_CASE(2) FHELIN_MODUP_CASE(3) FHELIN_MODUP_CASE(4)
        FHELIN_MODUP_CASE(5) FHELIN_MODUP_CASE(6) FHELIN_MODUP_CASE(7) FHELIN_MODUP_CASE(8)
        default: hipLaunchKernelGGL((modup_conv_kernel<16>), g, dim3(256), 0, s, t, sh, ext, cc, c_ntt, hatinv, hatmod); break;
    }
#undef FHELIN_MODUP_CASE
}
void launch_ks_inner(const DeviceTables& t, const KsShape& sh, u64* accQ, u64* accP, const u64* ext, const u64* evk, const u64* c_ntt,
                     hipStream_t s) {
    dim3 g((1u << t.log_n) / 512, (unsigned)(sh.batch * (sh.ell + sh.k)));
    hipLaunchKernelGGL(ks_inner_kernel, g, dim3(256), 0, s, t, sh, accQ, accP, ext, evk, c_ntt);
}
void launch_ks_inner_multi(const DeviceTables& t, const KsShape& sh, u64* accQ, u64* accP, const u64* ext, const u64* c_ntt,
                           hipStream_t s) {
    static const int pair_rows = [] { const char* e = std::getenv("FHELIN_KS_ROW_PAIRS"); return e ? std::atoi(e) : 1; }();
    const bool stage = sh.lds_digits && sh.rot_ext_stride == 0 && sh.beta <= 4;
    if (pair_rows && sh.batch >= 2) {
        dim3 g((1u << t.log_n) / 512, (unsigned)(((sh.batch + 1) / 2) * (sh.ell + sh.k)));
        if (stage)
            hipLaunchKernelGGL((ks_inner_multi_kernel<true, 2>), g, dim3(256), 0, s, t, sh, accQ, accP, ext, c_ntt);
        else
            hipLaunchKernelGGL((ks_inner_multi_kernel<false, 2>), g, dim3(256), 0, s, t, sh, accQ, accP, ext, c_ntt);
        return;
    }
    dim3 g((1u << t.log_n) / 512, (unsigned)(sh.batch * (sh.ell + sh.k)));
    if (stage)
        hipLaunchKernelGGL((ks_inner_multi_kernel<true, 1>), g, dim3(256), 0, s, t, sh, accQ, accP, ext, c_ntt);
    else
        hipLaunchKernelGGL((ks_inner_multi_kernel<false, 1>), g, dim3(256), 0, s, t, sh, accQ, accP, ext, c_ntt);
}
void launch_gather_sum(const DeviceTables& t, const KsShape& sh, u64* out, const u64* in, size_t in_stride, hipStream_t s) {
    dim3 g((1u << t.log_n) / 256, (unsigned)(sh.batch * sh.ell));
    hipLaunchKernelGGL(gather_sum_kernel, g, dim3(256), 0, s, t, sh, out, in, in_stride);
}
void launch_moddown_conv(const DeviceTables& t, const KsShape& sh_in, u64* conv, const u64* accP, const u64* phatinv, const u64* phatmod,
                         hipStream_t s) {
    KsShape sh = sh_in;
    const unsigned nx = (1u << t.log_n) / 256;
    sh.tch = conv_tch(nx * (unsigned)(2 * sh.batch), sh.ell);
    dim3 g(nx, (unsigned)(2 * sh.batch), (unsigned)((sh.ell + sh.tch - 1) / sh.tch));
#define FHELIN_MODDOWN_CASE(K) case K: hipLaunchKernelGGL((moddown_conv_kernel<K>), g, dim3(256), 0, s, t, sh, conv, accP, phatinv, phatmod); break;
    switch (sh.k) {
        FHELIN_MODDOWN_CASE(1) FHELIN_MODDOWN_CASE(2) FHELIN_MODDOWN_CASE(3) FHELIN_MODDOWN_CASE(4)
        FHELIN_MODDOWN_CASE(5) FHELIN_MODDOWN_CASE(6) FHELIN_MODDOWN_CASE(7) FHELIN_MODDOWN_CASE(8)
        default: hipLaunchKernelGGL((moddown_conv_kernel<16>), g, dim3(256), 0, s, t, sh, conv, accP, phatinv, phatmod); break;
    }
#undef FHELIN_MODDOWN_CASE
}
void launch_moddown_finish(const DeviceTables& t, const KsShape& sh, u64* out, const u64* accQ, const u64* conv, const u64* pinv,
                           const u64* add0, const u64* add1, const u32* map, const u64* post, hipStream_t s) {
    dim3 g((1u << t.log_n) / 512, (unsigned)(sh.batch * 2 * sh.ell));
    hipLaunchKernelGGL(moddown_finish_kernel, g, dim3(256), 0, s, t, sh, out, accQ, conv, pinv, add0, add1, map, post);
}

}
```

Before: 240.1.

## Fold rotation automorphism into key-switch inner product and sum addend into row pass

Adds a rot_gather mode, on by default, in which single and batched rotations apply the automorphism inside the key-switch inner kernel. The kernel reads permuted NTT indices with a parity swap and uses pre-permuted evaluation keys, and ModDown conversion applies a sign correction from the inverse Galois element. This removes the separate un-permuted modup and permuting finish pass. The rotate-sum paths also move the c0 gather-sum, scaled by P mod q, into the inner kernel so the row-pass ModDown can finish directly. It adds template variants, per-map Galois bookkeeping and correctness risk in the sign and index handling.

```diff
diff --git a/fhe-linformer_amd/csrc/context.cpp b/fhe-linformer_amd/csrc/context.cpp
--- a/fhe-linformer_amd/csrc/context.cpp
+++ b/fhe-linformer_amd/csrc/context.cpp
@@ -314,6 +314,7 @@
         if (const char* e = std::getenv("FHELIN_FUSE_FINISH")) fuse_finish = std::atoi(e) != 0;
         if (const char* e = std::getenv("FHELIN_HOST_ENCODE")) host_encode = std::atoi(e) != 0;
         if (const char* e = std::getenv("FHELIN_FUSE_GATHER")) fuse_gather = std::atoi(e) != 0;
+        if (const char* e = std::getenv("FHELIN_ROT_GATHER")) rot_gather = std::atoi(e) != 0;
         if (const char* e = std::getenv("FHELIN_FUSE_LIFT")) fuse_lift = std::atoi(e) != 0;
         if (const char* e = std::getenv("FHELIN_LDS_DIGITS")) lds_digits = std::atoi(e) != 0;
         if (const char* e = std::getenv("FHELIN_NTT_TRACE")) trace_small_ntt = std::atoi(e);
@@ -664,7 +665,15 @@
     }
     automorph_inverse[d] = di;
     automorph_inverse[di] = d;
+    automorph_ginv[d] = (u32)gi;
+    automorph_ginv[di] = (u32)g;
     return d;
+}
+
+u32 Context::automorph_ginv_of(const u32* map) const {
+    auto it = automorph_ginv.find(map);
+    if (it == automorph_ginv.end()) throw Error(FHELIN_ERR_INTERNAL, "automorphism map without a registered Galois element");
+    return it->second;
 }
 
 const u32* Context::automorph_inverse_of(const u32* map) {
diff --git a/fhe-linformer_amd/csrc/context.h b/fhe-linformer_amd/csrc/context.h
--- a/fhe-linformer_amd/csrc/context.h
+++ b/fhe-linformer_amd/csrc/context.h
@@ -232,10 +232,13 @@
     const u32* automorph_map(u64 galois);
     const u32* automorph_inverse_of(const u32* map);
     std::map<const u32*, const u32*> automorph_inverse;
+    u32 automorph_ginv_of(const u32* map) const;
+    std::map<const u32*, u32> automorph_ginv;
     bool fuse_finish = true;
     bool fuse_moddown = false;
     bool host_encode = false;
     bool fuse_gather = true;
+    bool rot_gather = true;
     bool fuse_lift = true;
     bool lds_digits = true;
     struct FftDev {
diff --git a/fhe-linformer_amd/csrc/evaluator.cpp b/fhe-linformer_amd/csrc/evaluator.cpp
--- a/fhe-linformer_amd/csrc/evaluator.cpp
+++ b/fhe-linformer_amd/csrc/evaluator.cpp
@@ -156,12 +156,33 @@
     shu.batch = shared ? 1 : B;
     c_.stats.keyswitch += (u64)B;
     c_.stats.keyswitch_limbs += (u64)B * ell;
-    Scratch<u64> ext = modup(shu, c_ntt, true);
+    const bool identity = !map && !rows;
+    const bool gather = !identity && !add1 && rot_in_gather();
+    const u64* evk = key ? key->d : nullptr;
+    if (gather) {
+        sh.gather = 1;
+        if (rows) {
+            for (int b = 0; b < B; ++b) {
+                sh.evk_row[b] = permuted(*rows->keys[b], rows->maps[b]);
+                sh.ginv_row[b] = c_.automorph_ginv_of(rows->maps[b]);
+            }
+        } else {
+            evk = permuted(*key, map);
+            sh.map_row[0] = map;
+            sh.ginv = c_.automorph_ginv_of(map);
+        }
+        if (add0) {
+            sh.gsrc = add0;
+            sh.gsrc_stride = add_stride;
+            sh.gsrc_pmod = c_.d_pmod;
+        }
+    }
+    Scratch<u64> ext = modup(shu, c_ntt, !gather);
     Scratch<u64> accQ = c_.scratch<u64>((size_t)B * 2 * ell * N);
     Scratch<u64> accP = c_.scratch<u64>((size_t)B * 2 * K * N);
-    launch_ks_inner(c_.dt, sh, accQ, accP, ext, key ? key->d : nullptr, c_ntt, c_.stream);
-    const bool identity = !map && !rows;
-    moddown(sh, accQ, accP, out, add0, add1, map, post, c_.fuse_moddown || (c_.fuse_finish && identity));
+    launch_ks_inner(c_.dt, sh, accQ, accP, ext, evk, c_ntt, c_.stream);
+    if (gather) moddown(sh, accQ, accP, out, nullptr, nullptr, nullptr, post, true);
+    else moddown(sh, accQ, accP, out, add0, add1, map, post, c_.fuse_moddown || (c_.fuse_finish && identity));
     launch_ok("keyswitch");
 }
 
@@ -196,6 +217,7 @@
                         const u64* post, bool row_pass, const std::function<void(const u64* conv)>& finish) {
     const size_t N = c_.N;
     const int B = sh.batch, ell = sh.ell, K = c_.K;
+    if (row_pass && sh.gsrc && !sh.gsrc_pmod) throw Error(FHELIN_ERR_INTERNAL, "moddown: the row pass cannot gather");
     c_.ntt(LimbBatch{accP, B * 2 * K, nullptr, c_.L + 1, K}, true);
     Scratch<u64> conv = c_.scratch<u64>((size_t)B * 2 * ell * N);
     launch_moddown_conv(c_.dt, sh, conv, accP, c_.d_phatinv, c_.d_phatmod, c_.stream);
@@ -213,7 +235,8 @@
         ep.add_stride = sh.add_stride;
         ep.post = post;
         ep.post_stride = sh.post_stride;
-        if (sh.per_row) {
+        if (sh.gather) {
+        } else if (sh.per_row) {
             ep.per_row = 1;
             for (int b = 0; b < B; ++b) ep.invmap_row[b] = c_.automorph_inverse_of(sh.map_row[b]);
         } else if (map) {
@@ -332,16 +355,19 @@
             Scratch<u64> ext = modup(sh, base + pn, false);
             Scratch<u64> accQ = c_.scratch<u64>((size_t)B * 2 * ell * N);
             Scratch<u64> accP = c_.scratch<u64>((size_t)B * 2 * K * N);
-            launch_ks_inner_multi(c_.dt, sh, accQ, accP, ext, base + pn, s);
-            Scratch<u64> c0sum;
+            const bool rp = sum_in_row_pass();
             if (c_.fuse_gather) {
                 sh.gsrc = base;
                 sh.gsrc_stride = ctw;
-            } else {
+                if (rp) sh.gsrc_pmod = c_.d_pmod;
+            }
+            launch_ks_inner_multi(c_.dt, sh, accQ, accP, ext, base + pn, s);
+            Scratch<u64> c0sum;
+            if (!c_.fuse_gather) {
                 c0sum = c_.scratch<u64>((size_t)B * ell * N);
                 launch_gather_sum(c_.dt, sh, c0sum, base, ctw, s);
             }
-            moddown(sh, accQ, accP, o[0]->d, c0sum, nullptr, nullptr, base);
+            moddown(sh, accQ, accP, o[0]->d, c0sum, nullptr, nullptr, base, rp);
             launch_ok("rotate_sum_batch");
         }
         for (int b = 0; b < B; ++b) {
@@ -476,7 +502,7 @@
             if (!merged) {
                 Scratch<u64> pre = c_.scratch<u64>((size_t)B * ctw);
                 launch_hoist_addends(c_.dt, sh, h, pre, base, s);
-                moddown(sh, accQ, accP, o[0]->d, nullptr, nullptr, nullptr, pre);
+                moddown(sh, accQ, accP, o[0]->d, nullptr, nullptr, nullptr, pre, sum_in_row_pass());
             } else {
                 h.acc = accQ;
                 h.pmod = c_.d_pmod;
@@ -546,16 +572,19 @@
             c_.stats.keyswitch_limbs += (u64)R * ell;
             Scratch<u64> accQ = c_.scratch<u64>((size_t)2 * ell * N);
             Scratch<u64> accP = c_.scratch<u64>((size_t)2 * K * N);
-            launch_ks_inner_multi(c_.dt, sh, accQ, accP, ext, base + pn, s);
-            Scratch<u64> c0sum;
+            const bool rp = sum_in_row_pass();
             if (c_.fuse_gather) {
                 sh.gsrc = base;
                 sh.gsrc_stride = 0;
-            } else {
+                if (rp) sh.gsrc_pmod = c_.d_pmod;
+            }
+            launch_ks_inner_multi(c_.dt, sh, accQ, accP, ext, base + pn, s);
+            Scratch<u64> c0sum;
+            if (!c_.fuse_gather) {
                 c0sum = c_.scratch<u64>((size_t)ell * N);
                 launch_gather_sum(c_.dt, sh, c0sum, base, 0, s);
             }
-            moddown(sh, accQ, accP, o->d, c0sum, nullptr, nullptr, nullptr);
+            moddown(sh, accQ, accP, o->d, c0sum, nullptr, nullptr, nullptr, rp);
             launch_ok("rotate_each_sum");
         }
         acc = acc ? add(acc, o) : o;
@@ -634,14 +663,16 @@
                 sh.map_rot[r] = c_.automorph_map(g);
                 sh.evk_rot[r] = permuted(*rot_keys.at(g), sh.map_rot[r]);
             }
+            const bool rp = sum_in_row_pass();
             sh.gsrc = base;
             sh.gsrc_stride = row_stride;
+            if (rp) sh.gsrc_pmod = c_.d_pmod;
             c_.stats.keyswitch += (u64)B * R;
             c_.stats.keyswitch_limbs += (u64)B * R * ell;
             Scratch<u64> accQ = c_.scratch<u64>((size_t)B * 2 * ell * N);
             Scratch<u64> accP = c_.scratch<u64>((size_t)B * 2 * K * N);
             launch_ks_inner_multi(c_.dt, sh, accQ, accP, ext, base + pn, s);
-            moddown(sh, accQ, accP, o[0]->d, nullptr, nullptr, nullptr, nullptr);
+            moddown(sh, accQ, accP, o[0]->d, nullptr, nullptr, nullptr, nullptr, rp);
             launch_ok("rotate_each_sum_rows");
         }
         for (int b = 0; b < B; ++b) out[lo + b] = o[b];
@@ -890,6 +921,7 @@
     }
     const int R = (int)todo.size();
     if (R == 0) return out;
+    const bool gather = rot_in_gather() && R <= (int)KsShape::MAX_ROWS;
     std::vector<const EvalKey*> keys;
     std::vector<const u32*> maps;
     for (size_t k : todo) {
@@ -917,7 +949,7 @@
         c_.stats.keyswitch_limbs += (u64)rows * ell;
         std::vector<CtPtr> o = new_ct_batch(rows, 2, ell, xs[lo]->deg, xs[lo]->scale, xs[lo]->slots);
         {
-            Scratch<u64> ext = modup(KsShape{ell, K, c_.alpha, lt.beta, L1, B, ctw, 0, 0, 0}, base + pn, true);
+            Scratch<u64> ext = modup(KsShape{ell, K, c_.alpha, lt.beta, L1, B, ctw, 0, 0, 0}, base + pn, !gather);
             Scratch<u64> accQ = c_.scratch<u64>((size_t)rows * 2 * ell * N);
             Scratch<u64> accP = c_.scratch<u64>((size_t)rows * 2 * K * N);
             auto row_shape = [&](int first, int cnt) {
@@ -947,21 +979,36 @@
                     }
             };
             const bool one_chunk = R <= (int)KsShape::MAX_ROWS;
-            if (one_chunk) launch_ks_inner(c_.dt, row_shape(0, R), accQ, accP, ext, nullptr, base + pn, s);
-            else
-                for_row_chunks([&](const KsShape& sh1, size_t row0, int i) {
-                    launch_ks_inner(c_.dt, sh1, accQ + row0 * 2 * ell * N, accP + row0 * 2 * K * N, ext + (size_t)i * lt.beta * nt * N, nullptr,
-                                    base + pn + (size_t)i * ctw, s);
-                });
-            moddown(KsShape{ell, K, c_.alpha, lt.beta, L1, rows, 0, ctw, 0, 0}, accQ, accP, nullptr, nullptr, nullptr, nullptr, nullptr, false,
-                    [&](const u64* conv) {
-                        if (one_chunk) launch_moddown_finish(c_.dt, row_shape(0, R), o[0]->d, accQ, conv, c_.d_pinv, base, nullptr, nullptr, nullptr, s);
-                        else
-                            for_row_chunks([&](const KsShape& sh1, size_t row0, int i) {
-                                launch_moddown_finish(c_.dt, sh1, o[row0]->d, accQ + row0 * 2 * ell * N, conv + row0 * 2 * ell * N, c_.d_pinv,
-                                                      base + (size_t)i * ctw, nullptr, nullptr, nullptr, s);
-                            });
+            if (gather) {
+                KsShape sh = row_shape(0, R);
+                sh.gather = 1;
+                for (int b = 0; b < R; ++b) {
+                    sh.evk_row[b] = permuted(*keys[b], maps[b]);
+                    sh.ginv_row[b] = c_.automorph_ginv_of(maps[b]);
+                }
+                sh.gsrc = base;
+                sh.gsrc_stride = ctw;
+                sh.gsrc_pmod = c_.d_pmod;
+                launch_ks_inner(c_.dt, sh, accQ, accP, ext, nullptr, base + pn, s);
+                moddown(sh, accQ, accP, o[0]->d, nullptr, nullptr, nullptr, nullptr, true);
+            } else {
+                if (one_chunk) launch_ks_inner(c_.dt, row_shape(0, R), accQ, accP, ext, nullptr, base + pn, s);
+                else
+                    for_row_chunks([&](const KsShape& sh1, size_t row0, int i) {
+                        launch_ks_inner(c_.dt, sh1, accQ + row0 * 2 * ell * N, accP + row0 * 2 * K * N, ext + (size_t)i * lt.beta * nt * N, nullptr,
+                                        base + pn + (size_t)i * ctw, s);
                     });
+                moddown(KsShape{ell, K, c_.alpha, lt.beta, L1, rows, 0, ctw, 0, 0}, accQ, accP, nullptr, nullptr, nullptr, nullptr, nullptr, false,
+                        [&](const u64* conv) {
+                            if (one_chunk)
+                                launch_moddown_finish(c_.dt, row_shape(0, R), o[0]->d, accQ, conv, c_.d_pinv, base, nullptr, nullptr, nullptr, s);
+                            else
+                                for_row_chunks([&](const KsShape& sh1, size_t row0, int i) {
+                                    launch_moddown_finish(c_.dt, sh1, o[row0]->d, accQ + row0 * 2 * ell * N, conv + row0 * 2 * ell * N,
+                                                          c_.d_pinv, base + (size_t)i * ctw, nullptr, nullptr, nullptr, s);
+                                });
+                        });
+            }
             launch_ok("rotate_many_batch");
         }
         for (int i = 0; i < B; ++i)
diff --git a/fhe-linformer_amd/csrc/evaluator.h b/fhe-linformer_amd/csrc/evaluator.h
--- a/fhe-linformer_amd/csrc/evaluator.h
+++ b/fhe-linformer_amd/csrc/evaluator.h
@@ -203,6 +203,8 @@
     void moddown(const KsShape& sh, const u64* accQ, u64* accP, u64* out, const u64* add0, const u64* add1, const u32* map, const u64* post,
                  bool row_pass = false, const std::function<void(const u64* conv)>& finish = nullptr);
     void moddown_rescale(const KsShape& sh, const u64* accQ, u64* accP, u64* out);
+    bool sum_in_row_pass() const { return c_.fuse_finish && c_.rot_gather; }
+    bool rot_in_gather() const { return c_.fuse_finish && c_.rot_gather && !c_.fuse_moddown; }
     void moddown_rescale_finish(const KsShape& sh, u64* out, const u64* accQ, u64* conv, const u64* minv);
     typedef std::vector<CtPtr> CtRow;
     CtRow cheb_recurse(const std::vector<double>& c, const std::vector<CtRow>& T, const std::map<int, CtRow>& G, int baby);
diff --git a/fhe-linformer_amd/csrc/kernels_elem.h b/fhe-linformer_amd/csrc/kernels_elem.h
--- a/fhe-linformer_amd/csrc/kernels_elem.h
+++ b/fhe-linformer_amd/csrc/kernels_elem.h
@@ -124,6 +124,10 @@
     size_t ext_batch_stride = 0;
     const u64* gsrc = nullptr;
     size_t gsrc_stride = 0;
+    const u64* gsrc_pmod = nullptr;
+    int gather = 0;
+    u32 ginv = 0;
+    u32 ginv_row[MAX_ROWS] = {};
     int tch = 16;
 };
 void launch_modup_conv(const DeviceTables& t, const KsShape& sh, u64* ext, const u64* cc, const u64* c_ntt, const u64* hatinv,
diff --git a/fhe-linformer_amd/csrc/kernels_ks.hip b/fhe-linformer_amd/csrc/kernels_ks.hip
--- a/fhe-linformer_amd/csrc/kernels_ks.hip
+++ b/fhe-linformer_amd/csrc/kernels_ks.hip
@@ -88,14 +88,22 @@
     return k;
 }
 
+__device__ __forceinline__ u32 sel_mask(u32 a, u32 b, unsigned long long mask) {
+    u32 r;
+    asm("v_cndmask_b32_e64 %0, %1, %2, %3" : "=v"(r) : "v"(a), "v"(b), "s"(mask));
+    return r;
+}
+
+template <bool GATHER>
 __global__ __launch_bounds__(256) void ks_inner_kernel(DeviceTables t, KsShape sh, u64* __restrict__ accQ, u64* __restrict__ accP, const u64* __restrict__ ext,
                                                        const u64* __restrict__ evk, const u64* __restrict__ c_ntt) {
     const int nt = sh.ell + sh.k;
     const KsBlock kb_ = ks_block(sh);
     const int bi = kb_.bi, tt = kb_.tt;
     const int limb = tt < sh.ell ? tt : sh.L1 + (tt - sh.ell);
+    const int in = sh.row_mod ? bi / sh.row_mod : bi;
+    const int ri = sh.per_row ? (sh.row_mod ? bi % sh.row_mod : bi) : 0;
     if (sh.row_mod) {
-        const int in = bi / sh.row_mod;
         ext += (size_t)in * sh.ext_batch_stride;
         c_ntt += (size_t)in * sh.c_stride;
         evk = sh.evk_row[bi % sh.row_mod];
@@ -117,28 +125,47 @@
     const u64x2* K = reinterpret_cast<const u64x2*>(evk);
     u64 lo[4] = {0, 0, 0, 0}, hi[4] = {0, 0, 0, 0};
     const u64 monR = t.mont[2 * limb], monRs = t.mont[2 * limb + 1];
+    size_t nd = n2;
+    [[maybe_unused]] u32 m0 = 0;
+    [[maybe_unused]] unsigned long long swp = 0;
+    if constexpr (GATHER) {
+        m0 = sh.map_row[ri][2 * n2];
+        nd = m0 >> 1;
+        swp = __ballot((m0 & 1) != 0);
+    }
     for (int j0 = 0; j0 < sh.beta; j0 += 8) {
         Acc30 b0 = {0, 0, 0}, b1 = {0, 0, 0}, a0 = {0, 0, 0}, a1 = {0, 0, 0};
         const int j1 = min(sh.beta, j0 + 8);
         for (int j = j0; j < j1; ++j) {
-            u64x2 d = j == own ? reinterpret_cast<const u64x2*>(c_ntt)[(size_t)tt * row + n2] : E[((size_t)j * nt + tt) * row + n2];
-            if (j == own) {
-                d.x = mul_shoup(d.x, monR, monRs, br.q);
-                d.y = mul_shoup(d.y, monR, monRs, br.q);
-            }
+            u64x2 d = j == own ? reinterpret_cast<const u64x2*>(c_ntt)[(size_t)tt * row + nd] : E[((size_t)j * nt + tt) * row + nd];
             const u64x2 kb = K[(size_t)(2 * j) * kstride + (size_t)limb * row + n2];
             const u64x2 ka = K[(size_t)(2 * j + 1) * kstride + (size_t)limb * row + n2];
-            u32 dx0, dx1, dy0, dy1, k0, k1;
-            split30(d.x, dx0, dx1);
-            split30(d.y, dy0, dy1);
-            split30(kb.x, k0, k1);
-            mac30(b0, dx0, dx1, k0, k1);
-            split30(kb.y, k0, k1);
-            mac30(b1, dy0, dy1, k0, k1);
-            split30(ka.x, k0, k1);
-            mac30(a0, dx0, dx1, k0, k1);
-            split30(ka.y, k0, k1);
-            mac30(a1, dy0, dy1, k0, k1);
+            if constexpr (GATHER) {
+                u32 p0, p1, q0, q1;
+                split30(d.x, p0, p1);
+                split30(d.y, q0, q1);
+                const u32 dx0 = sel_mask(p0, q0, swp), dx1 = sel_mask(p1, q1, swp), dy0 = sel_mask(q0, p0, swp), dy1 = sel_mask(q1, p1, swp);
+                mac30(b0, dx0, dx1, (u32)kb.x, (u32)(kb.x >> 32));
+                mac30(b1, dy0, dy1, (u32)kb.y, (u32)(kb.y >> 32));
+                mac30(a0, dx0, dx1, (u32)ka.x, (u32)(ka.x >> 32));
+                mac30(a1, dy0, dy1, (u32)ka.y, (u32)(ka.y >> 32));
+            } else {
+                if (j == own) {
+                    d.x = mul_shoup(d.x, monR, monRs, br.q);
+                    d.y = mul_shoup(d.y, monR, monRs, br.q);
+                }
+                u32 dx0, dx1, dy0, dy1, k0, k1;
+                split30(d.x, dx0, dx1);
+                split30(d.y, dy0, dy1);
+                split30(kb.x, k0, k1);
+                mac30(b0, dx0, dx1, k0, k1);
+                split30(kb.y, k0, k1);
+                mac30(b1, dy0, dy1, k0, k1);
+                split30(ka.x, k0, k1);
+                mac30(a0, dx0, dx1, k0, k1);
+                split30(ka.y, k0, k1);
+                mac30(a1, dy0, dy1, k0, k1);
+            }
         }
         acc30_flush(b0, lo[0], hi[0]);
         acc30_flush(b1, lo[1], hi[1]);
@@ -152,6 +179,14 @@
     ra.x = redc128(lo[2], hi[2], br.q, qi);
     ra.y = redc128(lo[3], hi[3], br.q, qi);
     if (tt < sh.ell) {
+        if constexpr (GATHER) {
+            if (sh.gsrc_pmod) {
+                const u64x2 gp = reinterpret_cast<const u64x2*>(sh.gsrc + (size_t)in * sh.gsrc_stride)[(size_t)tt * row + nd];
+                const u64 w = sh.gsrc_pmod[2 * tt], ws = sh.gsrc_pmod[2 * tt + 1];
+                rb.x = add_mod(rb.x, mul_shoup((m0 & 1) ? gp.y : gp.x, w, ws, br.q), br.q);
+                rb.y = add_mod(rb.y, mul_shoup((m0 & 1) ? gp.x : gp.y, w, ws, br.q), br.q);
+            }
+        }
         u64x2* O = reinterpret_cast<u64x2*>(accQ);
         O[(size_t)tt * row + n2] = rb;
         O[(size_t)(sh.ell + tt) * row + n2] = ra;
@@ -161,12 +196,6 @@
         O[(size_t)pj * row + n2] = rb;
         O[(size_t)(sh.k + pj) * row + n2] = ra;
     }
-}
-
-__device__ __forceinline__ u32 sel_mask(u32 a, u32 b, unsigned long long mask) {
-    u32 r;
-    asm("v_cndmask_b32_e64 %0, %1, %2, %3" : "=v"(r) : "v"(a), "v"(b), "s"(mask));
-    return r;
 }
 
 template <bool STAGE, int ROWS>
@@ -290,6 +319,33 @@
         j = jn;
         m_cur = mn;
     }
+    u64 gx[ROWS], gy[ROWS];
+#pragma unroll
+    for (int q = 0; q < ROWS; ++q) gx[q] = gy[q] = 0;
+    if (sh.gsrc_pmod && tt < sh.ell) {
+        for (int r0 = 0; r0 < sh.n_rot; r0 += 4) {
+            int rr[4];
+            u32 mm[4];
+#pragma unroll
+            for (int i = 0; i < 4; ++i) {
+                rr[i] = r0 + i < sh.n_rot ? r0 + i : r0;
+                mm[i] = map_of(rr[i]);
+            }
+#pragma unroll
+            for (int q = 0; q < ROWS; ++q) {
+                const u64* __restrict__ g = sh.gsrc + (size_t)(live[q] ? bi + q : bi) * sh.gsrc_stride + (size_t)tt * N;
+                u64x2 gp[4];
+#pragma unroll
+                for (int i = 0; i < 4; ++i) gp[i] = reinterpret_cast<const u64x2*>(g + (size_t)rr[i] * sh.rot_input_stride)[mm[i] >> 1];
+#pragma unroll
+                for (int i = 0; i < 4; ++i) {
+                    const bool on = r0 + i < sh.n_rot, odd = (mm[i] & 1) != 0;
+                    gx[q] = add_mod(gx[q], on ? (odd ? gp[i].y : gp[i].x) : 0, br.q);
+                    gy[q] = add_mod(gy[q], on ? (odd ? gp[i].x : gp[i].y) : 0, br.q);
+                }
+            }
+        }
+    }
 #pragma unroll
     for (int q = 0; q < ROWS; ++q) {
         if (!live[q]) continue;
@@ -302,6 +358,11 @@
         ra.x = redc128(lo[q][2], hi[q][2], br.q, qi);
         ra.y = redc128(lo[q][3], hi[q][3], br.q, qi);
         if (tt < sh.ell) {
+            if (sh.gsrc_pmod) {
+                const u64 w = sh.gsrc_pmod[2 * tt], ws = sh.gsrc_pmod[2 * tt + 1];
+                rb.x = add_mod(rb.x, mul_shoup(gx[q], w, ws, br.q), br.q);
+                rb.y = add_mod(rb.y, mul_shoup(gy[q], w, ws, br.q), br.q);
+            }
             u64x2* O = reinterpret_cast<u64x2*>(accQ + (size_t)(bi + q) * 2 * sh.ell * N);
             O[(size_t)tt * row + n2] = rb;
             O[(size_t)(sh.ell + tt) * row + n2] = ra;
@@ -329,15 +390,18 @@
     out[((size_t)bi * sh.ell + tt) * N + n] = acc;
 }
 
-template <int MAXK, bool FULL>
+template <int MAXK, bool FULL, bool SIGNED>
 __device__ __forceinline__ void moddown_body(const DeviceTables& t, const KsShape& sh, u64* __restrict__ conv, const u64* __restrict__ accP,
-                                             const u64* __restrict__ phatinv, const u64* __restrict__ phatmod, int c, size_t n) {
+                                             const u64* __restrict__ phatinv, const u64* __restrict__ phatmod, int c, size_t n, bool neg) {
     const size_t N = (size_t)1 << t.log_n;
     u32 z0[MAXK], z1[MAXK];
 #pragma unroll
     for (int p = 0; p < MAXK; ++p) {
         if (FULL || p < sh.k) {
-            split30(mul_shoup(accP[((size_t)c * sh.k + p) * N + n], phatinv[2 * p], phatinv[2 * p + 1], t.moduli[sh.L1 + p]), z0[p], z1[p]);
+            const u64 m = t.moduli[sh.L1 + p];
+            u64 x = accP[((size_t)c * sh.k + p) * N + n];
+            if constexpr (SIGNED) x = neg && x ? m - x : x;
+            split30(mul_shoup(x, phatinv[2 * p], phatinv[2 * p + 1], m), z0[p], z1[p]);
         } else {
             z0[p] = z1[p] = 0;
         }
@@ -358,11 +422,13 @@
                 }
             acc30_flush(acc, slo, shi);
         }
-        dst[(size_t)tt * N] = redc128(slo, shi, qt, qti);
-    }
-}
-
-template <int MAXK>
+        u64 r = redc128(slo, shi, qt, qti);
+        if constexpr (SIGNED) r = neg && r ? qt - r : r;
+        dst[(size_t)tt * N] = r;
+    }
+}
+
+template <int MAXK, bool SIGNED = false>
 __global__ __launch_bounds__(256) void moddown_conv_kernel(DeviceTables t, KsShape sh, u64* __restrict__ conv, const u64* __restrict__ accP, const u64* __restrict__ phatinv,
                                                            const u64* __restrict__ phatmod) {
     const int bi = blockIdx.y >> 1, c = blockIdx.y & 1;
@@ -370,10 +436,15 @@
     const size_t n = (size_t)blockIdx.x * 256 + threadIdx.x;
     accP += (size_t)bi * 2 * sh.k * N;
     conv += (size_t)bi * 2 * sh.ell * N;
+    bool neg = false;
+    if constexpr (SIGNED) {
+        const u32 gi = sh.per_row ? sh.ginv_row[sh.row_mod ? bi % sh.row_mod : bi] : sh.ginv;
+        neg = ((gi * (u32)n) & (u32)(2 * N - 1)) >= (u32)N;
+    }
     if (sh.k == MAXK)
-        moddown_body<MAXK, true>(t, sh, conv, accP, phatinv, phatmod, c, n);
+        moddown_body<MAXK, true, SIGNED>(t, sh, conv, accP, phatinv, phatmod, c, n, neg);
     else
-        moddown_body<MAXK, false>(t, sh, conv, accP, phatinv, phatmod, c, n);
+        moddown_body<MAXK, false, SIGNED>(t, sh, conv, accP, phatinv, phatmod, c, n, neg);
 }
 
 __global__ __launch_bounds__(256) void moddown_finish_kernel(DeviceTables t, KsShape sh, u64* __restrict__ out, const u64* __restrict__ accQ, const u64* __restrict__ conv,
@@ -417,7 +488,7 @@
         r.x = add_mod(r.x, p.x, q);
         r.y = add_mod(r.y, p.y, q);
     }
-    if (sh.gsrc && c == 0) {
+    if (sh.gsrc && !sh.gsrc_pmod && c == 0) {
         const u64* __restrict__ g = sh.gsrc + (size_t)bi * sh.gsrc_stride + (size_t)tt * N;
         for (int rr = 0; rr < sh.n_rot; ++rr) {
             const u64* __restrict__ gr = g + (size_t)rr * sh.rot_input_stride;
@@ -627,7 +698,10 @@
 void launch_ks_inner(const DeviceTables& t, const KsShape& sh, u64* accQ, u64* accP, const u64* ext, const u64* evk, const u64* c_ntt,
                      hipStream_t s) {
     dim3 g((1u << t.log_n) / 512, (unsigned)(sh.batch * (sh.ell + sh.k)));
-    hipLaunchKernelGGL(ks_inner_kernel, g, dim3(256), 0, s, t, sh, accQ, accP, ext, evk, c_ntt);
+    if (sh.gather)
+        hipLaunchKernelGGL(ks_inner_kernel<true>, g, dim3(256), 0, s, t, sh, accQ, accP, ext, evk, c_ntt);
+    else
+        hipLaunchKernelGGL(ks_inner_kernel<false>, g, dim3(256), 0, s, t, sh, accQ, accP, ext, evk, c_ntt);
 }
 void launch_ks_inner_multi(const DeviceTables& t, const KsShape& sh, u64* accQ, u64* accP, const u64* ext, const u64* c_ntt,
                            hipStream_t s) {
@@ -657,12 +731,19 @@
     const unsigned nx = (1u << t.log_n) / 256;
     sh.tch = conv_tch(nx * (unsigned)(2 * sh.batch), sh.ell);
     dim3 g(nx, (unsigned)(2 * sh.batch), (unsigned)((sh.ell + sh.tch - 1) / sh.tch));
-#define FHELIN_MODDOWN_CASE(K) case K: hipLaunchKernelGGL((moddown_conv_kernel<K>), g, dim3(256), 0, s, t, sh, conv, accP, phatinv, phatmod); break;
-    switch (sh.k) {
-        FHELIN_MODDOWN_CASE(1) FHELIN_MODDOWN_CASE(2) FHELIN_MODDOWN_CASE(3) FHELIN_MODDOWN_CASE(4)
-        FHELIN_MODDOWN_CASE(5) FHELIN_MODDOWN_CASE(6) FHELIN_MODDOWN_CASE(7) FHELIN_MODDOWN_CASE(8)
-        default: hipLaunchKernelGGL((moddown_conv_kernel<16>), g, dim3(256), 0, s, t, sh, conv, accP, phatinv, phatmod); break;
-    }
+#define FHELIN_MODDOWN_CASE(K, S) case K: hipLaunchKernelGGL((moddown_conv_kernel<K, S>), g, dim3(256), 0, s, t, sh, conv, accP, phatinv, phatmod); break;
+#define FHELIN_MODDOWN_SWITCH(S)                                                                                                                \
+    switch (sh.k) {                                                                                                                             \
+        FHELIN_MODDOWN_CASE(1, S) FHELIN_MODDOWN_CASE(2, S) FHELIN_MODDOWN_CASE(3, S) FHELIN_MODDOWN_CASE(4, S)                                 \
+        FHELIN_MODDOWN_CASE(5, S) FHELIN_MODDOWN_CASE(6, S) FHELIN_MODDOWN_CASE(7, S) FHELIN_MODDOWN_CASE(8, S)                                 \
+        default: hipLaunchKernelGGL((moddown_conv_kernel<16, S>), g, dim3(256), 0, s, t, sh, conv, accP, phatinv, phatmod); break;              \
+    }
+    if (sh.gather) {
+        FHELIN_MODDOWN_SWITCH(true)
+    } else {
+        FHELIN_MODDOWN_SWITCH(false)
+    }
+#undef FHELIN_MODDOWN_SWITCH
 #undef FHELIN_MODDOWN_CASE
 }
 void launch_moddown_finish(const DeviceTables& t, const KsShape& sh, u64* out, const u64* accQ, const u64* conv, const u64* pinv,
```

Measured after the change: 235.5 (median of 6 runs). 1.9% less time.
